# APRIL-ZJU/Ctrl-VIO

Measured on NVIDIA H100. Metric: residual+Jacobian block evaluations per second (sliding-window LM solve), higher is better.
Workload: dtype f64

## Files before the change

ctrl-vio_b200/csrc/engine.cu:

```cuda
#include <atomic>
#include <cmath>
#include <cstdlib>
#include <map>

#include "engine_state.h"

namespace ctvio::host {

int refresh_mirror(ctvio_engine* e) {
  const size_t need = 4 * size_t(e->nK) + kPStride * size_t(e->nK) + 6 * size_t(std::max(e->nB, 1)) + size_t(std::max(e->nL, 1)) + 8;
  if (need > e->h_mirror_cap) {
    if (e->h_mirror) cudaFreeHost(e->h_mirror);
    e->h_mirror = nullptr;
    e->h_mirror_cap = 0;
    if (cudaHostAlloc(reinterpret_cast<void**>(&e->h_mirror), (2 * need) * sizeof(double), cudaHostAllocDefault) != cudaSuccess) {
      cudaGetLastError();
      e->mirror_valid = false;
      return CTVIO_OK;
    }
    e->h_mirror_cap = 2 * need;
  }
  DevState& x = e->x[e->cur];
  double* m = e->h_mirror;
  cudaStream_t st = e->stream;
  CUDA_OK(cudaMemcpyAsync(m, x.q.p, 4 * size_t(e->nK) * sizeof(double), cudaMemcpyDeviceToHost, st));
  m += 4 * size_t(e->nK);
  CUDA_OK(cudaMemcpyAsync(m, x.p.p, kPStride * size_t(e->nK) * sizeof(double), cudaMemcpyDeviceToHost, st));
  m += kPStride * size_t(e->nK);
  if (e->nB) CUDA_OK(cudaMemcpyAsync(m, x.bias.p, 6 * size_t(e->nB) * sizeof(double), cudaMemcpyDeviceToHost, st));
  m += 6 * size_t(std::max(e->nB, 1));
  if (e->nL) CUDA_OK(cudaMemcpyAsync(m, x.rho.p, size_t(e->nL) * sizeof(double), cudaMemcpyDeviceToHost, st));
  m += size_t(std::max(e->nL, 1));
  CUDA_OK(cudaMemcpyAsync(m, x.ld.p, sizeof(double), cudaMemcpyDeviceToHost, st));
  e->mirror_valid = true;
  return CTVIO_OK;
}

int knot_window_first(const ctvio_engine* e, int64_t t) {
  int64_t s = (t - e->cfg.t0_ns) / e->cfg.dt_ns;
  return int(s);
}

bool knot_window(const ctvio_engine* e, int64_t t, int& first, int& last) {
  const int64_t maxt = e->cfg.t0_ns + int64_t(e->nK - 3) * e->cfg.dt_ns;
  if (t < e->cfg.t0_ns || t >= maxt) return false;
  const int smax = e->nK - 4;
  const int s1 = knot_window_first(e, t);
  int64_t t2 = t + e->cfg.rs_padding_ns;
  int s2 = (t2 >= maxt) ? smax : int((t2 - e->cfg.t0_ns) / e->cfg.dt_ns);
  if (s2 > s1 + 1) return false;
  first = s1;
  last = std::min(s2 + 3, e->nK - 1);
  return true;
}

int prepare_prior(ctvio_engine* e);
int fetch_new_prior(ctvio_engine* e);

int prepare(ctvio_engine* e) {
  if (!e->have_knots) return fail(CTVIO_ERR_STATE, "knots have not been set");
  ArenaScope arena(e);
  if (e->nK < 4) return fail(CTVIO_ERR_STATE, "need at least 4 knots");
  if (!e->have_bias) { e->nB = 0; }
  cudaStream_t st = e->stream;
  const ProblemDims d = e->dims();
  if (e->structure_dirty) {
    e->shard_checked = false;
    const int n = int(e->img.size());
    std::vector<int32_t>&wi0 = e->img_wi0, &wj0 = e->img_wj0;
    wi0.resize(n); wj0.resize(n);
    e->img_li.resize(n); e->img_lj.resize(n);
    e->h_lo.assign(e->nL, INT32_MAX);
    e->h_hi.assign(e->nL, 0);
    struct WinCache { int64_t t = INT64_MIN; int f = 0, l = 0; bool ok = false; } wc[64];
    auto window_of = [&](int64_t t, int& f, int& l) {
      WinCache& c = wc[size_t(uint64_t(t) * 0x9E3779B97F4A7C15ull >> 58)];
      if (c.t != t) { c.t = t; c.ok = knot_window(e, t, c.f, c.l); }
      f = c.f; l = c.l;
      return c.ok;
    };
    for (int k = 0; k < n; ++k) {
      const HostImage& o = e->img[k];
      int f0, l0, f1, l1;
      if (!window_of(o.ti, f0, l0) || !window_of(o.tj, f1, l1))
        return fail(CTVIO_ERR_TIME_RANGE, "image factor time (+ rolling-shutter padding) outside the spline");
      if (o.lm < 0 || o.lm >= e->nL) return fail(CTVIO_ERR_INVALID, "landmark index out of range");
      wi0[k] = f0; wj0[k] = f1;
      e->img_li[k] = l0; e->img_lj[k] = l1;
      e->h_lo[o.lm] = std::min(e->h_lo[o.lm], 6 * std::min(f0, f1));
      e->h_hi[o.lm] = std::max(e->h_hi[o.lm], 6 * (std::max(l0, l1) + 1));
    }
    e->img_order.resize(n);
    {
      bool lm_sorted = true;
      for (int k = 1; k < n && lm_sorted; ++k) lm_sorted = e->img[k - 1].lm <= e->img[k].lm;
      const size_t nKk = size_t(e->nK) + 1;
      if (lm_sorted && nKk * nKk <= (size_t(1) << 22)) {
        std::vector<int32_t> start(nKk * nKk + 1, 0);
        for (int k = 0; k < n; ++k) ++start[size_t(wi0[k]) * nKk + size_t(wj0[k]) + 1];
        for (size_t g = 1; g < start.size(); ++g) start[g] += start[g - 1];
        for (int k = 0; k < n; ++k) e->img_order[start[size_t(wi0[k]) * nKk + size_t(wj0[k])]++] = k;
      } else {
        std::vector<uint64_t> key(n);
        const uint64_t nLl = uint64_t(std::max(e->nL, 1));
        if (uint64_t(nKk) * nKk * nLl < (uint64_t(1) << 40) && uint64_t(n) < (uint64_t(1) << 24)) {
          for (int k = 0; k < n; ++k)
            key[k] = (((uint64_t(wi0[k]) * nKk + uint64_t(wj0[k])) * nLl + uint64_t(e->img[k].lm)) << 24) | uint64_t(k);
          std::sort(key.begin(), key.end());
          for (int k = 0; k < n; ++k) e->img_order[k] = int32_t(key[k] & 0xffffffu);
        } else {
          for (int k = 0; k < n; ++k) e->img_order[k] = k;
          std::stable_sort(e->img_order.begin(), e->img_order.end(), [&](int a, int b) {
            if (wi0[a] != wi0[b]) return wi0[a] < wi0[b];
            if (wj0[a] != wj0[b]) return wj0[a] < wj0[b];
            return e->img[a].lm < e->img[b].lm;
          });
        }
      }
    }
    std::vector<longlong2> ht(n);
    std::vector<double2> hpi(n), hpj(n);
    std::vector<int4> hm(n);
    for (int k = 0; k < n; ++k) {
      const HostImage& o = e->img[e->img_order[k]];
      ht[k] = make_longlong2(o.ti, o.tj);
      hpi[k] = make_double2(o.pi[0], o.pi[1]);
      hpj[k] = make_double2(o.pj[0], o.pj[1]);
      hm[k] = make_int4(o.rowi, o.rowj, o.lm, o.marg);
    }
    std::vector<int2> groups;
    for (int k = 0; k < n;) {
      const int a = e->img_order[k];
      int end = k;
      while (end < n && wi0[e->img_order[end]] == wi0[a] && wj0[e->img_order[end]] == wj0[a]) ++end;
      groups.push_back(make_int2(k, end));
      k = end;
    }
    auto n_chunks = [&](int c) {
      size_t m = 0;
      for (const int2& g : groups) m += (g.y - g.x + c - 1) / c;
      return m;
    };
    int cap = kVisObsPerRound;
    const size_t n_sm = size_t(device_sm_count());
    while (cap / 2 >= kVisMinChunk && n_chunks(cap / 2) <= n_sm) cap /= 2;
    std::vector<VisualItem>& items = e->h_items;
    items.clear();
    for (const int2& g : groups) {
      const int a = e->img_order[g.x];
      const int cnt = g.y - g.x;
      const int nchunks = (cnt + cap - 1) / cap;
      const int per = (cnt + nchunks - 1) / nchunks;
      for (int s = g.x; s < g.y; s += per) items.push_back(VisualItem{s, std::min(per, g.y - s), wi0[a], wj0[a]});
    }
    e->n_items = int(items.size());
    if (!e->img_desc.empty()) {
      std::vector<ctvio::FactorDesc> sd(n);
      for (int k = 0; k < n; ++k) sd[k] = e->img_desc[e->img_order[k]];
      CUDA_OK(e->d_img_desc.upload(sd, st));
      CUDA_OK(e->d_img_t.reserve(n)); CUDA_OK(e->d_img_pi.reserve(n)); CUDA_OK(e->d_img_pj.reserve(n)); CUDA_OK(e->d_img_meta.reserve(n));
      ctvio::GatherFactorsArgs ga;
      ga.n = n; ga.desc = e->d_img_desc.p; ga.table = e->d_frames.p; ga.frame_t = e->d_frame_t.p;
      ga.frame_cap = ctvio_engine::kFrameCap;
      ga.t = e->d_img_t.p; ga.pi = e->d_img_pi.p; ga.pj = e->d_img_pj.p; ga.meta = e->d_img_meta.p;
      e->launches += ctvio::launch_gather_factors(ga, st);
    } else {
      CUDA_OK(e->d_img_t.upload(ht, st));
      CUDA_OK(e->d_img_pi.upload(hpi, st));
      CUDA_OK(e->d_img_pj.upload(hpj, st));
      CUDA_OK(e->d_img_meta.upload(hm, st));
    }
    CUDA_OK(e->d_img_orig.upload(e->img_order, st));
    CUDA_OK(e->d_items.upload(items, st));

    e->h_woff.assign(e->nL + 1, 0);
    for (int l = 0; l < e->nL; ++l) {
      if (e->h_hi[l] == 0) e->h_lo[l] = 0;
      e->h_woff[l + 1] = e->h_woff[l] + (e->h_hi[l] - e->h_lo[l]);
    }
    CUDA_OK(e->d_lo.upload(e->h_lo, st));
    CUDA_OK(e->d_hi.upload(e->h_hi, st));
    CUDA_OK(e->d_woff.upload(e->h_woff, st));
    const int ni = int(e->imu.size());
    std::vector<longlong2> it(ni);
    std::vector<double2> iga(3 * size_t(ni));
    const int64_t maxt = e->cfg.t0_ns + int64_t(e->nK - 3) * e->cfg.dt_ns;
    std::vector<int32_t>& imu_order = e->imu_order;
    imu_order.assign(ni, 0);
    std::vector<int32_t> imu_s(ni);
    for (int k = 0; k < ni; ++k) {
      const HostImu& o = e->imu[k];
      if (o.t < e->cfg.t0_ns || o.t >= maxt) return fail(CTVIO_ERR_TIME_RANGE, "imu time outside the spline");
      if (o.node < 0 || o.node >= e->nB) return fail(CTVIO_ERR_INVALID, "bias node out of range");
      imu_order[k] = k;
      imu_s[k] = knot_window_first(e, o.t);
    }
    std::stable_sort(imu_order.begin(), imu_order.end(), [&](int a, int b) {
      if (imu_s[a] != imu_s[b]) return imu_s[a] < imu_s[b];
      return e->imu[a].node < e->imu[b].node;
    });
    std::vector<ImuItem> imu_items;
    for (int k = 0; k < ni; ++k) {
      const HostImu& o = e->imu[imu_order[k]];
      it[k] = make_longlong2(o.t, o.node);
      iga[3 * k] = make_double2(o.gyro[0], o.gyro[1]);
      iga[3 * k + 1] = make_double2(o.gyro[2], o.accel[0]);
      iga[3 * k + 2] = make_double2(o.accel[1], o.accel[2]);
      const int s = imu_s[imu_order[k]];
      if (imu_items.empty() || imu_items.back().s != s || imu_items.back().node != o.node ||
          imu_items.back().count >= kImuMaxPerItem)
        imu_items.push_back(ImuItem{k, 0, s, o.node});
      imu_items.back().count++;
    }
    e->n_imu_items = int(imu_items.size());
    CUDA_OK(e->d_imu_items.upload(imu_items, st));
    CUDA_OK(e->d_imu_orig.upload(imu_order, st));
    if (!e->imu_src.empty()) {
      std::vector<int2> src(ni);
      for (int k = 0; k < ni; ++k) src[k] = make_int2(e->imu_src[imu_order[k]], e->imu[imu_order[k]].node);
      CUDA_OK(e->d_imu_src.upload(src, st));
      CUDA_OK(e->d_imu_t.reserve(ni)); CUDA_OK(e->d_imu_ga.reserve(3 * size_t(ni)));
      e->launches += ctvio::launch_gather_imu(e->d_imu_src.p, ni, e->d_imu_tab_t.p, e->d_imu_tab_ga.p, e->d_imu_t.p, e->d_imu_ga.p, st);
    } else {
      CUDA_OK(e->d_imu_t.upload(it, st));
      CUDA_OK(e->d_imu_ga.upload(iga, st));
    }
    const int nb = int(e->biasf.size());
    std::vector<int2> bij(nb);
    std::vector<double> bs(6 * size_t(nb));
    for (int k = 0; k < nb; ++k) {
      const HostBias& o = e->biasf[k];
      if (o.i < 0 || o.i >= e->nB || o.j < 0 || o.j >= e->nB) return fail(CTVIO_ERR_INVALID, "bias node out of range");
      bij[k] = make_int2(o.i, o.j);
      for (int c = 0; c < 6; ++c) bs[6 * k + c] = o.s[c];
    }
    CUDA_OK(e->d_bf_ij.upload(bij, st));
    CUDA_OK(e->d_bf_s.upload(bs, st));

    const size_t np = size_t(d.np);
    e->off_gc = np * np;
    e->off_hl = e->off_gc + np;
    e->off_gl = e->off_hl + e->nL;
    e->off_wld = e->off_gl + e->nL;
    e->off_W = e->off_wld + e->nL;
    e->ne_slab_len = e->off_W + size_t(e->h_woff[e->nL]);
    for (int b = 0; b < 2; ++b) CUDA_OK(e->ne_slab[b].reserve(e->ne_slab_len));
    e->npad = ((d.np + kCholNB - 1) / kCholNB) * kCholNB;
    CUDA_OK(e->d_M.reserve(size_t(e->npad) * e->npad + 3 * size_t(e->npad)));
    if (chol_dag_lpub_len(e->npad) > e->d_Linv.cap || chol_dag_part_len(e->npad) > e->d_chol_part.cap || e->linv_npad != e->npad) {
      CUDA_OK(e->d_Linv.reserve(chol_dag_lpub_len(e->npad)));
      CUDA_OK(e->d_chol_part.reserve(chol_dag_part_len(e->npad)));
      e->launches += launch_chol_dag_init(e->d_Linv.p, e->d_chol_part.p, e->npad, e->stream);
      e->linv_npad = e->npad;
      e->chol_seq = 0;
    }
    {
      const int T = e->npad / kCholNB;
      std::vector<std::vector<int32_t>> lists(size_t(T) * (T + 1) / 2);
      std::vector<int32_t> order;
      for (int l = 0; l < e->nL; ++l)
        if (e->h_hi[l] > 0) order.push_back(l);
      std::stable_sort(order.begin(), order.end(), [&](int a, int b) {
        if (e->h_lo[a] != e->h_lo[b]) return e->h_lo[a] < e->h_lo[b];
        return e->h_hi[a] < e->h_hi[b];
      });
      size_t total = 0;
      for (int l : order) {
        int blocks[64], nbk = 0;
        const int b0 = e->h_lo[l] / kCholNB, b1 = (e->h_hi[l] - 1) / kCholNB;
        for (int b = b0; b <= b1 && nbk < 63; ++b) blocks[nbk++] = b;
        for (int x = 0; x < nbk; ++x)
          for (int y = 0; y <= x; ++y) {
            lists[size_t(blocks[x]) * (blocks[x] + 1) / 2 + blocks[y]].push_back(l);
            ++total;
          }
      }
      const int n_sm = device_sm_count();
      const int part = std::max(32, int((total / size_t(2 * n_sm) + 31) / 32) * 32);
      std::vector<SchurTileItem> items;
      std::vector<SchurEntry> flat;
      flat.reserve(total);
      for (int ti = 0; ti < T; ++ti)
        for (int tj = 0; tj <= ti; ++tj) {
          const std::vector<int32_t>& v = lists[size_t(ti) * (ti + 1) / 2 + tj];
          for (size_t s0 = 0; s0 < v.size(); s0 += part)
            items.push_back(SchurTileItem{ti, tj, int32_t(flat.size() + s0), int32_t(std::min(v.size() - s0, size_t(part)))});
          for (int32_t l : v) flat.push_back(SchurEntry{l, e->h_lo[l], e->h_hi[l], 0, e->h_woff[l]});
        }
      e->n_schur_items = int(items.size());
      CUDA_OK(e->d_schur_list.upload(flat, st));
      CUDA_OK(e->d_schur_items.upload(items, st));
      CUDA_OK(e->d_lis.reserve(e->nL));
      CUDA_OK(e->d_lc.reserve(e->nL));
    }
    if (chol_dag_flags_len(e->npad) > e->d_chol_flags.cap) {
      CUDA_OK(e->d_chol_flags.reserve(chol_dag_flags_len(e->npad)));
      CUDA_OK(cudaMemsetAsync(e->d_chol_flags.p, 0, e->d_chol_flags.cap * sizeof(int32_t), e->stream));
    }
    CUDA_OK(e->d_y.reserve(e->npad));
    CUDA_OK(e->d_sc.reserve(np));
    CUDA_OK(e->d_sl.reserve(e->nL));
    CUDA_OK(e->d_hh.reserve(e->nL));
    CUDA_OK(e->d_dc.reserve(np));
    CUDA_OK(e->d_dl.reserve(e->nL));
    if (e->nL > 0) CUDA_OK(cudaMemsetAsync(e->d_hh.p, 0, sizeof(double) * e->nL, st));
    e->prior_dirty = true;
  }
  if (e->structure_dirty || e->masks_dirty) {
    e->h_cmask.assign(d.np, 0);
    for (int k = 0; k < e->nK; ++k)
      if (e->opt.lock_traj || (e->opt.fixed_knot_index >= 0 && k <= e->opt.fixed_knot_index))
        for (int c = 0; c < 6; ++c) e->h_cmask[6 * k + c] = 1;
    for (int b = 0; b < e->nB; ++b)
      for (int c = 0; c < 3; ++c) {
        if (e->opt.lock_wb) e->h_cmask[d.idx_bias0 + 6 * b + c] = 1;
        if (e->opt.lock_ab) e->h_cmask[d.idx_bias0 + 6 * b + 3 + c] = 1;
      }
    if (e->opt.fix_ld) e->h_cmask[d.idx_ld] = 1;
    std::vector<uint8_t> touched(d.np + e->nL, 0);
    auto mark = [&](int f, int l) {
      for (int k = f; k <= l; ++k)
        for (int c = 0; c < 6; ++c) touched[6 * k + c] = 1;
    };
    {
      std::vector<uint8_t> seen(size_t(e->nK) * 8, 0);
      auto mark_once = [&](int f, int l) {
        uint8_t& sflag = seen[size_t(f) * 8 + size_t(l - f)];
        if (!sflag) { sflag = 1; mark(f, l); }
      };
      const size_t n = e->img.size();
      for (size_t k = 0; k < n; ++k) {
        mark_once(e->img_wi0[k], e->img_li[k]);
        mark_once(e->img_wj0[k], e->img_lj[k]);
        touched[d.np + e->img[k].lm] = 1;
      }
      if (n) touched[d.idx_ld] = 1;
    }
    for (const HostImu& o : e->imu) {
      const int s = knot_window_first(e, o.t);
      mark(s, s + 3);
      for (int c = 0; c < 6; ++c) touched[d.idx_bias0 + 6 * o.node + c] = 1;
    }
    for (const HostBias& o : e->biasf)
      for (int c = 0; c < 6; ++c) touched[d.idx_bias0 + 6 * o.i + c] = touched[d.idx_bias0 + 6 * o.j + c] = 1;
    if (e->prior.n > 0 && e->prior_enabled)
      for (size_t b = 0; b < e->prior.type.size(); ++b) {
        const int g = ctvio::prior_block_base(e->prior.type[b], e->prior.index[b], d.nK, d.nB);
        const int ls = (e->prior.type[b] == CTVIO_BLK_LD || e->prior.type[b] == CTVIO_BLK_RHO) ? 1 : 3;
        if (g >= 0) for (int c = 0; c < ls; ++c) touched[g + c] = 1;
      }
    e->h_active.assign(d.np + e->nL, 0);
    for (int i = 0; i < d.np; ++i) e->h_active[i] = touched[i] && !e->h_cmask[i];
    for (int l = 0; l < e->nL; ++l) e->h_active[d.np + l] = touched[d.np + l];
    CUDA_OK(e->d_cmask.upload(e->h_cmask, st));
    CUDA_OK(e->d_active.upload(e->h_active, st));
    e->masks_dirty = false;
  }
  e->structure_dirty = false;
  if (e->prior_dirty) {
    const int rc = prepare_prior(e);
    if (rc != CTVIO_OK) return rc;
  }
  return CTVIO_OK;
}

int prepare_prior(ctvio_engine* e) {
  const ProblemDims d = e->dims();
  const ctvio::PriorHost& pr = e->prior;
  e->prior_dirty = false;
  if (pr.n <= 0) return CTVIO_OK;
  cudaStream_t st = e->stream;
  std::vector<int32_t> col2g(pr.n, -1);
  for (size_t b = 0; b < pr.type.size(); ++b) {
    const int g = ctvio::prior_block_base(pr.type[b], pr.index[b], d.nK, d.nB);
    if (pr.type[b] == CTVIO_BLK_RHO) return fail(CTVIO_ERR_INVALID, "inverse-depth blocks cannot be part of a prior");
    if (g < 0) return fail(CTVIO_ERR_INVALID, "prior block index out of range");
    const int ls = pr.type[b] == CTVIO_BLK_LD ? 1 : 3;
    for (int c = 0; c < ls; ++c)
      if (!e->h_cmask[g + c]) col2g[pr.col[b] + c] = g + c;
  }
  if (!e->prior_on_device) {
    CUDA_OK(e->d_prior_J.upload(pr.J, st));
    CUDA_OK(e->d_prior_r.upload(pr.r, st));
    CUDA_OK(e->d_prior_x0.upload(pr.x0, st));
  }
  CUDA_OK(e->d_prior_type.upload(pr.type, st));
  CUDA_OK(e->d_prior_index.upload(pr.index, st));
  CUDA_OK(e->d_prior_col.upload(pr.col, st));
  CUDA_OK(e->d_prior_col2g.upload(col2g, st));
  CUDA_OK(e->d_prior_JtJ.reserve(size_t(pr.n) * pr.n));
  CUDA_OK(e->d_prior_dx.reserve(pr.n));
  CUDA_OK(e->d_prior_res.reserve(pr.n));
  CUDA_OK(cudaMemsetAsync(e->d_prior_dx.p, 0, size_t(pr.n) * sizeof(double), st));
  e->launches += ctvio::launch_gram(e->d_prior_J.p, pr.n, pr.n, e->d_prior_JtJ.p, st);
  return CTVIO_OK;
}

int fetch_new_prior(ctvio_engine* e) {
  ctvio::PriorHost& np_ = e->new_prior;
  if (e->new_prior_on_host || np_.n <= 0) return CTVIO_OK;
  np_.J.resize(size_t(np_.n) * np_.n);
  np_.r.resize(np_.n);
  np_.x0.resize(4 * np_.type.size());
  CUDA_OK(cudaMemcpyAsync(np_.J.data(), e->mws.J.p, np_.J.size() * sizeof(double), cudaMemcpyDeviceToHost, e->stream));
  CUDA_OK(cudaMemcpyAsync(np_.r.data(), e->mws.r.p, np_.r.size() * sizeof(double), cudaMemcpyDeviceToHost, e->stream));
  CUDA_OK(cudaMemcpyAsync(np_.x0.data(), e->d_newprior_x0.p, np_.x0.size() * sizeof(double), cudaMemcpyDeviceToHost, e->stream));
  CUDA_OK(cudaStreamSynchronize(e->stream));
  e->d2h_bytes += (np_.J.size() + np_.r.size() + np_.x0.size()) * sizeof(double);
  e->new_prior_on_host = true;
  return CTVIO_OK;
}

PriorPtrs prior_ptrs(ctvio_engine* e) {
  PriorPtrs p;
  std::memset(&p, 0, sizeof(p));
  p.n = e->prior_enabled ? e->prior.n : 0;
  if (p.n <= 0) return p;
  p.n_blocks = int(e->prior.type.size());
  p.J = e->d_prior_J.p; p.r = e->d_prior_r.p; p.JtJ = e->d_prior_JtJ.p;
  p.type = e->d_prior_type.p; p.index = e->d_prior_index.p; p.col = e->d_prior_col.p;
  p.x0 = e->d_prior_x0.p; p.col2g = e->d_prior_col2g.p;
  p.dx = e->d_prior_dx.p; p.res = e->d_prior_res.p;
  return p;
}

VisualLaunch visual_launch(ctvio_engine* e, int xb, int nb, double cauchy) {
  VisualLaunch v;
  v.obs = ImageObsPtrs{e->d_img_t.p, e->d_img_pi.p, e->d_img_pj.p, e->d_img_meta.p, int32_t(e->img.size())};
  v.items = e->d_items.p;
  v.n_items = e->n_items;
  v.st = e->state(xb).ptrs();
  v.ne = e->ne(nb);
  v.lm = e->lml();
  v.dims = e->dims();
  v.sp = e->sp;
  v.rig = e->rig;
  v.cauchy = cauchy;
  v.cmask = e->d_cmask.p;
  v.scal = e->d_scal.p;
  v.det_ticket = e->deterministic ? e->d_ticket.p : nullptr;
  return v;
}
ImuLaunch imu_launch(ctvio_engine* e, int xb, int nb) {
  ImuLaunch v;
  v.obs = ImuObsPtrs{e->d_imu_t.p, e->d_imu_ga.p, int32_t(e->imu.size())};
  v.items = e->d_imu_items.p;
  v.n_items = e->n_imu_items;
  v.st = e->state(xb).ptrs();
  v.ne = e->ne(nb);
  v.dims = e->dims();
  v.sp = e->sp;
  v.rig = e->rig;
  v.cmask = e->d_cmask.p;
  v.scal = e->d_scal.p;
  v.det_ticket = e->deterministic ? e->d_ticket.p : nullptr;
  return v;
}
SmallFactorsLaunch small_launch(ctvio_engine* e, int xb, int nb) {
  SmallFactorsLaunch v;
  v.bf = BiasFactorPtrs{e->d_bf_ij.p, e->d_bf_s.p, int32_t(e->biasf.size())};
  v.prior = prior_ptrs(e);
  v.st = e->state(xb).ptrs();
  v.ne = e->ne(nb);
  v.dims = e->dims();
  v.cmask = e->d_cmask.p;
  v.scal = e->d_scal.p;
  v.deterministic = e->deterministic ? 1 : 0;
  return v;
}
LinearLaunch linear_launch(ctvio_engine* e, int nb) {
  LinearLaunch a;
  a.dims = e->dims();
  a.ne = e->ne(nb);
  a.lm = e->lml();
  a.schur_list = e->d_schur_list.p;
  a.schur_items = e->d_schur_items.p;
  a.n_schur_items = e->n_schur_items;
  a.lis = e->d_lis.p; a.lc = e->d_lc.p;
  a.cmask = e->d_cmask.p;
  a.active = e->d_active.p;
  a.sc = e->d_sc.p; a.sl = e->d_sl.p;
  a.M = e->d_M.p; a.Linv = e->d_Linv.p; a.y = e->d_y.p;
  a.rhs = e->d_M.p + size_t(e->npad) * e->npad;
  a.diagA = a.rhs + e->npad;
  a.yf = a.diagA + e->npad;
  a.chol_part = e->d_chol_part.p; a.chol_flags = e->d_chol_flags.p; a.chol_seq = &e->chol_seq;
  a.sharded = e->world > 1 ? 1 : 0;
  a.hh = e->d_hh.p; a.dc = e->d_dc.p; a.dl = e->d_dl.p;
  a.npad = e->npad;
  a.scal = e->d_scal.p;
  a.go = nullptr;
  a.det_ticket = e->deterministic ? e->d_ticket.p : nullptr;
  return a;
}

void evaluate(ctvio_engine* e, int xb, int nb, bool full, bool reset_cost) {
  cudaStream_t st = e->stream;
  if (full) {
    if (e->slab_zeroed[nb]) {
      cudaStreamWaitEvent(st, e->ev_zero, 0);
      e->slab_zeroed[nb] = false;
    } else {
      cudaMemsetAsync(e->ne_slab[nb].p, 0, e->ne_slab_len * sizeof(double), st);
    }
  }
  if (reset_cost) cudaMemsetAsync(&e->d_scal.p->cost_eval, 0, sizeof(double), st);
  const bool fork = (e->rank == 0) && (!e->imu.empty() || !e->biasf.empty() || (e->prior.n > 0 && e->prior_enabled));
  if (e->deterministic) {
    cudaMemsetAsync(e->d_ticket.p, 0, 2 * sizeof(int32_t), st);
    e->launches += launch_visual(visual_launch(e, xb, nb, e->cfg.cauchy_solve), full, st);
    if (fork) {
      cudaMemsetAsync(e->d_ticket.p, 0, 2 * sizeof(int32_t), st);
      e->launches += launch_imu(imu_launch(e, xb, nb), full, st);
      e->launches += launch_small_factors(small_launch(e, xb, nb), full, st);
    }
    return;
  }
  const bool split = fork && !e->imu.empty() && (!e->biasf.empty() || (e->prior.n > 0 && e->prior_enabled));
  if (fork) {
    cudaEventRecord(e->ev_fork, st);
    cudaStreamWaitEvent(e->stream2, e->ev_fork, 0);
    e->launches += launch_imu(imu_launch(e, xb, nb), full, e->stream2);
    if (split) {
      cudaStreamWaitEvent(e->stream3, e->ev_fork, 0);
      e->launches += launch_small_factors(small_launch(e, xb, nb), full, e->stream3);
      cudaEventRecord(e->ev_join3, e->stream3);
    } else {
      e->launches += launch_small_factors(small_launch(e, xb, nb), full, e->stream2);
    }
    cudaEventRecord(e->ev_join, e->stream2);
  }
  e->launches += launch_visual(visual_launch(e, xb, nb, e->cfg.cauchy_solve), full, st);
  if (fork) cudaStreamWaitEvent(st, e->ev_join, 0);
  if (split) cudaStreamWaitEvent(st, e->ev_join3, 0);
}

int read_scalars(ctvio_engine* e, bool published) {
  if (published) {
    volatile unsigned long long* seq = &e->h_pub->seq;
    unsigned spins = 0;
    while (*seq != e->pub_seq) {
      if ((++spins & 0xfffu) == 0 && cudaStreamQuery(e->stream) != cudaErrorNotReady) {
        if (*seq == e->pub_seq) break;
        CUDA_OK(cudaStreamSynchronize(e->stream));
        CUDA_OK(cudaStreamSynchronize(e->stream2));
        if (*seq != e->pub_seq) return fail(CTVIO_ERR_CUDA, "LM step finished without publishing its scalars");
      }
    }
    std::atomic_thread_fence(std::memory_order_acquire);
    *e->h_scal = const_cast<const LmPublished*>(e->h_pub)->s;
  } else {
    CUDA_OK(cudaMemcpyAsync(e->h_scal, e->d_scal.p, sizeof(LmScalars), cudaMemcpyDeviceToHost, e->stream));
    CUDA_OK(cudaStreamSynchronize(e->stream));
  }
  if ((e->h_scal->error_flags & 1) || (e->world > 1 && e->h_scal->err_sum > 0.0)) {
    cudaMemsetAsync(&e->d_scal.p->error_flags, 0, sizeof(int32_t), e->stream);
    return fail(CTVIO_ERR_TIME_RANGE, "a factor time left its knot window / the spline (line delay too large?)");
  }
  return CTVIO_OK;
}

int alloc_state(ctvio_engine* e, DevState& s) {
  CUDA_OK(s.q.reserve(4 * size_t(e->nK)));
  CUDA_OK(s.p.reserve(kPStride * size_t(e->nK)));
  CUDA_OK(s.tab.reserve(size_t(std::max(e->nK - 1, 1))));
  CUDA_OK(s.bias.reserve(6 * size_t(std::max(e->nB, 1))));
  CUDA_OK(s.rho.reserve(size_t(std::max(e->nL, 1))));
  CUDA_OK(s.ld.reserve(1));
  return CTVIO_OK;
}

}

extern "C" {

const char* ctvio_last_error(void) { return g_err.c_str(); }
int ctvio_abi_version(void) { return CTVIO_ABI_VERSION; }

int ctvio_create(const ctvio_config* cfg, ctvio_handle* out) {
  if (!cfg || !out) return fail(CTVIO_ERR_INVALID, "null argument");
  if (cfg->dt_ns <= 0) return fail(CTVIO_ERR_INVALID, "dt_ns must be positive");
  if (cfg->rs_padding_ns < 0 || cfg->rs_padding_ns > cfg->dt_ns)
    return fail(CTVIO_ERR_INVALID, "rs_padding_ns must lie in [0, dt_ns]: the staged knot window holds 5 knots "
                                   "(4 + one interval of rolling-shutter padding, se3_spline.h:463-503 with 39 ms / 50 ms)");
  int ndev = 0;
  if (cudaGetDeviceCount(&ndev) != cudaSuccess || ndev == 0)
    return fail(CTVIO_ERR_NO_DEVICE, "no CUDA device visible: the ctvio engine has no CPU fallback");
  if (cfg->device < 0 || cfg->device >= ndev) return fail(CTVIO_ERR_NO_DEVICE, "device ordinal out of range");
  CUDA_OK(cudaSetDevice(cfg->device));
  cudaDeviceProp prop;
  CUDA_OK(cudaGetDeviceProperties(&prop, cfg->device));
  if (prop.major != 9 || prop.minor != 0)
    return fail(CTVIO_ERR_NO_DEVICE, "libctvio_b200 is built for sm_90a (H100) only");
  ctvio_engine* e = new ctvio_engine();
  e->cfg = *cfg;
  std::memset(&e->opt, 0, sizeof(e->opt));
  e->opt.fixed_knot_index = -1;
  e->opt.fix_ld = 1;
  e->sp = SplineParams{cfg->t0_ns, cfg->dt_ns, 0, 1e9 / double(cfg->dt_ns)};
  e->rig.R_CI = so3_matrix(Q4{cfg->q_CtoI[0], cfg->q_CtoI[1], cfg->q_CtoI[2], cfg->q_CtoI[3]});
  e->rig.p_CI = V3{cfg->p_CinI[0], cfg->p_CinI[1], cfg->p_CinI[2]};
  e->rig.w_img = cfg->image_weight;
  e->rig.gravity = V3{cfg->gravity[0], cfg->gravity[1], cfg->gravity[2]};
  for (int k = 0; k < 6; ++k) e->rig.imu_info[k] = cfg->imu_info[k];
  if (const char* det = std::getenv("CTVIO_DETERMINISTIC")) e->deterministic = det[0] == '1';
  if (cudaStreamCreateWithFlags(&e->stream, cudaStreamNonBlocking) != cudaSuccess ||
      cudaStreamCreateWithFlags(&e->stream2, cudaStreamNonBlocking) != cudaSuccess ||
      cudaStreamCreateWithFlags(&e->stream3, cudaStreamNonBlocking) != cudaSuccess ||
      cudaEventCreateWithFlags(&e->ev_join3, cudaEventDisableTiming) != cudaSuccess ||
      cudaEventCreate(&e->ev0) != cudaSuccess || cudaEventCreate(&e->ev1) != cudaSuccess ||
      cudaEventCreateWithFlags(&e->ev_fork, cudaEventDisableTiming) != cudaSuccess ||
      cudaEventCreateWithFlags(&e->ev_join, cudaEventDisableTiming) != cudaSuccess ||
      cudaEventCreateWithFlags(&e->ev_zero, cudaEventDisableTiming) != cudaSuccess ||
      e->d_dec.reserve(1) != cudaSuccess ||
      cudaHostAlloc(&e->h_pub, sizeof(LmPublished), cudaHostAllocMapped) != cudaSuccess ||
      cudaMallocHost(&e->h_scal, sizeof(LmScalars)) != cudaSuccess || e->d_scal.reserve(1) != cudaSuccess ||
      e->d_ticket.reserve(4) != cudaSuccess) {
    delete e;
    return fail(CTVIO_ERR_CUDA, "could not create stream / events / scalar block");
  }
  cudaMemsetAsync(e->d_scal.p, 0, sizeof(LmScalars), e->stream);
  std::memset(e->h_pub, 0, sizeof(LmPublished));
  *out = e;
  return CTVIO_OK;
}

int ctvio_destroy(ctvio_handle e) {
  if (!e) return CTVIO_OK;
  cudaSetDevice(e->cfg.device);
  cudaStreamSynchronize(e->stream);
  ctvio::comm_destroy(e->nccl_comm);
  if (e->h_scal) cudaFreeHost(e->h_scal);
  if (e->h_pub) cudaFreeHost(e->h_pub);
  if (e->h_mirror) cudaFreeHost(e->h_mirror);
  if (e->ft.h_map_head) cudaFreeHost(e->ft.h_map_head);
  if (e->ev_zero) cudaEventDestroy(e->ev_zero);
  cudaEventDestroy(e->ev0);
  cudaEventDestroy(e->ev1);
  cudaEventDestroy(e->ev_fork);
  cudaEventDestroy(e->ev_join);
  cudaStreamDestroy(e->stream2);
  if (e->stream3) cudaStreamDestroy(e->stream3);
  if (e->ev_join3) cudaEventDestroy(e->ev_join3);
  cudaStreamDestroy(e->stream);
  delete e;
  return CTVIO_OK;
}

int ctvio_set_options(ctvio_handle e, const ctvio_options* o) {
  if (!e || !o) return fail(CTVIO_ERR_INVALID, "null argument");
  e->opt = *o;
  e->masks_dirty = true;
  e->prior_dirty = true;
  return CTVIO_OK;
}

int ctvio_set_knots(ctvio_handle e, int32_t n, const double* q, const double* p) {
  if (!e || !q || !p || n < 4) return fail(CTVIO_ERR_INVALID, "need >= 4 knots");
  cudaSetDevice(e->cfg.device);
  if (n != e->nK) e->structure_dirty = true;
  e->nK = n;
  e->sp.n_knots = n;
  for (int b = 0; b < 2; ++b) { const int rc = alloc_state(e, e->x[b]); if (rc) return rc; }
  ArenaScope arena(e);
  std::vector<double> p4(kPStride * size_t(n), 0.0);
  for (int k = 0; k < n; ++k) for (int c = 0; c < 3; ++c) p4[kPStride * k + c] = p[3 * k + c];
  CUDA_OK(staged_h2d(e->x[e->cur].q.p, q, 4 * size_t(n) * sizeof(double), e->stream));
  CUDA_OK(staged_h2d(e->x[e->cur].p.p, p4.data(), p4.size() * sizeof(double), e->stream));
  e->mirror_valid = false;
  e->h2d_bytes += size_t(n) * 56;
  e->have_knots = true;
  e->table_valid = false;
  return CTVIO_OK;
}

int ctvio_set_biases(ctvio_handle e, int32_t n, const double* b) {
  if (!e || (n > 0 && !b) || n < 0) return fail(CTVIO_ERR_INVALID, "bad bias array");
  cudaSetDevice(e->cfg.device);
  if (n != e->nB) e->structure_dirty = true;
  e->nB = n;
  for (int k = 0; k < 2; ++k) CUDA_OK(e->x[k].bias.reserve(6 * size_t(std::max(n, 1))));
  ArenaScope arena(e);
  if (n > 0) CUDA_OK(staged_h2d(e->x[e->cur].bias.p, b, 6 * size_t(n) * sizeof(double), e->stream));
  e->mirror_valid = false;
  e->h2d_bytes += size_t(n) * 48;
  e->have_bias = true;
  return CTVIO_OK;
}

int ctvio_set_inv_depths(ctvio_handle e, int32_t n, const double* r) {
  if (!e || (n > 0 && !r) || n < 0) return fail(CTVIO_ERR_INVALID, "bad inverse-depth array");
  cudaSetDevice(e->cfg.device);
  if (n != e->nL) e->structure_dirty = true;
  e->nL = n;
  for (int k = 0; k < 2; ++k) CUDA_OK(e->x[k].rho.reserve(size_t(std::max(n, 1))));
  ArenaScope arena(e);
  if (n > 0) CUDA_OK(staged_h2d(e->x[e->cur].rho.p, r, size_t(n) * sizeof(double), e->stream));
  e->mirror_valid = false;
  e->h2d_bytes += size_t(n) * 8;
  e->have_rho = true;
  return CTVIO_OK;
}

int ctvio_set_time_origin(ctvio_handle e, int64_t t0_ns) {
  if (!e) return fail(CTVIO_ERR_INVALID, "null handle");
  if ((t0_ns - e->cfg.t0_ns) % e->cfg.dt_ns != 0) return fail(CTVIO_ERR_INVALID, "time origin off the knot grid");
  e->cfg.t0_ns = t0_ns;
  e->sp.t0_ns = t0_ns;
  e->structure_dirty = true;
  e->table_valid = false;
  return CTVIO_OK;
}

int ctvio_set_line_delay(ctvio_handle e, double ld) {
  if (!e) return fail(CTVIO_ERR_INVALID, "null handle");
  cudaSetDevice(e->cfg.device);
  for (int k = 0; k < 2; ++k) CUDA_OK(e->x[k].ld.reserve(1));
  ArenaScope arena(e);
  CUDA_OK(staged_h2d(e->x[e->cur].ld.p, &ld, sizeof(double), e->stream));
  e->mirror_valid = false;
  return CTVIO_OK;
}

int ctvio_get_knots(ctvio_handle e, double* q, double* p) {
  if (!e || !e->have_knots) return fail(CTVIO_ERR_STATE, "knots have not been set");
  cudaSetDevice(e->cfg.device);
  e->d2h_bytes += size_t(e->nK) * ((q ? 32 : 0) + (p ? 32 : 0));
  if (e->mirror_valid) {
    const double* mq = e->h_mirror;
    const double* mp = mq + 4 * size_t(e->nK);
    if (q) std::memcpy(q, mq, 4 * size_t(e->nK) * sizeof(double));
    if (p) for (int k = 0; k < e->nK; ++k) for (int c = 0; c < 3; ++c) p[3 * k + c] = mp[kPStride * k + c];
    return CTVIO_OK;
  }
  if (q) CUDA_OK(cudaMemcpyAsync(q, e->x[e->cur].q.p, 4 * size_t(e->nK) * sizeof(double), cudaMemcpyDeviceToHost, e->stream));
  std::vector<double> p4;
  if (p) {
    p4.resize(kPStride * size_t(e->nK));
    CUDA_OK(cudaMemcpyAsync(p4.data(), e->x[e->cur].p.p, p4.size() * sizeof(double), cudaMemcpyDeviceToHost, e->stream));
  }
  CUDA_OK(cudaStreamSynchronize(e->stream));
  if (p) for (int k = 0; k < e->nK; ++k) for (int c = 0; c < 3; ++c) p[3 * k + c] = p4[kPStride * k + c];
  return CTVIO_OK;
}
int ctvio_get_biases(ctvio_handle e, double* b) {
  if (!e || !b) return fail(CTVIO_ERR_INVALID, "null argument");
  cudaSetDevice(e->cfg.device);
  e->d2h_bytes += size_t(e->nB) * 48;
  if (e->mirror_valid) {
    std::memcpy(b, e->h_mirror + (4 + kPStride) * size_t(e->nK), 6 * size_t(e->nB) * sizeof(double));
    return CTVIO_OK;
  }
  if (e->nB > 0) CUDA_OK(cudaMemcpyAsync(b, e->x[e->cur].bias.p, 6 * size_t(e->nB) * sizeof(double), cudaMemcpyDeviceToHost, e->stream));
  CUDA_OK(cudaStreamSynchronize(e->stream));
  return CTVIO_OK;
}
int ctvio_get_inv_depths(ctvio_handle e, double* r) {
  if (!e || !r) return fail(CTVIO_ERR_INVALID, "null argument");
  cudaSetDevice(e->cfg.device);
  e->d2h_bytes += size_t(e->nL) * 8;
  if (e->mirror_valid) {
    std::memcpy(r, e->h_mirror + (4 + kPStride) * size_t(e->nK) + 6 * size_t(std::max(e->nB, 1)), size_t(e->nL) * sizeof(double));
    return CTVIO_OK;
  }
  if (e->nL > 0) CUDA_OK(cudaMemcpyAsync(r, e->x[e->cur].rho.p, size_t(e->nL) * sizeof(double), cudaMemcpyDeviceToHost, e->stream));
  CUDA_OK(cudaStreamSynchronize(e->stream));
  return CTVIO_OK;
}
int ctvio_get_line_delay(ctvio_handle e, double* ld) {
  if (!e || !ld) return fail(CTVIO_ERR_INVALID, "null argument");
  cudaSetDevice(e->cfg.device);
  if (e->mirror_valid) {
    *ld = e->h_mirror[(4 + kPStride) * size_t(e->nK) + 6 * size_t(std::max(e->nB, 1)) + size_t(std::max(e->nL, 1))];
    return CTVIO_OK;
  }
  CUDA_OK(cudaMemcpyAsync(ld, e->x[e->cur].ld.p, sizeof(double), cudaMemcpyDeviceToHost, e->stream));
  CUDA_OK(cudaStreamSynchronize(e->stream));
  return CTVIO_OK;
}

int ctvio_clear_factors(ctvio_handle e) {
  if (!e) return fail(CTVIO_ERR_INVALID, "null handle");
  e->img.clear(); e->imu.clear(); e->biasf.clear();
  e->img_desc.clear(); e->imu_src.clear();
  e->structure_dirty = true;
  return CTVIO_OK;
}

int ctvio_add_image_features(ctvio_handle e, int32_t n, const int64_t* ti, const int32_t* rowi, const double* pi,
                             const int64_t* tj, const int32_t* rowj, const double* pj, const int32_t* lm,
                             const int32_t* marg) {
  if (!e || n < 0 || (n > 0 && (!ti || !rowi || !pi || !tj || !rowj || !pj || !lm)))
    return fail(CTVIO_ERR_INVALID, "null argument");
  if (!e->img_desc.empty()) return fail(CTVIO_ERR_STATE, "image factors from the resident tables are already present");
  e->img.reserve(e->img.size() + n);
  for (int k = 0; k < n; ++k) {
    HostImage o{ti[k], tj[k], rowi[k], rowj[k], {pi[2 * k], pi[2 * k + 1]}, {pj[2 * k], pj[2 * k + 1]}, lm[k],
                marg ? marg[k] : 0};
    e->img.push_back(o);
  }
  e->structure_dirty = true;
  return CTVIO_OK;
}
int ctvio_add_imu_measurements(ctvio_handle e, int32_t n, const int64_t* t, const double* gyro, const double* accel,
                               const int32_t* node, const int32_t* marg) {
  if (!e || n < 0 || (n > 0 && (!t || !gyro || !accel || !node))) return fail(CTVIO_ERR_INVALID, "null argument");
  if (!e->imu_src.empty()) return fail(CTVIO_ERR_STATE, "IMU factors from the resident table are already present");
  for (int k = 0; k < n; ++k) {
    HostImu o{t[k], {gyro[3 * k], gyro[3 * k + 1], gyro[3 * k + 2]}, {accel[3 * k], accel[3 * k + 1], accel[3 * k + 2]},
              node[k], marg ? marg[k] : 0};
    e->imu.push_back(o);
  }
  e->structure_dirty = true;
  return CTVIO_OK;
}
int ctvio_add_bias_factors(ctvio_handle e, int32_t n, const int32_t* ni, const int32_t* nj, const double* s,
                           const int32_t* marg) {
  if (!e || n < 0 || (n > 0 && (!ni || !nj || !s))) return fail(CTVIO_ERR_INVALID, "null argument");
  for (int k = 0; k < n; ++k) {
    HostBias o{ni[k], nj[k], {s[6 * k], s[6 * k + 1], s[6 * k + 2], s[6 * k + 3], s[6 * k + 4], s[6 * k + 5]},
               marg ? marg[k] : 0};
    e->biasf.push_back(o);
  }
  e->structure_dirty = true;
  return CTVIO_OK;
}

int ctvio_set_prior(ctvio_handle e, int32_t n, const double* J, const double* r, int32_t nb, const int32_t* type,
                    const int32_t* index, const int32_t* col, const double* x0) {
  if (!e) return fail(CTVIO_ERR_INVALID, "null handle");
  e->prior = ctvio::PriorHost();
  e->prior_dirty = true;
  e->prior_on_device = false;
  e->masks_dirty = true;
  if (n <= 0) return CTVIO_OK;
  if (!J || !r || nb <= 0 || !type || !index || !col || !x0) return fail(CTVIO_ERR_INVALID, "null argument");
  {
    std::vector<uint8_t> covered(size_t(n), 0);
    for (int b = 0; b < nb; ++b) {
      if (type[b] < CTVIO_BLK_ROT || type[b] > CTVIO_BLK_RHO) return fail(CTVIO_ERR_INVALID, "prior block type out of range");
      const int ls = (type[b] == CTVIO_BLK_LD || type[b] == CTVIO_BLK_RHO) ? 1 : 3;
      if (col[b] < 0 || col[b] + ls > n) return fail(CTVIO_ERR_INVALID, "prior block column outside [0, n)");
      for (int c = 0; c < ls; ++c) {
        if (covered[col[b] + c]) return fail(CTVIO_ERR_INVALID, "prior blocks overlap");
        covered[col[b] + c] = 1;
      }
    }
    for (int c = 0; c < n; ++c)
      if (!covered[c]) return fail(CTVIO_ERR_INVALID, "prior blocks do not cover all n columns");
  }
  e->prior.n = n;
  e->prior.J.assign(J, J + size_t(n) * n);
  e->prior.r.assign(r, r + n);
  e->prior.type.assign(type, type + nb);
  e->prior.index.assign(index, index + nb);
  e->prior.col.assign(col, col + nb);
  e->prior.x0.assign(x0, x0 + 4 * size_t(nb));
  return CTVIO_OK;
}

int ctvio_gauge_realign(ctvio_handle e, int32_t min_idx, const double* R0, const double* t0) {
  if (!e || !R0 || !t0 || min_idx < 0 || min_idx >= e->nK) return fail(CTVIO_ERR_INVALID, "bad argument");
  cudaSetDevice(e->cfg.device);
  CUDA_OK(e->d_tmp.reserve(12));
  double h[12];
  for (int k = 0; k < 9; ++k) h[k] = R0[k];
  for (int k = 0; k < 3; ++k) h[9 + k] = t0[k];
  CUDA_OK(cudaMemcpyAsync(e->d_tmp.p, h, sizeof(h), cudaMemcpyHostToDevice, e->stream));
  e->launches += launch_gauge_realign(e->x[e->cur].ptrs(), e->nK, min_idx, e->d_tmp.p, e->stream);
  {
    const int rcm = refresh_mirror(e);
    if (rcm) return rcm;
  }
  CUDA_OK(cudaStreamSynchronize(e->stream));
  e->table_valid = true;
  return CTVIO_OK;
}

int ctvio_save_state(ctvio_handle e) {
  if (!e || !e->have_knots) return fail(CTVIO_ERR_STATE, "state not set");
  cudaSetDevice(e->cfg.device);
  int rc = alloc_state(e, e->snap);
  if (rc) return rc;
  DevState& s = e->x[e->cur];
  cudaStream_t st = e->stream;
  CUDA_OK(cudaMemcpyAsync(e->snap.q.p, s.q.p, 4 * size_t(e->nK) * sizeof(double), cudaMemcpyDeviceToDevice, st));
  CUDA_OK(cudaMemcpyAsync(e->snap.p.p, s.p.p, kPStride * size_t(e->nK) * sizeof(double), cudaMemcpyDeviceToDevice, st));
  if (e->nB) CUDA_OK(cudaMemcpyAsync(e->snap.bias.p, s.bias.p, 6 * size_t(e->nB) * sizeof(double), cudaMemcpyDeviceToDevice, st));
  if (e->nL) CUDA_OK(cudaMemcpyAsync(e->snap.rho.p, s.rho.p, size_t(e->nL) * sizeof(double), cudaMemcpyDeviceToDevice, st));
  CUDA_OK(cudaMemcpyAsync(e->snap.ld.p, s.ld.p, sizeof(double), cudaMemcpyDeviceToDevice, st));
  return CTVIO_OK;
}
int ctvio_restore_state(ctvio_handle e) {
  if (!e || !e->snap.q.p) return fail(CTVIO_ERR_STATE, "no snapshot");
  cudaSetDevice(e->cfg.device);
  DevState& s = e->x[e->cur];
  cudaStream_t st = e->stream;
  CUDA_OK(cudaMemcpyAsync(s.q.p, e->snap.q.p, 4 * size_t(e->nK) * sizeof(double), cudaMemcpyDeviceToDevice, st));
  CUDA_OK(cudaMemcpyAsync(s.p.p, e->snap.p.p, kPStride * size_t(e->nK) * sizeof(double), cudaMemcpyDeviceToDevice, st));
  if (e->nB) CUDA_OK(cudaMemcpyAsync(s.bias.p, e->snap.bias.p, 6 * size_t(e->nB) * sizeof(double), cudaMemcpyDeviceToDevice, st));
  if (e->nL) CUDA_OK(cudaMemcpyAsync(s.rho.p, e->snap.rho.p, size_t(e->nL) * sizeof(double), cudaMemcpyDeviceToDevice, st));
  CUDA_OK(cudaMemcpyAsync(s.ld.p, e->snap.ld.p, sizeof(double), cudaMemcpyDeviceToDevice, st));
  e->table_valid = false;
  e->mirror_valid = false;
  return CTVIO_OK;
}

int ctvio_eval_image_factors(ctvio_handle e, int32_t want_jac, double cauchy, double* r, int32_t* s, double* J,
                             double* cost) {
  if (!e) return fail(CTVIO_ERR_INVALID, "null handle");
  cudaSetDevice(e->cfg.device);
  int rc = prepare(e);
  if (rc) return rc;
  ensure_table(e);
  const size_t n = e->img.size();
  DevBuf<double> dr, dJ;
  DevBuf<int32_t> ds;
  CUDA_OK(dr.reserve(2 * n));
  CUDA_OK(ds.reserve(2 * n));
  if (want_jac) CUDA_OK(dJ.reserve(100 * n));
  cudaStream_t st = e->stream;
  cudaMemsetAsync(&e->d_scal.p->cost_eval, 0, sizeof(double), st);
  e->launches += launch_probe_image(visual_launch(e, e->cur, e->cur, cauchy), e->d_img_orig.p, want_jac != 0, dr.p, ds.p,
                                    want_jac ? dJ.p : nullptr, st);
  rc = read_scalars(e);
  if (rc) return rc;
  if (r && n) CUDA_OK(cudaMemcpy(r, dr.p, 2 * n * sizeof(double), cudaMemcpyDeviceToHost));
  if (s && n) CUDA_OK(cudaMemcpy(s, ds.p, 2 * n * sizeof(int32_t), cudaMemcpyDeviceToHost));
  if (J && want_jac && n) CUDA_OK(cudaMemcpy(J, dJ.p, 100 * n * sizeof(double), cudaMemcpyDeviceToHost));
  if (cost) *cost = e->h_scal->cost_eval;
  return CTVIO_OK;
}

int ctvio_eval_imu_factors(ctvio_handle e, int32_t want_jac, double* r, int32_t* s, double* J, double* cost) {
  if (!e) return fail(CTVIO_ERR_INVALID, "null handle");
  cudaSetDevice(e->cfg.device);
  int rc = prepare(e);
  if (rc) return rc;
  ensure_table(e);
  const size_t n = e->imu.size();
  DevBuf<double> dr, dJ;
  DevBuf<int32_t> ds;
  CUDA_OK(dr.reserve(6 * n));
  CUDA_OK(ds.reserve(n));
  if (want_jac) CUDA_OK(dJ.reserve(156 * n));
  cudaStream_t st = e->stream;
  cudaMemsetAsync(&e->d_scal.p->cost_eval, 0, sizeof(double), st);
  e->launches += launch_probe_imu(imu_launch(e, e->cur, e->cur), e->d_imu_orig.p, want_jac != 0, dr.p, ds.p,
                                  want_jac ? dJ.p : nullptr, st);
  rc = read_scalars(e);
  if (rc) return rc;
  if (r && n) CUDA_OK(cudaMemcpy(r, dr.p, 6 * n * sizeof(double), cudaMemcpyDeviceToHost));
  if (s && n) CUDA_OK(cudaMemcpy(s, ds.p, n * sizeof(int32_t), cudaMemcpyDeviceToHost));
  if (J && want_jac && n) CUDA_OK(cudaMemcpy(J, dJ.p, 156 * n * sizeof(double), cudaMemcpyDeviceToHost));
  if (cost) *cost = e->h_scal->cost_eval;
  return CTVIO_OK;
}

int ctvio_residual_summary(ctvio_handle e, int32_t* counts, double* sums, double* prior_sum) {
  if (!e || !counts || !sums) return fail(CTVIO_ERR_INVALID, "null argument");
  cudaSetDevice(e->cfg.device);
  int rc = prepare(e);
  if (rc) return rc;
  ensure_table(e);
  cudaStream_t st = e->stream;
  const size_t ni = e->img.size(), nm = e->imu.size(), nb = e->biasf.size();
  const int np_ = e->prior_enabled ? e->prior.n : 0;
  DevBuf<double> dr, dout;
  DevBuf<int32_t> ds;
  CUDA_OK(dr.reserve(2 * ni + 6 * nm + 8));
  CUDA_OK(ds.reserve(2 * ni + nm + 8));
  CUDA_OK(dout.reserve(18));
  CUDA_OK(cudaMemsetAsync(dout.p, 0, 18 * sizeof(double), st));
  if (ni) e->launches += launch_probe_image(visual_launch(e, e->cur, e->cur, 0.0), e->d_img_orig.p, false, dr.p, ds.p, nullptr, st);
  if (nm) e->launches += launch_probe_imu(imu_launch(e, e->cur, e->cur), e->d_imu_orig.p, false, dr.p + 2 * ni, ds.p + 2 * ni, nullptr, st);
  e->launches += ctvio::launch_abs_column_sums(dr.p, int(ni), 2, dout.p, st);
  e->launches += ctvio::launch_abs_column_sums(dr.p + 2 * ni, int(nm), 6, dout.p + 2, st);
  e->launches += ctvio::launch_bias_abs_sums(e->d_bf_ij.p, e->d_bf_s.p, int(nb), e->x[e->cur].bias.p, dout.p + 8, st);
  if (np_ > 0) {
    e->launches += launch_small_factors(small_launch(e, e->cur, e->cur), false, st);
  }
  rc = read_scalars(e);
  if (rc) return rc;
  CUDA_OK(cudaMemcpy(sums, dout.p, 18 * sizeof(double), cudaMemcpyDeviceToHost));
  counts[0] = int32_t(ni); counts[1] = int32_t(nm); counts[2] = int32_t(nb); counts[3] = np_ > 0 ? 1 : 0;
  if (prior_sum && np_ > 0) {
    CUDA_OK(cudaMemcpy(prior_sum, e->d_prior_res.p, size_t(np_) * sizeof(double), cudaMemcpyDeviceToHost));
    for (int i = 0; i < np_; ++i) prior_sum[i] = std::fabs(prior_sum[i]);
  }
  return CTVIO_OK;
}

int ctvio_eval_cost(ctvio_handle e, double* cost) {
  if (!e || !cost) return fail(CTVIO_ERR_INVALID, "null argument");
  cudaSetDevice(e->cfg.device);
  int rc = prepare(e);
  if (rc) return rc;
  ensure_table(e);
  evaluate(e, e->cur, e->cur, false);
  rc = read_scalars(e);
  if (rc) return rc;
  *cost = e->h_scal->cost_eval;
  return CTVIO_OK;
}

int ctvio_normal_equations(ctvio_handle e, double* Hcc, double* gc, double* hl, double* gl, double* cost) {
  if (!e) return fail(CTVIO_ERR_INVALID, "null handle");
  cudaSetDevice(e->cfg.device);
  int rc = prepare(e);
  if (rc) return rc;
  ensure_table(e);
  evaluate(e, e->cur, e->cur, true);
  rc = read_scalars(e);
  if (rc) return rc;
  const ProblemDims d = e->dims();
  const size_t np = d.np;
  NormalEqPtrs ne = e->ne(e->cur);
  if (Hcc) {
    std::vector<double> up(np * np);
    CUDA_OK(cudaMemcpy(up.data(), ne.A, np * np * sizeof(double), cudaMemcpyDeviceToHost));
    for (size_t i = 0; i < np; ++i)
      for (size_t j = i; j < np; ++j) Hcc[i * np + j] = Hcc[j * np + i] = up[i * np + j];
  }
  if (gc) CUDA_OK(cudaMemcpy(gc, ne.gc, np * sizeof(double), cudaMemcpyDeviceToHost));
  if (hl && e->nL) CUDA_OK(cudaMemcpy(hl, ne.hl, e->nL * sizeof(double), cudaMemcpyDeviceToHost));
  if (gl && e->nL) CUDA_OK(cudaMemcpy(gl, ne.gl, e->nL * sizeof(double), cudaMemcpyDeviceToHost));
  if (cost) *cost = e->h_scal->cost_eval;
  return CTVIO_OK;
}

int ctvio_query_trajectory(ctvio_handle e, int32_t n, const int64_t* t, double* q, double* p, double* omega,
                           double* vel, double* acc) {
  if (!e || n < 0 || (n > 0 && !t)) return fail(CTVIO_ERR_INVALID, "bad argument");
  if (!e->have_knots) return fail(CTVIO_ERR_STATE, "knots have not been set");
  cudaSetDevice(e->cfg.device);
  ensure_table(e);
  if (n == 0) return CTVIO_OK;
  DevBuf<int64_t> dt;
  DevBuf<double> out;
  CUDA_OK(dt.reserve(n));
  CUDA_OK(out.reserve(16 * size_t(n)));
  cudaStream_t st = e->stream;
  CUDA_OK(cudaMemcpyAsync(dt.p, t, size_t(n) * sizeof(int64_t), cudaMemcpyHostToDevice, st));
  QueryLaunch a;
  a.st = e->x[e->cur].ptrs();
  a.sp = e->sp;
  a.n = n;
  a.t = dt.p;
  a.q = out.p; a.p = out.p + 4 * size_t(n); a.omega = out.p + 7 * size_t(n); a.vel = out.p + 10 * size_t(n);
  a.acc = out.p + 13 * size_t(n);
  a.scal = e->d_scal.p;
  e->launches += launch_query(a, st);
  int rc = read_scalars(e);
  if (rc) return rc;
  if (q) CUDA_OK(cudaMemcpy(q, a.q, 4 * size_t(n) * sizeof(double), cudaMemcpyDeviceToHost));
  if (p) CUDA_OK(cudaMemcpy(p, a.p, 3 * size_t(n) * sizeof(double), cudaMemcpyDeviceToHost));
  if (omega) CUDA_OK(cudaMemcpy(omega, a.omega, 3 * size_t(n) * sizeof(double), cudaMemcpyDeviceToHost));
  if (vel) CUDA_OK(cudaMemcpy(vel, a.vel, 3 * size_t(n) * sizeof(double), cudaMemcpyDeviceToHost));
  if (acc) CUDA_OK(cudaMemcpy(acc, a.acc, 3 * size_t(n) * sizeof(double), cudaMemcpyDeviceToHost));
  return CTVIO_OK;
}

int ctvio_profile_kernels(ctvio_handle e, int32_t reps, int32_t flush_l2, double* out) {
  if (!e || !out || reps == 0) return fail(CTVIO_ERR_INVALID, "bad argument");
  const bool visual_only = reps < 0;
  if (visual_only) reps = -reps;
  cudaSetDevice(e->cfg.device);
  int rc = prepare(e);
  if (rc) return rc;
  ensure_table(e);
  cudaStream_t st = e->stream;
  const int cur = e->cur, cand = cur ^ 1;
  DevBuf<unsigned char> flush;
  const size_t flush_bytes = size_t(256) << 20;
  if (flush_l2) CUDA_OK(flush.reserve(flush_bytes));
  if (visual_only) {
    for (int k = 0; k < 8; ++k) out[k] = 0.0;
    double total = 0;
    for (int it = -3; it < reps; ++it) {
      if (flush_l2) cudaMemsetAsync(flush.p, it & 0xff, flush_bytes, st);
      cudaMemsetAsync(e->ne_slab[cur].p, 0, e->ne_slab_len * sizeof(double), st);
      cudaEventRecord(e->ev0, st);
      launch_visual(visual_launch(e, cur, cur, e->cfg.cauchy_solve), true, st);
      cudaEventRecord(e->ev1, st);
      if (cudaEventSynchronize(e->ev1) != cudaSuccess) return fail(CTVIO_ERR_CUDA, "kernel failed while profiling");
      float ms = 0;
      cudaEventElapsedTime(&ms, e->ev0, e->ev1);
      if (it >= 0) total += ms;
    }
    out[0] = total / reps;
    cudaMemsetAsync(&e->d_scal.p->error_flags, 0, sizeof(int32_t), st);
    CUDA_OK(cudaStreamSynchronize(st));
    return CTVIO_OK;
  }
  evaluate(e, cur, cur, true);
  LinearLaunch lin = linear_launch(e, cur);
  launch_jacobi_scale(lin, st);
  launch_lm_step(lin, 1e4, st);
  rc = read_scalars(e);
  if (rc) return rc;
  ApplyLaunch ap;
  ap.dims = e->dims();
  ap.x = e->x[cur].ptrs(); ap.xc = e->x[cand].ptrs();
  ap.dc = e->d_dc.p; ap.dl = e->d_dl.p; ap.alpha = 1.0; ap.active = e->d_active.p;
  ap.count_camera = 1;
  ap.clamp_ld = e->opt.fix_ld ? 0 : 1; ap.ld_lower = e->opt.ld_lower; ap.ld_upper = e->opt.ld_upper;
  ap.scal = e->d_scal.p;
  auto time_stage = [&](int stage, double* ms_out) -> int {
    double total = 0;
    for (int it = -3; it < reps; ++it) {
      if (flush_l2) cudaMemsetAsync(flush.p, it & 0xff, flush_bytes, st);
      if (stage == 0 || stage == 1 || stage == 2)
        cudaMemsetAsync(e->ne_slab[cur].p, 0, e->ne_slab_len * sizeof(double), st);
      cudaEventRecord(e->ev0, st);
      switch (stage) {
        case 0: launch_visual(visual_launch(e, cur, cur, e->cfg.cauchy_solve), true, st); break;
        case 1: launch_imu(imu_launch(e, cur, cur), true, st); break;
        case 2: launch_small_factors(small_launch(e, cur, cur), true, st); break;
        case 3: launch_reduced_system(lin, 1e4, st); break;
        case 4: launch_factor_solve(lin, st); break;
        case 5: launch_step_vectors(lin, st); break;
        case 6: launch_apply_step(ap, st); break;
        default: launch_visual(visual_launch(e, cur, cur, e->cfg.cauchy_solve), false, st); break;
      }
      cudaEventRecord(e->ev1, st);
      if (cudaEventSynchronize(e->ev1) != cudaSuccess) return fail(CTVIO_ERR_CUDA, "kernel failed while profiling");
      float ms = 0;
      cudaEventElapsedTime(&ms, e->ev0, e->ev1);
      if (it >= 0) total += ms;
    }
    *ms_out = total / reps;
    return CTVIO_OK;
  };
  for (int stage : {0, 1, 2, 7}) { rc = time_stage(stage, &out[stage]); if (rc) return rc; }
  evaluate(e, cur, cur, true);
  {
    double total3 = 0, total4 = 0, total5 = 0;
    for (int it = -3; it < reps; ++it) {
      float ms;
      if (flush_l2) cudaMemsetAsync(flush.p, it & 0xff, flush_bytes, st);
      cudaEventRecord(e->ev0, st); launch_reduced_system(lin, 1e4, st); cudaEventRecord(e->ev1, st);
      cudaEventSynchronize(e->ev1); cudaEventElapsedTime(&ms, e->ev0, e->ev1); if (it >= 0) total3 += ms;
      if (flush_l2) cudaMemsetAsync(flush.p, it & 0xff, flush_bytes, st);
      cudaEventRecord(e->ev0, st); launch_factor_solve(lin, st); cudaEventRecord(e->ev1, st);
      cudaEventSynchronize(e->ev1); cudaEventElapsedTime(&ms, e->ev0, e->ev1); if (it >= 0) total4 += ms;
      if (flush_l2) cudaMemsetAsync(flush.p, it & 0xff, flush_bytes, st);
      cudaEventRecord(e->ev0, st); launch_step_vectors(lin, st); cudaEventRecord(e->ev1, st);
      cudaEventSynchronize(e->ev1); cudaEventElapsedTime(&ms, e->ev0, e->ev1); if (it >= 0) total5 += ms;
    }
    out[3] = total3 / reps; out[4] = total4 / reps; out[5] = total5 / reps;
  }
  rc = time_stage(6, &out[6]);
  if (rc) return rc;
  cudaMemsetAsync(&e->d_scal.p->error_flags, 0, sizeof(int32_t), st);
  CUDA_OK(cudaStreamSynchronize(st));
  return CTVIO_OK;
}

int ctvio_selfcheck_solver(ctvio_handle e, int32_t reps, int32_t* mismatches, double* rel_residual) {
  if (!e || !mismatches || !rel_residual || reps <= 0) return fail(CTVIO_ERR_INVALID, "bad argument");
  cudaSetDevice(e->cfg.device);
  int rc = prepare(e);
  if (rc) return rc;
  ensure_table(e);
  cudaStream_t st = e->stream;
  const int cur = e->cur;
  evaluate(e, cur, cur, true);
  LinearLaunch lin = linear_launch(e, cur);
  launch_jacobi_scale(lin, st);
  launch_reduced_system(lin, 1e4, st);
  const size_t n = size_t(e->npad), len = n * n + n;
  DevBuf<double> backup;
  CUDA_OK(backup.reserve(len));
  CUDA_OK(cudaMemcpyAsync(backup.p, lin.M, len * sizeof(double), cudaMemcpyDeviceToDevice, st));
  std::vector<double> hM(len), x0(n), x(n);
  CUDA_OK(cudaMemcpyAsync(hM.data(), lin.M, len * sizeof(double), cudaMemcpyDeviceToHost, st));
  *mismatches = 0;
  for (int r = 0; r < reps; ++r) {
    if (r > 0) CUDA_OK(cudaMemcpyAsync(lin.M, backup.p, len * sizeof(double), cudaMemcpyDeviceToDevice, st));
    launch_factor_solve(lin, st);
    CUDA_OK(cudaMemcpyAsync((r == 0 ? x0 : x).data(), lin.y, n * sizeof(double), cudaMemcpyDeviceToHost, st));
    CUDA_OK(cudaStreamSynchronize(st));
    if (r > 0 && std::memcmp(x.data(), x0.data(), n * sizeof(double)) != 0) ++*mismatches;
  }
  for (size_t i = 0; i < n; ++i)
    for (size_t j = i + 1; j < n; ++j) hM[i * n + j] = hM[j * n + i];
  const double* rhs = hM.data() + n * n;
  double rmax = 0, bmax = 0;
  for (size_t i = 0; i < n; ++i) {
    double s = -rhs[i];
    for (size_t j = 0; j < n; ++j) s += hM[i * n + j] * x0[j];
    rmax = std::max(rmax, std::fabs(s));
    bmax = std::max(bmax, std::fabs(rhs[i]));
  }
  *rel_residual = bmax > 0 ? rmax / bmax : rmax;
  cudaMemsetAsync(&e->d_scal.p->error_flags, 0, sizeof(int32_t), st);
  CUDA_OK(cudaStreamSynchronize(st));
  return CTVIO_OK;
}

int ctvio_measure_fp64_tflops(ctvio_handle e, double* tflops) {
  if (!e || !tflops) return fail(CTVIO_ERR_INVALID, "null argument");
  cudaSetDevice(e->cfg.device);
  const double v = ctvio::measure_fp64_tflops(e->stream);
  if (v < 0) return fail(CTVIO_ERR_CUDA, "fp64 micro-benchmark failed");
  *tflops = v;
  return CTVIO_OK;
}

int ctvio_measure_fp64_tensor_tflops(ctvio_handle e, double* tflops) {
  if (!e || !tflops) return fail(CTVIO_ERR_INVALID, "null argument");
  cudaSetDevice(e->cfg.device);
  const double v = ctvio::measure_fp64_tensor_tflops(e->stream);
  if (v < 0) return fail(CTVIO_ERR_CUDA, "fp64 tensor-core micro-benchmark failed");
  *tflops = v;
  return CTVIO_OK;
}

int ctvio_marginalize(ctvio_handle e, int32_t* n_out, int32_t* nb_out) {
  if (!e || !n_out || !nb_out) return fail(CTVIO_ERR_INVALID, "null argument");
  *n_out = 0;
  *nb_out = 0;
  cudaSetDevice(e->cfg.device);
  e->new_prior = ctvio::PriorHost();
  if (!e->opt.is_marg_state) return CTVIO_OK;
  ArenaScope arena(e);
  int rc = prepare(e);
  if (rc) return rc;
  ensure_table(e);
  cudaStream_t st = e->stream;
  const ProblemDims d = e->dims();
  const int later = e->opt.ctrl_to_be_opt_later, nowk = e->opt.ctrl_to_be_opt_now;
  const bool drop_knots = later > nowk;

  struct Key {
    int type, index;
    bool operator<(const Key& o) const {
      auto rank = [](const Key& k) {
        switch (k.type) {
          case CTVIO_BLK_ROT: return std::make_pair(0, 2 * k.index);
          case CTVIO_BLK_POS: return std::make_pair(0, 2 * k.index + 1);
          case CTVIO_BLK_BG: return std::make_pair(1, 2 * k.index);
          case CTVIO_BLK_BA: return std::make_pair(1, 2 * k.index + 1);
          case CTVIO_BLK_LD: return std::make_pair(2, 0);
          default: return std::make_pair(3, k.index);
        }
      };
      return rank(*this) < rank(o);
    }
  };
  struct Info { bool dropped = false; int pos = -1; };
  std::map<Key, Info> blocks;
  auto touch = [&](int type, int index, bool drop) { Info& b = blocks[Key{type, index}]; b.dropped = b.dropped || drop; };
  bool use_prior = false;
  if (e->prior.n > 0) {
    auto is_drop = [&](size_t b) {
      const int t = e->prior.type[b], i = e->prior.index[b];
      const bool isknot = t == CTVIO_BLK_ROT || t == CTVIO_BLK_POS;
      return (isknot && i >= nowk && i < later) || ((t == CTVIO_BLK_BG || t == CTVIO_BLK_BA) && i == 0);
    };
    for (size_t b = 0; b < e->prior.type.size(); ++b) use_prior = use_prior || is_drop(b);
    if (use_prior)
      for (size_t b = 0; b < e->prior.type.size(); ++b) touch(e->prior.type[b], e->prior.index[b], is_drop(b));
  }
  std::vector<int32_t> marg_img, marg_imu;
  for (size_t k = 0; k < e->img_order.size(); ++k) {
    const HostImage& o = e->img[e->img_order[k]];
    if (!o.marg) continue;
    marg_img.push_back(int32_t(k));
    int f0, l0, f1, l1;
    knot_window(e, o.ti, f0, l0);
    knot_window(e, o.tj, f1, l1);
    for (int side = 0; side < 2; ++side)
      for (int kk = (side ? f1 : f0); kk <= (side ? l1 : l0); ++kk) {
        touch(CTVIO_BLK_ROT, kk, drop_knots && kk < later);
        touch(CTVIO_BLK_POS, kk, drop_knots && kk < later);
      }
    touch(CTVIO_BLK_RHO, o.lm, true);
    touch(CTVIO_BLK_LD, 0, false);
  }
  for (size_t k = 0; k < e->imu_order.size(); ++k) {
    const HostImu& o = e->imu[e->imu_order[k]];
    if (!o.marg) continue;
    marg_imu.push_back(int32_t(k));
    const int s = knot_window_first(e, o.t);
    for (int kk = s; kk <= s + 3; ++kk) {
      touch(CTVIO_BLK_ROT, kk, drop_knots && kk < later);
      touch(CTVIO_BLK_POS, kk, drop_knots && kk < later);
    }
    touch(CTVIO_BLK_BG, o.node, true);
    touch(CTVIO_BLK_BA, o.node, true);
  }
  std::vector<int2> bij;
  std::vector<double> bs;
  for (const HostBias& o : e->biasf) {
    if (!o.marg) continue;
    bij.push_back(make_int2(o.i, o.j));
    for (int c = 0; c < 6; ++c) bs.push_back(o.s[c]);
    touch(CTVIO_BLK_BG, o.i, true); touch(CTVIO_BLK_BG, o.j, false);
    touch(CTVIO_BLK_BA, o.i, true); touch(CTVIO_BLK_BA, o.j, false);
  }
  if (blocks.empty()) return CTVIO_OK;
  auto local_size = [](int t) { return (t == CTVIO_BLK_LD || t == CTVIO_BLK_RHO) ? 1 : 3; };
  int pos = 0;
  for (auto& kv : blocks) if (kv.second.dropped) { kv.second.pos = pos; pos += local_size(kv.first.type); }
  const int m = pos;
  for (auto& kv : blocks) if (!kv.second.dropped) { kv.second.pos = pos; pos += local_size(kv.first.type); }
  const int n = pos - m, P = pos;
  if (n <= 0) return CTVIO_OK;

  std::vector<int32_t> pos_cam(d.np, -1), pos_lm(std::max(e->nL, 1), -1), prior_pos(std::max(e->prior.n, 1), -1);
  for (const auto& kv : blocks) {
    if (kv.first.type == CTVIO_BLK_RHO) { pos_lm[kv.first.index] = kv.second.pos; continue; }
    const int g = ctvio::prior_block_base(kv.first.type, kv.first.index, d.nK, d.nB);
    if (g < 0) return fail(CTVIO_ERR_INVALID, "marginalization block index out of range");
    for (int c = 0; c < local_size(kv.first.type); ++c) pos_cam[g + c] = kv.second.pos + c;
  }
  if (use_prior)
    for (size_t b = 0; b < e->prior.type.size(); ++b) {
      const int p0 = blocks[Key{e->prior.type[b], e->prior.index[b]}].pos;
      for (int c = 0; c < local_size(e->prior.type[b]); ++c) prior_pos[e->prior.col[b] + c] = p0 + c;
    }

  ctvio_engine::MargWs& ws = e->mws;
  DevBuf<int32_t>&d_pos_cam = ws.pos_cam, &d_pos_lm = ws.pos_lm, &d_prior_pos = ws.prior_pos, &d_marg_img = ws.marg_img,
      &d_marg_imu = ws.marg_imu;
  DevBuf<int2>& d_bij = ws.bij;
  DevBuf<double>&d_bs = ws.bs, &d_A = ws.A, &d_b = ws.b;
  CUDA_OK(d_pos_cam.upload(pos_cam, st));
  CUDA_OK(d_pos_lm.upload(pos_lm, st));
  CUDA_OK(d_prior_pos.upload(prior_pos, st));
  CUDA_OK(d_marg_img.upload(marg_img, st));
  CUDA_OK(d_marg_imu.upload(marg_imu, st));
  CUDA_OK(d_bij.upload(bij, st));
  CUDA_OK(d_bs.upload(bs, st));
  CUDA_OK(d_A.reserve(size_t(P) * P));
  CUDA_OK(d_b.reserve(P));
  {
    const int n_old = use_prior ? e->prior.n : 0;
    const int row_img = 0, row_imu = 2 * int(marg_img.size()), row_bias = row_imu + 6 * int(marg_imu.size());
    const int row_prior = row_bias + 6 * int(bij.size());
    const int R = row_prior + n_old;
    const int ldj = (P + 2) & ~1;
    CUDA_OK(ws.Jrow.reserve(size_t(std::max(R, 1)) * ldj));
    CUDA_OK(cudaMemsetAsync(ws.Jrow.p, 0, size_t(std::max(R, 1)) * ldj * sizeof(double), st));
    ctvio::MargImageArgs a;
    a.obs = ImageObsPtrs{e->d_img_t.p, e->d_img_pi.p, e->d_img_pj.p, e->d_img_meta.p, int32_t(e->img.size())};
    a.marg_index = d_marg_img.p; a.n_marg = int32_t(marg_img.size());
    a.st = e->x[e->cur].ptrs(); a.sp = e->sp; a.rig = e->rig; a.cauchy = e->cfg.cauchy_marg;
    a.pos_cam = d_pos_cam.p; a.pos_lm = d_pos_lm.p; a.idx_ld = d.idx_ld;
    a.Jrow = ws.Jrow.p; a.ldj = ldj; a.row0 = row_img; a.P = P; a.scal = e->d_scal.p;
    cudaEventRecord(e->ev_fork, st);
    e->launches += ctvio::launch_marg_image(a, st);
    ctvio::MargImuArgs b;
    b.obs = ImuObsPtrs{e->d_imu_t.p, e->d_imu_ga.p, int32_t(e->imu.size())};
    b.marg_index = d_marg_imu.p; b.n_marg = int32_t(marg_imu.size());
    b.st = a.st; b.sp = e->sp; b.rig = e->rig; b.pos_cam = d_pos_cam.p; b.idx_bias0 = d.idx_bias0;
    b.Jrow = ws.Jrow.p; b.ldj = ldj; b.row0 = row_imu; b.P = P; b.scal = e->d_scal.p;
    cudaStreamWaitEvent(e->stream2, e->ev_fork, 0);
    e->launches += ctvio::launch_marg_imu(b, e->stream2);
    cudaEventRecord(e->ev_join, e->stream2);
    ctvio::MargSmallArgs c;
    c.bf_ij = d_bij.p; c.bf_s = d_bs.p; c.n_bias = int32_t(bij.size());
    c.prior = prior_ptrs(e); c.use_prior = use_prior ? 1 : 0; c.prior_pos = d_prior_pos.p;
    c.st = a.st; c.pos_cam = d_pos_cam.p; c.idx_bias0 = d.idx_bias0;
    c.Jrow = ws.Jrow.p; c.ldj = ldj; c.row0_bias = row_bias; c.row0_prior = row_prior; c.P = P;
    cudaStreamWaitEvent(e->stream3, e->ev_fork, 0);
    e->launches += ctvio::launch_marg_small(c, e->stream3);
    cudaEventRecord(e->ev_join3, e->stream3);
    cudaStreamWaitEvent(st, e->ev_join, 0);
    cudaStreamWaitEvent(st, e->ev_join3, 0);
    e->launches += ctvio::launch_marg_syrk(ws.Jrow.p, R, ldj, P, d_A.p, d_b.p, st);
  }
  const double eps = 1e-30;
  auto eig = [&](double* A, double* V, double* ev, int k) {
    const int launched = ctvio::launch_jacobi_eig(A, V, ev, k, ws.eig_scratch.p, st);
    if (launched < 0) return fail(CTVIO_ERR_CUDA, "marginalization: eigen-solver launch refused at n = " + std::to_string(k));
    e->launches += launched;
    return int(CTVIO_OK);
  };
  DevBuf<double>&d_Amm = ws.Amm, &d_V = ws.V, &d_ev = ws.ev, &d_Vs = ws.Vs, &d_Ainv = ws.Ainv, &d_T = ws.T, &d_Ap = ws.Ap,
      &d_bp = ws.bp, &d_Ap2 = ws.Ap2, &d_V2 = ws.V2, &d_ev2 = ws.ev2, &d_vb = ws.vb, &d_J = ws.J, &d_r = ws.r;
  CUDA_OK(d_Ap.reserve(size_t(n) * n));
  CUDA_OK(d_bp.reserve(n));
  CUDA_OK(cudaMemcpy2DAsync(d_Ap.p, size_t(n) * sizeof(double), d_A.p + size_t(m) * P + m, size_t(P) * sizeof(double),
                            size_t(n) * sizeof(double), n, cudaMemcpyDeviceToDevice, st));
  CUDA_OK(cudaMemcpyAsync(d_bp.p, d_b.p + m, size_t(n) * sizeof(double), cudaMemcpyDeviceToDevice, st));
  if (m > 0) {
    CUDA_OK(d_Amm.reserve(size_t(m) * m)); CUDA_OK(d_V.reserve(size_t(m) * m)); CUDA_OK(d_ev.reserve(m));
    CUDA_OK(d_Vs.reserve(size_t(m) * m)); CUDA_OK(d_Ainv.reserve(size_t(m) * m)); CUDA_OK(d_T.reserve(size_t(n) * m));
    e->launches += ctvio::launch_marg_elementwise(0, m, P, d_A.p, d_Amm.p, nullptr, nullptr, nullptr, eps, st);
    CUDA_OK(ws.eig_scratch.reserve(ctvio::jacobi_log_bytes(std::max(m, n), 40) / sizeof(double) + 1));
    if ((rc = eig(d_Amm.p, d_V.p, d_ev.p, m))) return rc;
    e->launches += ctvio::launch_marg_elementwise(1, m, m, d_V.p, d_Vs.p, d_ev.p, nullptr, nullptr, eps, st);
    e->launches += ctvio::launch_dense_gemm(m, m, m, 1.0, d_Vs.p, m, false, d_V.p, m, true, 0.0, d_Ainv.p, m, st);
    e->launches += ctvio::launch_dense_gemm(n, m, m, 1.0, d_A.p + size_t(m) * P, P, false, d_Ainv.p, m, false, 0.0, d_T.p, m, st);
    e->launches += ctvio::launch_dense_gemm(n, n, m, -1.0, d_T.p, m, false, d_A.p + m, P, false, 1.0, d_Ap.p, n, st);
    e->launches += ctvio::launch_dense_gemm(n, 1, m, -1.0, d_T.p, m, false, d_b.p, 1, false, 1.0, d_bp.p, 1, st);
  }
  CUDA_OK(d_Ap2.reserve(size_t(n) * n)); CUDA_OK(d_V2.reserve(size_t(n) * n)); CUDA_OK(d_ev2.reserve(n));
  CUDA_OK(d_vb.reserve(n)); CUDA_OK(d_J.reserve(size_t(n) * n)); CUDA_OK(d_r.reserve(n));
  e->launches += ctvio::launch_marg_elementwise(2, n, n, d_Ap.p, d_Ap2.p, nullptr, nullptr, nullptr, eps, st);
  CUDA_OK(ws.eig_scratch.reserve(ctvio::jacobi_log_bytes(n, 40) / sizeof(double) + 1));
  if ((rc = eig(d_Ap2.p, d_V2.p, d_ev2.p, n))) return rc;
  e->launches += ctvio::launch_dense_gemm(n, 1, n, 1.0, d_V2.p, n, true, d_bp.p, 1, false, 0.0, d_vb.p, 1, st);
  e->launches += ctvio::launch_marg_elementwise(3, n, n, d_V2.p, d_J.p, d_ev2.p, d_vb.p, d_r.p, eps, st);
  rc = read_scalars(e);
  if (rc) return rc;

  ctvio::PriorHost& np_ = e->new_prior;
  np_.n = n;
  e->new_prior_on_host = false;
  for (const auto& kv : blocks) {
    if (kv.second.dropped) continue;
    np_.type.push_back(kv.first.type);
    np_.index.push_back(kv.first.index);
    np_.col.push_back(kv.second.pos - m);
  }
  {
    DevBuf<int32_t>&d_t = ws.pos_cam, &d_i = ws.pos_lm;
    CUDA_OK(d_t.upload(np_.type, st));
    CUDA_OK(d_i.upload(np_.index, st));
    CUDA_OK(e->d_newprior_x0.reserve(4 * np_.type.size()));
    e->launches += ctvio::launch_prior_x0(e->x[e->cur].ptrs(), d_t.p, d_i.p, int(np_.type.size()), e->d_newprior_x0.p, st);
    CUDA_OK(cudaStreamSynchronize(st));
  }
// ... 81 lines not shown
```

ctrl-vio_b200/csrc/engine_state.h:

```cpp
#pragma once
#include <algorithm>
#include <cstring>
#include <string>
#include <vector>

#include "../../include/ctvio.h"
#include "frontend.h"
#include "marginalize.h"

namespace ctvio::host {

inline thread_local std::string g_err;
inline int fail(int code, const std::string& msg) {
  g_err = msg;
  return code;
}

#define CUDA_OK(call)                                                                                   \
  do {                                                                                                  \
    cudaError_t e_ = (call);                                                                            \
    if (e_ != cudaSuccess)                                                                              \
      return fail(CTVIO_ERR_CUDA, std::string(#call) + ": " + cudaGetErrorString(e_));                  \
  } while (0)

inline thread_local size_t g_upload_bytes = 0;

struct PinnedArena {
  unsigned char* base = nullptr;
  size_t cap = 0, need = 0;
  ~PinnedArena() { if (base) cudaFreeHost(base); }
  void rewind() {
    if (need > cap) {
      if (base) cudaFreeHost(base);
      base = nullptr;
      cap = 0;
      const size_t n = std::max<size_t>(size_t(1) << 20, need + need / 2);
      if (cudaHostAlloc(reinterpret_cast<void**>(&base), n, cudaHostAllocDefault) == cudaSuccess) cap = n;
      else cudaGetLastError();
    }
    need = 0;
  }
  void* put(const void* src, size_t bytes) {
    const size_t o = (need + 15) & ~size_t(15);
    need = o + bytes;
    if (!base || need > cap) return nullptr;
    std::memcpy(base + o, src, bytes);
    return base + o;
  }
};
inline thread_local PinnedArena* g_arena = nullptr;

inline cudaError_t staged_h2d(void* dst, const void* src, size_t bytes, cudaStream_t s) {
  if (bytes == 0) return cudaSuccess;
  if (g_arena) {
    if (void* st = g_arena->put(src, bytes)) return cudaMemcpyAsync(dst, st, bytes, cudaMemcpyHostToDevice, s);
  }
  return cudaMemcpyAsync(dst, src, bytes, cudaMemcpyHostToDevice, s);
}

template <typename T>
struct DevBuf {
  T* p = nullptr;
  size_t cap = 0;
  ~DevBuf() { if (p) cudaFree(p); }
  cudaError_t reserve(size_t n) {
    if (n <= cap) return cudaSuccess;
    if (p) cudaFree(p);
    p = nullptr;
    cap = 0;
    cudaError_t e = cudaMalloc(&p, std::max<size_t>(n, 1) * sizeof(T));
    if (e == cudaSuccess) cap = n;
    return e;
  }
  cudaError_t grow(size_t n, size_t from, size_t count, cudaStream_t s) {
    DevBuf<T> nb;
    cudaError_t e = nb.reserve(n);
    if (e == cudaSuccess && count) e = cudaMemcpyAsync(nb.p, p + from, count * sizeof(T), cudaMemcpyDeviceToDevice, s);
    if (e == cudaSuccess) e = cudaStreamSynchronize(s);
    if (e == cudaSuccess) swap(*this, nb);
    return e;
  }
  cudaError_t upload(const std::vector<T>& h, cudaStream_t s) {
    cudaError_t e = reserve(h.size());
    if (e != cudaSuccess || h.empty()) return e;
    g_upload_bytes += h.size() * sizeof(T);
    return staged_h2d(p, h.data(), h.size() * sizeof(T), s);
  }
};
template <typename T>
void swap(DevBuf<T>& a, DevBuf<T>& b) { std::swap(a.p, b.p); std::swap(a.cap, b.cap); }

struct DevState {
  DevBuf<double> q, p, bias, rho, ld;
  DevBuf<KnotPair> tab;
  StatePtrs ptrs() { return StatePtrs{q.p, p.p, bias.p, rho.p, ld.p, tab.p}; }
};

struct HostImage { int64_t ti, tj; int32_t rowi, rowj; double pi[2], pj[2]; int32_t lm, marg; };
struct HostImu { int64_t t; double gyro[3], accel[3]; int32_t node, marg; };
struct HostBias { int32_t i, j; double s[6]; int32_t marg; };

}

using namespace ctvio;
using namespace ctvio::host;

struct ctvio_engine {
  ctvio_config cfg;
  ctvio_options opt;
  cudaStream_t stream = nullptr, stream2 = nullptr, stream3 = nullptr;
  cudaEvent_t ev_join3 = nullptr;
  cudaEvent_t ev0 = nullptr, ev1 = nullptr, ev_fork = nullptr, ev_join = nullptr;
  bool masks_dirty = true;
  SplineParams sp;
  RigParams rig;
  bool deterministic = false;
  DevBuf<int32_t> d_ticket;

  int nK = 0, nB = 0, nL = 0;
  bool have_knots = false, have_bias = false, have_rho = false;

  DevState x[2], snap;
  DevState xs;
  DevBuf<LmDecision> d_dec;
  DevState& state(int i) { return i < 2 ? x[i] : xs; }
  int cur = 0;
  bool table_valid = false;

  std::vector<HostImage> img;
  std::vector<HostImu> imu;
  std::vector<HostBias> biasf;
  bool structure_dirty = true;

  DevBuf<longlong2> d_img_t;
  DevBuf<double2> d_img_pi, d_img_pj;
  DevBuf<int4> d_img_meta;
  DevBuf<int32_t> d_img_orig;
  DevBuf<VisualItem> d_items;
  int n_items = 0;
  std::vector<int32_t> img_order;
  std::vector<int32_t> img_li, img_lj;
  std::vector<int32_t> img_wi0, img_wj0;
  std::vector<VisualItem> h_items;
  std::vector<int32_t> imu_order;
  DevBuf<longlong2> d_imu_t;
  DevBuf<double2> d_imu_ga;
  DevBuf<ImuItem> d_imu_items;
  DevBuf<int32_t> d_imu_orig;
  int n_imu_items = 0;
  DevBuf<int2> d_bf_ij;
  DevBuf<double> d_bf_s;

  std::vector<int32_t> h_lo, h_hi;
  std::vector<int64_t> h_woff;
  DevBuf<int32_t> d_lo, d_hi;
  DevBuf<SchurEntry> d_schur_list;
  DevBuf<int64_t> d_woff;
  DevBuf<SchurTileItem> d_schur_items;
  DevBuf<double> d_lis, d_lc;
  int n_schur_items = 0;
  DevBuf<uint8_t> d_cmask, d_active;
  std::vector<uint8_t> h_cmask, h_active;

  DevBuf<double> ne_slab[2];
  size_t ne_slab_len = 0;
  size_t off_gc = 0, off_hl = 0, off_gl = 0, off_wld = 0, off_W = 0;
  DevBuf<double> d_M, d_Linv, d_y, d_sc, d_sl, d_hh, d_dc, d_dl, d_rho_sync, d_chol_part;
  DevBuf<int32_t> d_chol_flags;
  DevBuf<uint8_t> d_owned;
  DevBuf<double> d_shard_pack, d_shard_scal;
  int npad = 0, linv_npad = -1;
  unsigned chol_seq = 0;
  DevBuf<LmScalars> d_scal;
  LmScalars* h_scal = nullptr;
  LmPublished* h_pub = nullptr;
  unsigned long long pub_seq = 0;
  cudaEvent_t ev_zero = nullptr;
  bool slab_zeroed[2] = {false, false};

  ctvio::PriorHost prior, new_prior;
  DevBuf<double> d_prior_J, d_prior_r, d_prior_JtJ, d_prior_x0, d_prior_dx, d_prior_res;
  DevBuf<int32_t> d_prior_type, d_prior_index, d_prior_col, d_prior_col2g;
  bool prior_dirty = true;
  bool prior_enabled = true;
  bool prior_on_device = false;
  bool new_prior_on_host = false;
  DevBuf<double> d_newprior_x0;
  static constexpr int kFrameSlots = ctvio::kKeyframeMaxSlots, kFrameCap = ctvio::kKeyframeMaxFeatures;
  DevBuf<ctvio::FrameFeature> d_frames;
  DevBuf<int64_t> d_frame_t;
  DevBuf<float> d_cloud_stage;
  int64_t h_frame_t[16] = {0};
  int32_t h_frame_n[16] = {0};
  std::vector<ctvio::FactorDesc> img_desc;
  DevBuf<ctvio::FactorDesc> d_img_desc;
  DevBuf<longlong2> d_imu_tab_t;
  DevBuf<double2> d_imu_tab_ga;
  DevBuf<unsigned char> d_imu_raw;
  std::vector<int64_t> h_imu_tab_t;
  std::vector<int32_t> imu_src;
  DevBuf<int2> d_imu_src;
  PinnedArena arena;
  double* h_mirror = nullptr;
  size_t h_mirror_cap = 0;
  bool mirror_valid = false;
  size_t h2d_bytes = 0, d2h_bytes = 0;

  DevBuf<double> d_tmp;
  DevBuf<int32_t> d_tri_idx;
  DevBuf<int32_t> d_tri_cnt;
  DevBuf<ctvio::KeyframeResult> d_kf_result;
  uint32_t h_frame_ingested = 0;
  struct FeatureTable {
    DevBuf<int32_t> id, anchor, lm, idx, new_index;
    DevBuf<uint32_t> mask;
    DevBuf<double> rho;
    DevBuf<uint64_t> key[2];
    int cur_key = 0;
    DevBuf<int32_t> obs_offset, obs_slot, obs_idx, lm_id, lm_anchor, lm_used, result;
    DevBuf<ctvio::FactorDesc> desc;
    int n_entries = 0;
    uint32_t held = 0;
    int n_lm = -1;
    int n_obs = 0;
    bool window_current = false;
    int32_t oldest_slot = 0;
    ctvio::MapHeader* h_map_head = nullptr;
    ctvio::MapPoint* h_map_points = nullptr;
    ctvio::FeatureTablePtrs ptrs() { return ctvio::FeatureTablePtrs{id.p, anchor.p, mask.p, lm.p, rho.p, idx.p}; }
  } ft;
  struct MargWs {
    DevBuf<int32_t> pos_cam, pos_lm, prior_pos, marg_img, marg_imu;
    DevBuf<int2> bij;
    DevBuf<double> eig_scratch, Jrow, bs, A, b, Amm, V, ev, Vs, Ainv, T, Ap, bp, Ap2, V2, ev2, vb, J, r;
  } mws;

  void* nccl_comm = nullptr;
  int rank = 0, world = 1;
  bool shard_checked = false;

  int64_t launches = 0;

  ProblemDims dims() const {
    ProblemDims d;
    d.nK = nK; d.nB = nB; d.nL = nL;
    d.idx_bias0 = 6 * nK;
    d.idx_ld = 6 * nK + 6 * nB;
    d.np = d.idx_ld + 1;
    return d;
  }
  NormalEqPtrs ne(int b) {
    double* s = ne_slab[b].p;
    return NormalEqPtrs{s, s + off_gc, s + off_hl, s + off_gl, s + off_wld, s + off_W, &d_scal.p->cost_eval};
  }
  LandmarkLayout lml() { return LandmarkLayout{d_lo.p, d_hi.p, d_woff.p}; }
};

namespace ctvio::host {

struct ArenaScope {
  PinnedArena* prev;
  explicit ArenaScope(ctvio_engine* e) : prev(g_arena) {
    if (e->stream && cudaStreamQuery(e->stream) == cudaSuccess) e->arena.rewind();
    else cudaGetLastError();
    g_arena = &e->arena;
  }
  ~ArenaScope() { g_arena = prev; }
};

inline int ensure_table(ctvio_engine* e) {
  if (!e->table_valid) {
    e->launches += launch_knot_table(e->x[e->cur].ptrs(), e->nK, e->stream);
    e->table_valid = true;
  }
  return CTVIO_OK;
}

int prepare(ctvio_engine* e);
void evaluate(ctvio_engine* e, int xb, int nb, bool full, bool reset_cost = true);
int read_scalars(ctvio_engine* e, bool published = false);
LinearLaunch linear_launch(ctvio_engine* e, int nb);
int refresh_mirror(ctvio_engine* e);
int alloc_state(ctvio_engine* e, DevState& s);

}
```

ctrl-vio_b200/csrc/kernels.h:

```cpp
#pragma once
#include <cuda_runtime.h>

#include <atomic>

#include <cstdint>
#include <utility>

#include "spline_eval.cuh"

namespace ctvio {

constexpr int kPStride = 4;
constexpr int kVisThreads = 256;
constexpr int kVisObsPerRound = 128;
constexpr int kVisMinChunk = 64;
constexpr int kLocalDim = 64;
constexpr int kRowStride = 66;
constexpr int kObsStride = 2 * kRowStride + 2;
constexpr int kWinKnots = 5;
constexpr int kColLd = 60, kColR = 61, kColRho = 62;
constexpr int kCholNB = 64;

struct StatePtrs {
  double* q;
  double* p;
  double* bias;
  double* rho;
  double* ld;
  KnotPair* tab;
};

struct NormalEqPtrs {
  double* A;
  double* gc;
  double* hl;
  double* gl;
  double* wld;
  double* W;
  double* cost;
};

struct ImageObsPtrs {
  const longlong2* t;
  const double2* pi;
  const double2* pj;
  const int4* meta;
  int32_t n;
};

struct VisualItem {
  int32_t start, count;
  int32_t wi0, wj0;
};

struct ImuObsPtrs {
  const longlong2* t_node;
  const double2* ga;
  int32_t n;
};

struct ImuItem {
  int32_t start, count;
  int32_t s, node;
};
constexpr int kImuMaxPerItem = 32;

struct BiasFactorPtrs {
  const int2* ij;
  const double* sqrt_info;
  int32_t n;
};

struct PriorPtrs {
  int32_t n, n_blocks;
  const double* J;
  const double* r;
  const double* JtJ;
  const int32_t* type;
  const int32_t* index;
  const int32_t* col;
  const double* x0;
  const int32_t* col2g;
  double* dx;
  double* res;
};

struct ProblemDims {
  int32_t nK, nB, nL, np, idx_bias0, idx_ld;
};

struct LandmarkLayout {
  const int32_t* lo;
  const int32_t* hi;
  const int64_t* woff;
};

struct SchurEntry {
  int32_t l, lo, hi, pad;
  int64_t woff;
};
struct SchurTileItem {
  int32_t ti, tj;
  int32_t first, count;
};

struct LmScalars {
  double cost_eval;
  double gd;
  double dHd;
  double step_norm2;
  double x_norm2;
  double err_sum;
  double gmax;
  double dir_max;
  double ld_value;
  int32_t chol_fail;
  int32_t error_flags;
  int32_t pad[2];
};
struct LmDecision {
  double radius_next;
  double model_cost_change;
  double rho;
  int32_t valid;
  int32_t accept;
  int32_t go;
  int32_t pad;
};
struct LmDecideArgs {
  LmDecision* dec;
  double x_cost, radius;
  double min_relative_decrease, max_radius;
  double parameter_tolerance, function_tolerance, gradient_tolerance, min_radius;
};
struct LmPublished {
  LmScalars s;
  LmDecision dec;
  unsigned long long seq;
  unsigned long long pad;
};
constexpr int kLmSumScalars = 6;

struct PerDeviceOnce {
  std::atomic<unsigned long long> mask{0};
  bool first() {
    int d = 0;
    cudaGetDevice(&d);
    const unsigned long long bit = 1ull << (d & 63);
    return !(mask.fetch_or(bit) & bit);
  }
};
inline int device_sm_count() {
  static std::atomic<int> cache[64];
  int d = 0;
  cudaGetDevice(&d);
  int v = cache[d & 63].load(std::memory_order_relaxed);
  if (v == 0) {
    cudaDeviceGetAttribute(&v, cudaDevAttrMultiProcessorCount, d);
    cache[d & 63].store(v, std::memory_order_relaxed);
  }
  return v;
}

#if defined(__CUDACC__)
__device__ __forceinline__ void det_ticket_wait(const int* ticket, int my) {
  if (!ticket) return;
  if (threadIdx.x == 0) {
    int v;
    do { asm volatile("ld.acquire.gpu.global.s32 %0, [%1];" : "=r"(v) : "l"(ticket) : "memory"); } while (v != my);
  }
  __syncthreads();
}
__device__ __forceinline__ void det_ticket_done(int* ticket, int my) {
  if (!ticket) return;
  __threadfence();
  __syncthreads();
  if (threadIdx.x == 0) asm volatile("st.release.gpu.global.s32 [%0], %1;" ::"l"(ticket), "r"(my + 1) : "memory");
}
__device__ __forceinline__ void pdl_wait() { asm volatile("griddepcontrol.wait;" ::: "memory"); }
__device__ __forceinline__ void pdl_launch_dependents() { asm volatile("griddepcontrol.launch_dependents;" ::: "memory"); }
#endif

#if defined(__CUDACC__)
template <typename... KArgs, typename... Args>
cudaError_t launch_chained(bool pdl, void (*kernel)(KArgs...), dim3 grid, dim3 block, size_t smem, cudaStream_t s,
                           Args&&... args) {
  cudaLaunchConfig_t cfg = {};
  cfg.gridDim = grid;
  cfg.blockDim = block;
  cfg.dynamicSmemBytes = smem;
  cfg.stream = s;
  cudaLaunchAttribute at[1];
  at[0].id = cudaLaunchAttributeProgrammaticStreamSerialization;
  at[0].val.programmaticStreamSerializationAllowed = 1;
  cfg.attrs = at;
  cfg.numAttrs = pdl ? 1 : 0;
  return cudaLaunchKernelEx(&cfg, kernel, std::forward<Args>(args)...);
}
#endif

int launch_knot_table(const StatePtrs& st, int nK, cudaStream_t s);

struct VisualLaunch {
  ImageObsPtrs obs;
  const VisualItem* items;
  int32_t n_items;
  StatePtrs st;
  NormalEqPtrs ne;
  LandmarkLayout lm;
  ProblemDims dims;
  SplineParams sp;
  RigParams rig;
  double cauchy;
  const uint8_t* cmask;
  LmScalars* scal;
  int* det_ticket = nullptr;
};
int launch_visual(const VisualLaunch& a, bool full, cudaStream_t s);
size_t visual_smem_bytes();

struct ImuLaunch {
  ImuObsPtrs obs;
  const ImuItem* items;
  int32_t n_items;
  StatePtrs st;
  NormalEqPtrs ne;
  ProblemDims dims;
  SplineParams sp;
  RigParams rig;
  const uint8_t* cmask;
  LmScalars* scal;
  int* det_ticket = nullptr;
};
int launch_imu(const ImuLaunch& a, bool full, cudaStream_t s);

struct SmallFactorsLaunch {
  BiasFactorPtrs bf;
  PriorPtrs prior;
  StatePtrs st;
  NormalEqPtrs ne;
  ProblemDims dims;
  const uint8_t* cmask;
  LmScalars* scal;
  int deterministic = 0;
};
int launch_small_factors(const SmallFactorsLaunch& a, bool full, cudaStream_t s);

int launch_probe_image(const VisualLaunch& a, const int32_t* orig_index, bool want_jac, double* r, int32_t* s,
                       double* J, cudaStream_t st);
int launch_probe_imu(const ImuLaunch& a, const int32_t* orig_index, bool want_jac, double* r, int32_t* s, double* J,
                     cudaStream_t st);

struct LinearLaunch {
  ProblemDims dims;
  NormalEqPtrs ne;
  LandmarkLayout lm;
  const SchurEntry* schur_list;
  const SchurTileItem* schur_items;
  int32_t n_schur_items;
  double* lis;
  double* lc;
  const uint8_t* cmask;
  const uint8_t* active;
  double* sc;
  double* sl;
  double* M;
  double* Linv;
  double* rhs;
  double* y;
  double* yf;
  double* chol_part;
  int32_t* chol_flags;
  unsigned* chol_seq;
  double* hh;
  double* diagA;
  int32_t sharded;
  double* dc;
  double* dl;
  int32_t npad;
  LmScalars* scal;
  int* det_ticket;
  const int32_t* go;
  int32_t pdl = 0;
};
int launch_jacobi_scale(const LinearLaunch& a, cudaStream_t s);
int launch_lm_step(const LinearLaunch& a, double radius, cudaStream_t s);
int launch_reduced_system(const LinearLaunch& a, double radius, cudaStream_t s, const double* radius_dev = nullptr);
int launch_factor_solve(const LinearLaunch& a, cudaStream_t s);
bool chol_dag_supported(int npad, int n_sm);
size_t chol_dag_part_len(int npad);
size_t chol_dag_flags_len(int npad);
size_t chol_dag_lpub_len(int npad);
int launch_chol_dag_init(double* linv_buf, double* part_buf, int npad, cudaStream_t s);
int launch_chol_dag(const LinearLaunch& a, cudaStream_t s);
int launch_chol_coop(const LinearLaunch& a, cudaStream_t s);
int launch_step_vectors(const LinearLaunch& a, cudaStream_t s);
int launch_extract_diag(const LinearLaunch& a, cudaStream_t s);
int launch_jacobi_scale_from_diag(const LinearLaunch& a, cudaStream_t s);
int launch_gradient_norm(const LinearLaunch& a, const StatePtrs& st, int fix_ld, double ld_lower, double ld_upper,
                         cudaStream_t s, bool reset = true, LmPublished* pub = nullptr, unsigned long long seq = 0,
                         const LmDecideArgs* decide = nullptr);

struct ApplyLaunch {
  int32_t count_camera;
  ProblemDims dims;
  StatePtrs x, xc;
  const double* dc;
  const double* dl;
  double alpha;
  const uint8_t* active;
  int32_t clamp_ld;
  double ld_lower, ld_upper;
  LmScalars* scal;
  int* det_ticket = nullptr;
};
int launch_apply_step(const ApplyLaunch& a, cudaStream_t s, bool reset = true);
int launch_step_and_apply(const LinearLaunch& a, const ApplyLaunch& ap, cudaStream_t s);
int launch_gauge_realign(const StatePtrs& st, int nK, int min_idx, const double* R0_t0_dev, cudaStream_t s);

struct QueryLaunch {
  StatePtrs st;
  SplineParams sp;
  int32_t n;
  const int64_t* t;
  double *q, *p, *omega, *vel, *acc;
  LmScalars* scal;
};
int launch_query(const QueryLaunch& a, cudaStream_t s);

}
```

ctrl-vio_b200/csrc/kernels_linear.cu:

```cuda
#include <algorithm>

#include "dmma_tiles.cuh"
#include <cstddef>

#include "kernels.h"

namespace ctvio {

__device__ __forceinline__ double warp_sum_d(double v) {
#pragma unroll
  for (int o = 16; o > 0; o >>= 1) v += __shfl_xor_sync(0xffffffffu, v, o);
  return v;
}
__device__ __forceinline__ double warp_max_d(double v) {
#pragma unroll
  for (int o = 16; o > 0; o >>= 1) v = fmax(v, __shfl_xor_sync(0xffffffffu, v, o));
  return v;
}
__device__ __forceinline__ void atomic_max_pos(double* addr, double v) {
  atomicMax(reinterpret_cast<unsigned long long*>(addr), static_cast<unsigned long long>(__double_as_longlong(v)));
}

constexpr double kMinLmDiag = 1e-6, kMaxLmDiag = 1e32;

// ... 179 lines not shown
  for (int j = j0 + threadIdx.x; j < np; j += blockDim.x) dsh[j - j0] = a.cmask[j] ? 0.0 : -a.sc[j] * a.y[j];
  __syncthreads();
  if (i < np) {
    const double di = dsh[i - j0];
    if (lane == 0) {
      a.dc[i] = di;
      gd = a.ne.gc[i] * di;
      dmax = fabs(di);
      if (!isfinite(di)) a.scal->chol_fail = 1;
    }
    if (di != 0.0) {
      double s = 0;
      for (int j = i + lane; j < np; j += 32) s = fma(a.ne.A[size_t(i) * np + j] * (j == i ? 0.5 : 1.0), dsh[j - j0], s);
      dHd = 2.0 * di * s;
    }
  }
  dHd = warp_sum_d(dHd);
  if (lane == 0) { red[0][threadIdx.x >> 5] = gd; red[1][threadIdx.x >> 5] = dHd; red[2][threadIdx.x >> 5] = dmax; }
  __syncthreads();
  det_ticket_wait(a.det_ticket ? a.det_ticket + 1 : nullptr, blockIdx.x);
  if (threadIdx.x == 0) {
    double g = 0, h = 0, m = 0;
    for (int w = 0; w < 8; ++w) { g += red[0][w]; h += red[1][w]; m = fmax(m, red[2][w]); }
    atomicAdd(&a.scal->gd, g);
    atomicAdd(&a.scal->dHd, h);
    atomic_max_pos(&a.scal->dir_max, m);
  }
  det_ticket_done(a.det_ticket ? a.det_ticket + 1 : nullptr, blockIdx.x);
}

__device__ __forceinline__ void landmark_step_block(const LinearLaunch& a, int block, const ApplyLaunch* ap = nullptr) {
  __shared__ double red[3][8];
  __shared__ double red2[2][8];
  double xn = 0, sn = 0;
  const int lane = threadIdx.x & 31, warp = threadIdx.x >> 5;
  const int l = block * 8 + warp;
  double gd = 0, dHd = 0, dmax = 0;
  if (l < a.dims.nL) {
    const double sl = a.sl[l];
    const int lo = a.lm.lo[l], hi = a.lm.hi[l], ild = a.dims.idx_ld;
    const double* Wl = a.ne.W + a.lm.woff[l] - lo;
    double wy = 0;
    for (int g = lo + lane; g < hi; g += 32) wy = fma(Wl[g], a.cmask[g] ? 0.0 : a.sc[g] * a.y[g], wy);
    wy = warp_sum_d(wy);
    if (lane == 0) {
      wy = fma(a.ne.wld[l], a.cmask[ild] ? 0.0 : a.sc[ild] * a.y[ild], wy);
      const double hh = a.hh[l];
      const double yl = hh > 0.0 ? (sl * a.ne.gl[l] - sl * wy) / hh : 0.0;
      const double d = -sl * yl;
      a.dl[l] = d;
      gd = a.ne.gl[l] * d;
      dHd = 2.0 * d * (-wy) + a.ne.hl[l] * d * d;
      dmax = fabs(d);
      if (!isfinite(d)) a.scal->chol_fail = 1;
      if (ap) {
        const double v = ap->x.rho[l], vn = v + d;
        ap->xc.rho[l] = vn;
        if (ap->active[a.dims.np + l]) { xn = v * v; sn = (v - vn) * (v - vn); }
      }
    }
  }
  if (lane == 0) { red[0][warp] = gd; red[1][warp] = dHd; red[2][warp] = dmax; red2[0][warp] = xn; red2[1][warp] = sn; }
  __syncthreads();
  det_ticket_wait(a.det_ticket ? a.det_ticket + 1 : nullptr, blockIdx.x);
  if (threadIdx.x == 0) {
    double g = 0, h = 0, m = 0, x = 0, s = 0;
    for (int w = 0; w < 8; ++w) { g += red[0][w]; h += red[1][w]; m = fmax(m, red[2][w]); x += red2[0][w]; s += red2[1][w]; }
    if (g != 0.0) atomicAdd(&a.scal->gd, g);
    if (h != 0.0) atomicAdd(&a.scal->dHd, h);
    if (m > 0.0) atomic_max_pos(&a.scal->dir_max, m);
    if (x != 0.0) atomicAdd(&a.scal->x_norm2, x);
    if (s != 0.0) atomicAdd(&a.scal->step_norm2, s);
  }
  det_ticket_done(a.det_ticket ? a.det_ticket + 1 : nullptr, blockIdx.x);
}

__global__ void __launch_bounds__(256) step_vectors_kernel(LinearLaunch a, int ncb) {
  extern __shared__ double step_dsh[];
  if (int(blockIdx.x) < ncb) camera_step_block(a, blockIdx.x, step_dsh);
  else landmark_step_block(a, blockIdx.x - ncb, nullptr);
}

__global__ void extract_diag_kernel(LinearLaunch a) {
  const int i = blockIdx.x * blockDim.x + threadIdx.x;
  if (i >= a.npad) return;
  a.diagA[i] = i < a.dims.np ? a.ne.A[size_t(i) * a.dims.np + i] : 0.0;
}
int launch_extract_diag(const LinearLaunch& a, cudaStream_t s) {
  extract_diag_kernel<<<(a.npad + 255) / 256, 256, 0, s>>>(a);
  return 1;
}
__global__ void jacobi_scale_from_diag_kernel(LinearLaunch a) {
  const int i = blockIdx.x * blockDim.x + threadIdx.x;
  if (i < a.dims.np) a.sc[i] = 1.0 / (1.0 + sqrt(a.diagA[i]));
  if (i < a.dims.nL) a.sl[i] = 1.0 / (1.0 + sqrt(a.ne.hl[i]));
}
int launch_jacobi_scale_from_diag(const LinearLaunch& a, cudaStream_t s) {
  const int n = max(a.dims.np, a.dims.nL);
  jacobi_scale_from_diag_kernel<<<(n + 255) / 256, 256, 0, s>>>(a);
  return 1;
}

int launch_reduced_system(const LinearLaunch& a, double radius, cudaStream_t s, const double* radius_dev) {
  int launches = 0;
  const size_t total = std::max(size_t(a.npad) * a.npad, size_t(a.dims.nL));
  launch_chained(a.pdl, scale_copy_kernel, dim3(unsigned((total + 255) / 256)), dim3(256), 0, s, a, radius, radius_dev);
  ++launches;
  if (a.n_schur_items > 0) {
    launch_chained(a.pdl, schur_tile_kernel, dim3(a.n_schur_items), dim3(256), 0, s, a);
    ++launches;
  }
  return launches;
}

int launch_step_vectors(const LinearLaunch& a, cudaStream_t s) {
  const int ncb = (a.dims.np + 7) / 8, nlb = (a.dims.nL + 7) / 8;
  step_vectors_kernel<<<ncb + nlb, 256, size_t(a.dims.np) * sizeof(double), s>>>(a, ncb);
  return 1;
}

int launch_lm_step(const LinearLaunch& a, double radius, cudaStream_t s) {
  return launch_reduced_system(a, radius, s) + launch_factor_solve(a, s) + launch_step_vectors(a, s);
}

__global__ void __launch_bounds__(1024) gradient_norm_kernel(LinearLaunch a, StatePtrs st, int fix_ld, double ld_lower,
                                                             double ld_upper, LmPublished* pub, unsigned long long seq,
                                                             LmDecideArgs da) {
  __shared__ double red[32];
  pdl_wait();
  pdl_launch_dependents();
  const int np = a.dims.np, nL = a.dims.nL;
  double v = 0.0;
  for (int i = blockIdx.x * blockDim.x + threadIdx.x; i < np + nL; i += gridDim.x * blockDim.x) {
    if (!a.active[i]) continue;
    double x;
    if (i < np) {
      x = fabs(a.ne.gc[i]);
      if (i == a.dims.idx_ld && !fix_ld) {
        const double ld = *st.ld;
        x = fabs(ld - fmin(fmax(ld - a.ne.gc[i], ld_lower), ld_upper));
      }
    } else {
      x = fabs(a.ne.gl[i - np]);
    }
    v = fmax(v, x);
  }
  v = warp_max_d(v);
  if ((threadIdx.x & 31) == 0) red[threadIdx.x >> 5] = v;
  __syncthreads();
  if (threadIdx.x < 32) {
    v = warp_max_d(red[threadIdx.x]);
    if (threadIdx.x == 0) {
      bool last = true;
      if (gridDim.x > 1) {
        atomicMax(reinterpret_cast<unsigned long long*>(&a.scal->gmax), static_cast<unsigned long long>(__double_as_longlong(v)));
        __threadfence();
        last = atomicAdd(&a.scal->pad[0], 1) == int(gridDim.x) - 1;
        if (last) a.scal->pad[0] = 0;
      } else {
        a.scal->gmax = fmax(a.scal->gmax, v);
      }
      if (last && pub) {
        static_assert(sizeof(LmScalars) == 88, "scalar block is copied as five 16-byte words + one 8-byte word");
        __threadfence();
        const uint4* src = reinterpret_cast<const uint4*>(a.scal);
        uint4 w[5];
#pragma unroll
        for (int k = 0; k < 5; ++k) w[k] = __ldcg(src + k);
        const uint2 w5 = __ldcg(reinterpret_cast<const uint2*>(src + 5));
        uint4* dst = reinterpret_cast<uint4*>(&pub->s);
#pragma unroll
        for (int k = 0; k < 5; ++k) dst[k] = w[k];
        *reinterpret_cast<uint2*>(dst + 5) = w5;
        if (da.dec) {
          LmScalars sc;
          uint4* loc = reinterpret_cast<uint4*>(&sc);
#pragma unroll
          for (int k = 0; k < 5; ++k) loc[k] = w[k];
          *reinterpret_cast<uint2*>(loc + 5) = w5;
          LmDecision d;
          d.model_cost_change = __dsub_rn(-sc.gd, __dmul_rn(0.5, sc.dHd));
          d.valid = (!sc.chol_fail && isfinite(d.model_cost_change) && d.model_cost_change > 0.0) ? 1 : 0;
          d.rho = __ddiv_rn(__dsub_rn(da.x_cost, sc.cost_eval), d.model_cost_change);
          d.accept = (d.valid && d.rho > da.min_relative_decrease) ? 1 : 0;
          const double t = __dsub_rn(__dmul_rn(2.0, d.rho), 1.0);
          const double t3 = __dmul_rn(__dmul_rn(t, t), t);
          d.radius_next = fmin(da.max_radius, __ddiv_rn(da.radius, fmax(1.0 / 3.0, __dsub_rn(1.0, t3))));
          const double step_norm = sqrt(sc.step_norm2), x_norm = sqrt(sc.x_norm2);
          const bool stop = step_norm <= __dmul_rn(da.parameter_tolerance, __dadd_rn(x_norm, da.parameter_tolerance)) ||
                            fabs(__dsub_rn(da.x_cost, sc.cost_eval)) <= __dmul_rn(da.function_tolerance, da.x_cost) ||
                            fmax(sc.gmax, v) <= da.gradient_tolerance || d.radius_next < da.min_radius;
          d.go = (d.accept && !stop) ? 1 : 0;
          d.pad = 0;
          *da.dec = d;
          pub->dec = d;
        }
        __threadfence_system();
        *reinterpret_cast<volatile unsigned long long*>(&pub->seq) = seq;
      }
    }
  }
}
int launch_gradient_norm(const LinearLaunch& a, const StatePtrs& st, int fix_ld, double ld_lower, double ld_upper,
                         cudaStream_t s, bool reset, LmPublished* pub, unsigned long long seq, const LmDecideArgs* decide) {
  if (reset) cudaMemsetAsync(&a.scal->gmax, 0, sizeof(double), s);
  LmDecideArgs da{};
  if (decide) da = *decide;
  const int n = a.dims.np + a.dims.nL;
  const int grid = std::min(16, std::max(1, (n + 1023) / 1024));
  launch_chained(a.pdl, gradient_norm_kernel, dim3(grid), dim3(1024), 0, s, a, st, fix_ld, ld_lower, ld_upper, pub, seq, da);
  return 1;
}

struct StepSource {
  const double* dc;
  const double* y;
  const double* sc;
  const uint8_t* cmask;
  __device__ __forceinline__ double operator()(int g) const {
    if (dc) return dc[g];
    return cmask[g] ? 0.0 : -sc[g] * y[g];
  }
};

__device__ __forceinline__ Q4 stepped_knot(const ApplyLaunch& a, const StepSource& src, int i) {
  const double d0 = src(6 * i), d1 = src(6 * i + 1), d2 = src(6 * i + 2);
  const Q4 q = load_q(a.x.q, i);
  if (d0 != 0.0 || d1 != 0.0 || d2 != 0.0) return so3_mul(q, so3_exp(V3{a.alpha * d0, a.alpha * d1, a.alpha * d2}));
  return q;
}

__device__ __forceinline__ void apply_step_block(const ApplyLaunch& a, const StepSource& src, int block, bool with_landmarks) {
  __shared__ double red[2][8];
  const int i = block * blockDim.x + threadIdx.x;
  const int nK = a.dims.nK, nB = a.dims.nB, nL = with_landmarks ? a.dims.nL : 0;
  double xn = 0, sn = 0;
  if (i < nK) {
    const Q4 q = load_q(a.x.q, i);
    const Q4 qn = stepped_knot(a, src, i);
    a.xc.q[4 * i] = qn.x; a.xc.q[4 * i + 1] = qn.y; a.xc.q[4 * i + 2] = qn.z; a.xc.q[4 * i + 3] = qn.w;
    if (i + 1 < nK) {
      const Q4 qm = stepped_knot(a, src, i + 1);
      const double q2[8] = {qn.x, qn.y, qn.z, qn.w, qm.x, qm.y, qm.z, qm.w};
      KnotPair kp;
      make_knot_pair(q2, 0, kp);
      a.xc.tab[i] = kp;
    }
    if (a.count_camera && a.active[6 * i]) {
      xn += q.x * q.x + q.y * q.y + q.z * q.z + q.w * q.w;
      sn += (q.x - qn.x) * (q.x - qn.x) + (q.y - qn.y) * (q.y - qn.y) + (q.z - qn.z) * (q.z - qn.z) + (q.w - qn.w) * (q.w - qn.w);
    }
#pragma unroll
    for (int c = 0; c < 3; ++c) {
      const double p = a.x.p[kPStride * i + c];
      const double pn = p + a.alpha * src(6 * i + 3 + c);
      a.xc.p[kPStride * i + c] = pn;
      if (a.count_camera && a.active[6 * i + 3 + c]) { xn += p * p; sn += (p - pn) * (p - pn); }
    }
    a.xc.p[kPStride * i + 3] = 0.0;
  } else if (i < nK + 6 * nB) {
    const int b = i - nK;
    const double v = a.x.bias[b];
    const double vn = v + a.alpha * src(a.dims.idx_bias0 + b);
    a.xc.bias[b] = vn;
    if (a.count_camera && a.active[a.dims.idx_bias0 + b]) { xn += v * v; sn += (v - vn) * (v - vn); }
  } else if (i == nK + 6 * nB) {
    const double v = *a.x.ld;
    double vn = v + a.alpha * src(a.dims.idx_ld);
    if (a.clamp_ld) vn = fmin(fmax(vn, a.ld_lower), a.ld_upper);
    *a.xc.ld = vn;
    a.scal->ld_value = vn;
    if (a.count_camera && a.active[a.dims.idx_ld]) { xn += v * v; sn += (v - vn) * (v - vn); }
  } else if (i < nK + 6 * nB + 1 + nL) {
    const int l = i - (nK + 6 * nB + 1);
    const double v = a.x.rho[l];
    const double vn = v + a.alpha * a.dl[l];
    a.xc.rho[l] = vn;
    if (a.active[a.dims.np + l]) { xn += v * v; sn += (v - vn) * (v - vn); }
  }
  xn = warp_sum_d(xn); sn = warp_sum_d(sn);
  if ((threadIdx.x & 31) == 0) { red[0][threadIdx.x >> 5] = xn; red[1][threadIdx.x >> 5] = sn; }
  __syncthreads();
  det_ticket_wait(a.det_ticket ? a.det_ticket + 1 : nullptr, blockIdx.x);
  if (threadIdx.x == 0) {
    double x = 0, s = 0;
    for (int w = 0; w < 8; ++w) { x += red[0][w]; s += red[1][w]; }
    if (x != 0.0) atomicAdd(&a.scal->x_norm2, x);
    if (s != 0.0) atomicAdd(&a.scal->step_norm2, s);
  }
  det_ticket_done(a.det_ticket ? a.det_ticket + 1 : nullptr, blockIdx.x);
}

__global__ void __launch_bounds__(256) apply_step_kernel(ApplyLaunch a) {
  apply_step_block(a, StepSource{a.dc, nullptr, nullptr, nullptr}, blockIdx.x, true);
}

int launch_apply_step(const ApplyLaunch& a, cudaStream_t s, bool reset) {
  const int n = a.dims.nK + 6 * a.dims.nB + 1 + a.dims.nL;
  if (reset) cudaMemsetAsync(&a.scal->step_norm2, 0, 2 * sizeof(double), s);
  apply_step_kernel<<<(n + 255) / 256, 256, 0, s>>>(a);
  return 1;
}

__global__ void __launch_bounds__(256) step_apply_kernel(LinearLaunch a, ApplyLaunch ap, int ncb, int nlb) {
  extern __shared__ double step_dsh[];
  const int b = blockIdx.x;
  pdl_wait();
  pdl_launch_dependents();
  if (b < ncb) camera_step_block(a, b, step_dsh);
  else if (b < ncb + nlb) landmark_step_block(a, b - ncb, &ap);
  else apply_step_block(ap, StepSource{nullptr, a.y, a.sc, a.cmask}, b - ncb - nlb, false);
}

int launch_step_and_apply(const LinearLaunch& a, const ApplyLaunch& ap, cudaStream_t s) {
  const int ncb = (a.dims.np + 7) / 8, nlb = (a.dims.nL + 7) / 8;
  const int nab = (a.dims.nK + 6 * a.dims.nB + 1 + 255) / 256;
  launch_chained(a.pdl, step_apply_kernel, dim3(ncb + nlb + nab), dim3(256), size_t(a.dims.np) * sizeof(double), s, a, ap,
                 ncb, nlb);
  return 1;
}

__device__ void r2ypr_deg(const M3& R, double ypr[3]) {
  const double nx = R.m[0], ny = R.m[3], nz = R.m[6];
  const double ox = R.m[1], oy = R.m[4];
  const double ax = R.m[2], ay = R.m[5];
  const double y = atan2(ny, nx);
  const double p = atan2(-nz, nx * cos(y) + ny * sin(y));
  const double r = atan2(ax * sin(y) - ay * cos(y), -ox * sin(y) + oy * cos(y));
  const double k = 180.0 / 3.14159265358979323846;
  ypr[0] = y * k; ypr[1] = p * k; ypr[2] = r * k;
}

__global__ void gauge_realign_kernel(StatePtrs st, int nK, int min_idx, const double* R0t0) {
  __shared__ double T[16];
  if (threadIdx.x == 0) {
    M3 R0;
    for (int e = 0; e < 9; ++e) R0.m[e] = R0t0[e];
    const V3 t0 = V3{R0t0[9], R0t0[10], R0t0[11]};
    const M3 R00 = so3_matrix(load_q(st.q, min_idx));
    const V3 t00 = load_p<kPStride>(st.p, min_idx);
    double e0[3], e00[3];
    r2ypr_deg(R0, e0);
    r2ypr_deg(R00, e00);
    const double y = (e0[0] - e00[0]) / 180.0 * 3.14159265358979323846;
    M3 rd = m3_identity();
    rd.m[0] = cos(y); rd.m[1] = -sin(y); rd.m[3] = sin(y); rd.m[4] = cos(y);
    if (fabs(fabs(e0[1]) - 90.0) < 1.0 || fabs(fabs(e00[1]) - 90.0) < 1.0) rd = m3_mul_bt(R0, R00);
    const V3 td = t0 - m3_vec(rd, t00);
    const Q4 qd = quat_from_matrix(rd);
    T[0] = qd.x; T[1] = qd.y; T[2] = qd.z; T[3] = qd.w; T[4] = td.x; T[5] = td.y; T[6] = td.z;
  }
  __syncthreads();
  const Q4 qd = Q4{T[0], T[1], T[2], T[3]};
  const V3 td = V3{T[4], T[5], T[6]};
  for (int i = min_idx + threadIdx.x; i < nK; i += blockDim.x) {
    const Q4 qn = so3_mul(qd, load_q(st.q, i));
    const V3 pn = so3_rotate(qd, load_p<kPStride>(st.p, i)) + td;
    st.q[4 * i] = qn.x; st.q[4 * i + 1] = qn.y; st.q[4 * i + 2] = qn.z; st.q[4 * i + 3] = qn.w;
    st.p[kPStride * i] = pn.x; st.p[kPStride * i + 1] = pn.y; st.p[kPStride * i + 2] = pn.z;
  }
}

int launch_gauge_realign(const StatePtrs& st, int nK, int min_idx, const double* R0_t0_dev, cudaStream_t s) {
  gauge_realign_kernel<<<1, 256, 0, s>>>(st, nK, min_idx, R0_t0_dev);
  return 1 + launch_knot_table(st, nK, s);
}

}
```

ctrl-vio_b200/csrc/kernels_residual.cu:

```cuda
#include <cstdio>

#include "kernels.h"

namespace ctvio {


__device__ __forceinline__ uint32_t smem_u32(const void* p) { return static_cast<uint32_t>(__cvta_generic_to_shared(p)); }

__device__ __forceinline__ void mbar_init(uint64_t* bar, uint32_t count) {
  asm volatile("mbarrier.init.shared::cta.b64 [%0], %1;" ::"r"(smem_u32(bar)), "r"(count) : "memory");
}
__device__ __forceinline__ void fence_mbar_init() { asm volatile("fence.mbarrier_init.release.cluster;" ::: "memory"); }
__device__ __forceinline__ void mbar_expect_tx(uint64_t* bar, uint32_t bytes) {
  asm volatile("mbarrier.arrive.expect_tx.shared::cta.b64 _, [%0], %1;" ::"r"(smem_u32(bar)), "r"(bytes) : "memory");
}
__device__ __forceinline__ void tma_bulk_g2s(void* dst, const void* src, uint32_t bytes, uint64_t* bar) {
  asm volatile("cp.async.bulk.shared::cluster.global.mbarrier::complete_tx::bytes [%0], [%1], %2, [%3];" ::"r"(
                   smem_u32(dst)),
               "l"(src), "r"(bytes), "r"(smem_u32(bar))
               : "memory");
}
__device__ __forceinline__ bool mbar_try_wait(uint64_t* bar, uint32_t phase) {
  uint32_t ok;
  asm volatile(
      "{\n"
      ".reg .pred p;\n"
      "mbarrier.try_wait.parity.shared::cta.b64 p, [%1], %2;\n"
      "selp.u32 %0, 1, 0, p;\n"
      "}\n"
      : "=r"(ok)
      : "r"(smem_u32(bar)), "r"(phase)
      : "memory");
  return ok != 0;
}

__device__ __forceinline__ double warp_sum(double v) {
#pragma unroll
  for (int o = 16; o > 0; o >>= 1) v += __shfl_xor_sync(0xffffffffu, v, o);
  return v;
}


__global__ void knot_table_kernel(StatePtrs st, int nK) {
  const int k = blockIdx.x * blockDim.x + threadIdx.x;
  if (k >= nK - 1) return;
  KnotPair kp;
  make_knot_pair(st.q, k, kp);
  st.tab[k] = kp;
}

int launch_knot_table(const StatePtrs& st, int nK, cudaStream_t s) {
  if (nK < 2) return 0;
  knot_table_kernel<<<(nK - 1 + 127) / 128, 128, 0, s>>>(st, nK);
  return 1;
}


struct VisArgs {
  ImageObsPtrs obs;
  const VisualItem* items;
  StatePtrs st;
  NormalEqPtrs ne;
  LandmarkLayout lm;
  ProblemDims dims;
  SplineParams sp;
  RigParams rig;
  double cauchy;
  const uint8_t* cmask;
  LmScalars* scal;
  int* det_ticket;
};

struct __align__(128) VisStatic {
  KnotPair tab[2][4];
  double q[2][kWinKnots][4];
  double p[2][kWinKnots][4];
  double cost_part[8];
  unsigned long long bar;
  int err;
};

__constant__ uint8_t c_tile_i[36] = {0, 0, 0, 0, 0, 0, 0, 0, 1, 1, 1, 1, 1, 1, 1, 2, 2, 2,
                                     2, 2, 2, 3, 3, 3, 3, 3, 4, 4, 4, 4, 5, 5, 5, 6, 6, 7};
__constant__ uint8_t c_tile_j[36] = {0, 1, 2, 3, 4, 5, 6, 7, 1, 2, 3, 4, 5, 6, 7, 2, 3, 4,
                                     5, 6, 7, 3, 4, 5, 6, 7, 4, 5, 6, 7, 5, 6, 7, 6, 7, 7};

#ifdef CTVIO_CHOL_TIMING
__device__ long long g_vis_clk[8];
__device__ long long g_imu_clk[8];
#define VCLK(i) do { if (blockIdx.x == 0 && threadIdx.x == 0) g_vis_clk[(i)] = clock64(); } while (0)
#define ICLK(i) do { if (blockIdx.x == 0 && threadIdx.x == 0) g_imu_clk[(i)] = clock64(); } while (0)
extern "C" int ctvio_debug_vis_clk(long long* out) {
  return cudaMemcpyFromSymbol(out, g_vis_clk, sizeof(g_vis_clk)) == cudaSuccess ? 0 : -1;
}
extern "C" int ctvio_debug_imu_clk(long long* out) {
  return cudaMemcpyFromSymbol(out, g_imu_clk, sizeof(g_imu_clk)) == cudaSuccess ? 0 : -1;
}
#else
#define VCLK(i)
#define ICLK(i)
#endif

size_t visual_smem_bytes() {
  return size_t(kVisObsPerRound) * kObsStride * sizeof(double) + size_t(36) * 64 * sizeof(double);
}

template <bool DIAG>
__device__ __noinline__ void syrk_round_warp(const double* Jt, double* accs, int nround, int warp, int lane) {
  constexpr int NB = DIAG ? 2 : 1;
  const int g = lane >> 2, q = lane & 3;
  int bi[NB], bj[NB];
  if constexpr (DIAG) {
    bi[0] = bj[0] = 2 * (warp - 6);
    bi[1] = bj[1] = 2 * (warp - 6) + 1;
  } else {
    bi[0] = warp < 3 ? 0 : (warp < 5 ? 1 : 2);
    bj[0] = warp < 3 ? warp + 1 : (warp < 5 ? warp - 1 : 3);
  }
  double acc[NB][2][2][2];
#pragma unroll
  for (int b = 0; b < NB; ++b)
#pragma unroll
    for (int mi = 0; mi < 2; ++mi)
#pragma unroll
      for (int nj = 0; nj < 2; ++nj) {
        if (DIAG && mi == 1 && nj == 0) continue;
        const int ti = 2 * bi[b] + mi, tj = 2 * bj[b] + nj;
        const double2 v = *reinterpret_cast<const double2*>(accs + (ti * 8 - ti * (ti - 1) / 2 + (tj - ti)) * 64 + g * 8 + 2 * q);
        acc[b][mi][nj][0] = v.x; acc[b][mi][nj][1] = v.y;
      }
  const int nsteps = (2 * nround + 3) >> 2;
#pragma unroll 2
  for (int st = 0; st < nsteps; ++st) {
    const int row = 4 * st + q;
    const double* rp = Jt + size_t(row >> 1) * kObsStride + (row & 1) * kRowStride + g;
#pragma unroll
    for (int b = 0; b < NB; ++b) {
      double av[2], bv[2];
#pragma unroll
      for (int m = 0; m < 2; ++m) {
        av[m] = rp[16 * bi[b] + 8 * m];
        bv[m] = DIAG ? av[m] : rp[16 * bj[b] + 8 * m];
      }
#pragma unroll
      for (int mi = 0; mi < 2; ++mi)
#pragma unroll
        for (int nj = 0; nj < 2; ++nj) {
          if (DIAG && mi == 1 && nj == 0) continue;
          asm volatile("mma.sync.aligned.m8n8k4.row.col.f64.f64.f64.f64 {%0,%1}, {%2}, {%3}, {%0,%1};"
                       : "+d"(acc[b][mi][nj][0]), "+d"(acc[b][mi][nj][1])
                       : "d"(av[mi]), "d"(bv[nj]));
        }
    }
  }
#pragma unroll
  for (int b = 0; b < NB; ++b)
#pragma unroll
    for (int mi = 0; mi < 2; ++mi)
#pragma unroll
      for (int nj = 0; nj < 2; ++nj) {
        if (DIAG && mi == 1 && nj == 0) continue;
        const int ti = 2 * bi[b] + mi, tj = 2 * bj[b] + nj;
        *reinterpret_cast<double2*>(accs + (ti * 8 - ti * (ti - 1) / 2 + (tj - ti)) * 64 + g * 8 + 2 * q) =
            make_double2(acc[b][mi][nj][0], acc[b][mi][nj][1]);
      }
}

__device__ __forceinline__ void syrk_round(const double* Jt, double* accs, int nround, int tid) {
  const int warp = tid >> 5, lane = tid & 31;
  if (warp < 6) syrk_round_warp<false>(Jt, accs, nround, warp, lane);
  else syrk_round_warp<true>(Jt, accs, nround, warp, lane);
  __syncthreads();
}

template <bool FULL>
__global__ void __launch_bounds__(kVisThreads, 1) visual_kernel(const __grid_constant__ VisArgs a) {
  extern __shared__ __align__(128) unsigned char dyn_smem[];
  double* Jt = reinterpret_cast<double*>(dyn_smem);
  double* accs = Jt + size_t(kVisObsPerRound) * kObsStride;
  __shared__ VisStatic sm;

  const int tid = threadIdx.x;
  const int lane = tid & 31, warp = tid >> 5;
  const VisualItem item = a.items[blockIdx.x];
  const int nK = a.dims.nK;
  VCLK(0);

  const int w0[2] = {item.wi0, item.wj0};
  if (tid == 0) {
    sm.err = 0;
    mbar_init(reinterpret_cast<uint64_t*>(&sm.bar), 1);
    fence_mbar_init();
  }
  __syncthreads();
  if (tid == 0) {
    uint32_t bytes = 0;
#pragma unroll
    for (int sd = 0; sd < 2; ++sd) {
      const int nk = min(kWinKnots, nK - w0[sd]);
      const int npair = min(4, nK - 1 - w0[sd]);
      bytes += uint32_t(nk) * 64u + uint32_t(npair) * uint32_t(sizeof(KnotPair));
    }
    mbar_expect_tx(reinterpret_cast<uint64_t*>(&sm.bar), bytes);
#pragma unroll
    for (int sd = 0; sd < 2; ++sd) {
      const int nk = min(kWinKnots, nK - w0[sd]);
      const int npair = min(4, nK - 1 - w0[sd]);
      tma_bulk_g2s(&sm.q[sd][0][0], a.st.q + 4 * w0[sd], uint32_t(nk) * 32u, reinterpret_cast<uint64_t*>(&sm.bar));
      tma_bulk_g2s(&sm.p[sd][0][0], a.st.p + 4 * w0[sd], uint32_t(nk) * 32u, reinterpret_cast<uint64_t*>(&sm.bar));
      tma_bulk_g2s(&sm.tab[sd][0], a.st.tab + w0[sd], uint32_t(npair) * uint32_t(sizeof(KnotPair)),
                   reinterpret_cast<uint64_t*>(&sm.bar));
    }
  }
  if (FULL)
    for (int i = tid; i < 36 * 64; i += kVisThreads) accs[i] = 0.0;
  while (!mbar_try_wait(reinterpret_cast<uint64_t*>(&sm.bar), 0)) {
  }
  __syncthreads();

  const double ld = *a.st.ld;
  const int64_t ld_ns = int64_t(ld * 1e9);
  const int side = tid & 1;
  double cost_local = 0.0;
  VCLK(1);

  for (int base = 0; base < item.count; base += kVisObsPerRound) {
    const int nround = min(kVisObsPerRound, item.count - base);
    const int ol = tid >> 1;
    const bool active = ol < nround;
    double* row0 = Jt + size_t(ol) * kObsStride;
    double* row1 = row0 + kRowStride;
    bool valid = false;
    const unsigned m_act = __ballot_sync(0xffffffffu, active);
    if (active) {
      const int oi = item.start + base + ol;
      const longlong2 tt = a.obs.t[oi];
      const double2 pi = a.obs.pi[oi];
      const double2 pj = a.obs.pj[oi];
      const int4 meta = a.obs.meta[oi];
      const double rho = a.st.rho[meta.z];
      const int64_t w_base = FULL ? a.lm.woff[meta.z] - a.lm.lo[meta.z] : 0;
      const int64_t t_eval = side == 0 ? tt.x + int64_t(meta.x) * ld_ns : tt.y + int64_t(meta.y) * ld_ns;
      int32_t s;
      double u;
      bool ok = spline_index(a.sp, t_eval, s, u);
      const int slot = s - w0[side];
      ok = ok && (slot == 0 || slot == 1);
      const bool ok_both = __shfl_xor_sync(m_act, ok ? 1 : 0, 1) && ok;
      const unsigned m_ok = __ballot_sync(m_act, ok_both);
      valid = ok_both;
      if (!ok_both) {
        atomicOr(&sm.err, 1);
      } else {
        PoseStage ev;
        pose_stage<FULL, kPStride>(a.sp, &sm.q[side][0][0], &sm.p[side][0][0], sm.tab[side], slot, u, ev);
        M3 Ro;
        V3 po, omo, vo;
#pragma unroll
        for (int e = 0; e < 9; ++e) Ro.m[e] = __shfl_xor_sync(m_ok, ev.R.m[e], 1);
        po = V3{__shfl_xor_sync(m_ok, ev.p.x, 1), __shfl_xor_sync(m_ok, ev.p.y, 1), __shfl_xor_sync(m_ok, ev.p.z, 1)};
        if (FULL) {
          omo = V3{__shfl_xor_sync(m_ok, ev.omega.x, 1), __shfl_xor_sync(m_ok, ev.omega.y, 1),
                   __shfl_xor_sync(m_ok, ev.omega.z, 1)};
          vo = V3{__shfl_xor_sync(m_ok, ev.vel.x, 1), __shfl_xor_sync(m_ok, ev.vel.y, 1),
                  __shfl_xor_sync(m_ok, ev.vel.z, 1)};
        }
        const M3& R_i = side == 0 ? ev.R : Ro;
        const M3& R_j = side == 0 ? Ro : ev.R;
        const V3 p_i = side == 0 ? ev.p : po;
        const V3 p_j = side == 0 ? po : ev.p;
        ImageCommon cm;
        const double pixy[2] = {pi.x, pi.y}, pjxy[2] = {pj.x, pj.y};
        image_common(a.rig, pixy, pjxy, rho, R_i, p_i, R_j, p_j, a.cauchy, cm);
        if (side == 0) cost_local += cm.cost;
        if (FULL) {
          double jrho[2], lhs[6];
          image_jrho(a.rig, cm, R_i, rho, jrho);
          image_side_lhs(side, cm, ev.R, lhs);
          const int cb = side * 30;
          const int gk0 = w0[side];
          const int l = meta.z;
          double* Wl = a.ne.W + w_base;
          {
            const int unused = cb + (slot == 0 ? 4 : 0) * 6;
#pragma unroll
            for (int c = 0; c < 6; ++c) { row0[unused + c] = 0.0; row1[unused + c] = 0.0; }
          }
          const double sgn = side == 0 ? 1.0 : -1.0;
          jacobian_stage(sm.tab[side], ev, [&](int k, const M3& Jk) {
            double rk[6];
            mul23_33(lhs, Jk, rk);
            const int gd = 6 * (gk0 + slot + k);
            const int col = cb + (slot + k) * 6;
            const double ck = sgn * ev.c[k];
#pragma unroll
            for (int c = 0; c < 3; ++c) {
              const bool mr = a.cmask[gd + c] != 0, mp = a.cmask[gd + 3 + c] != 0;
              const double r0v = mr ? 0.0 : rk[c], r1v = mr ? 0.0 : rk[3 + c];
              const double p0v = mp ? 0.0 : ck * cm.JvR[c], p1v = mp ? 0.0 : ck * cm.JvR[3 + c];
              row0[col + c] = r0v; row1[col + c] = r1v;
              row0[col + 3 + c] = p0v; row1[col + 3 + c] = p1v;
              if (!a.det_ticket) {
                if (!mr) atomicAdd(Wl + gd + c, r0v * jrho[0] + r1v * jrho[1]);
                if (!mp) atomicAdd(Wl + gd + 3 + c, p0v * jrho[0] + p1v * jrho[1]);
              }
            }
          });
          if (side == 0) {
            row0[kColR] = cm.r[0]; row1[kColR] = cm.r[1];
            row0[kColRho] = jrho[0]; row1[kColRho] = jrho[1];
          } else {
            double jld[2];
            image_jld(a.rig, cm, meta.x, meta.y, R_i, omo, vo, R_j, ev.omega, ev.vel, jld);
            const bool ld_const = a.cmask[a.dims.idx_ld] != 0;
            row0[kColLd] = ld_const ? 0.0 : jld[0];
            row1[kColLd] = ld_const ? 0.0 : jld[1];
            row0[63] = 0.0; row1[63] = 0.0;
          }
          if (!a.det_ticket) {
            if (side == 0) {
              atomicAdd(a.ne.hl + l, jrho[0] * jrho[0] + jrho[1] * jrho[1]);
              atomicAdd(a.ne.gl + l, jrho[0] * cm.r[0] + jrho[1] * cm.r[1]);
            } else {
              atomicAdd(a.ne.wld + l, row0[kColLd] * jrho[0] + row1[kColLd] * jrho[1]);
            }
          }
        }
      }
    }
    if (FULL) {
      if (!valid && ol < kVisObsPerRound) {
        const int cb = side * 30;
        for (int c = 0; c < 30; ++c) { row0[cb + c] = 0.0; row1[cb + c] = 0.0; }
        if (side == 0) { row0[kColR] = row1[kColR] = 0.0; row0[kColRho] = row1[kColRho] = 0.0; }
        else { row0[kColLd] = row1[kColLd] = 0.0; row0[63] = row1[63] = 0.0; }
      }
      VCLK(2);
      __syncthreads();
      VCLK(3);
      if (a.det_ticket) {
        det_ticket_wait(a.det_ticket, blockIdx.x * 1024 + base / kVisObsPerRound);
        if (active && valid) {
          const int oi = item.start + base + ol;
          const int l = a.obs.meta[oi].z;
          const double j0 = row0[kColRho], j1 = row1[kColRho];
          if (side == 0) {
            atomicAdd(a.ne.hl + l, j0 * j0 + j1 * j1);
            atomicAdd(a.ne.gl + l, j0 * row0[kColR] + j1 * row1[kColR]);
          } else {
            atomicAdd(a.ne.wld + l, row0[kColLd] * j0 + row1[kColLd] * j1);
          }
        }
        for (int ph = 0; ph < 2; ++ph) {
          if (active && valid && side == ph) {
            const int oi = item.start + base + ol;
            const int l = a.obs.meta[oi].z;
            const double j0 = row0[kColRho], j1 = row1[kColRho];
            double* Wl = a.ne.W + (a.lm.woff[l] - a.lm.lo[l]);
            const int cb = side * 30, gk0 = w0[side];
            for (int c = 0; c < 30; ++c) {
              const double v = row0[cb + c] * j0 + row1[cb + c] * j1;
              if (v != 0.0) atomicAdd(Wl + 6 * gk0 + c, v);
            }
          }
          __threadfence();
          __syncthreads();
        }
        det_ticket_done(a.det_ticket, blockIdx.x * 1024 + base / kVisObsPerRound);
      }
      syrk_round(Jt, accs, nround, tid);
      VCLK(4);
    }
  }

  const int n_rounds = (item.count + kVisObsPerRound - 1) / kVisObsPerRound;
  det_ticket_wait(a.det_ticket, blockIdx.x * 1024 + (FULL ? n_rounds : 0));
  cost_local = warp_sum(cost_local);
  if (lane == 0) sm.cost_part[warp] = cost_local;
  __syncthreads();
  if (tid == 0) {
    double c = 0;
#pragma unroll
    for (int w = 0; w < kVisThreads / 32; ++w) c += sm.cost_part[w];
    atomicAdd(a.ne.cost, c);
    if (sm.err) atomicOr(&a.scal->error_flags, 1);
  }
  if (FULL) {
    const int np = a.dims.np;
    const int n_class = a.det_ticket ? 11 : 1;
    for (int cls = 0; cls < n_class; ++cls) {
      for (int idx = tid; idx < 36 * 64; idx += kVisThreads) {
        const double val = accs[idx];
        if (val == 0.0) continue;
        const int tile = idx >> 6, e = idx & 63;
        const int la = c_tile_i[tile] * 8 + (e >> 3), lb = c_tile_j[tile] * 8 + (e & 7);
        if (la > lb || lb > kColR || la >= kColR) continue;
        const int sa = la < 30 ? 0 : (la < 60 ? 1 : 2);
        const int ga = sa == 0 ? 6 * item.wi0 + la : (sa == 1 ? 6 * item.wj0 + (la - 30) : a.dims.idx_ld);
        if (lb == kColR) {
          if (n_class > 1 && cls != 8 + sa) continue;
          atomicAdd(a.ne.gc + ga, val);
          continue;
        }
        const int sb = lb < 30 ? 0 : (lb < 60 ? 1 : 2);
        const int gb = sb == 0 ? 6 * item.wi0 + lb : (sb == 1 ? 6 * item.wj0 + (lb - 30) : a.dims.idx_ld);
        if (n_class > 1) {
          int c;
          if (sb == 2) c = 5 + sa;
          else if (sa == sb) c = sa == 0 ? 0 : 4;
          else c = ga < gb ? 1 : (ga > gb ? 2 : 3);
          if (c != cls) continue;
        }
        const double v = (la != lb && ga == gb) ? 2.0 * val : val;
        const int g0 = min(ga, gb), g1 = max(ga, gb);
        atomicAdd(a.ne.A + size_t(g0) * np + g1, v);
      }
      if (n_class > 1) {
        __threadfence();
        __syncthreads();
      }
    }
  }
  if (a.det_ticket) {
    __threadfence();
    __syncthreads();
    if (tid == 0) asm volatile("st.release.gpu.global.s32 [%0], %1;" ::"l"(a.det_ticket), "r"((int(blockIdx.x) + 1) * 1024) : "memory");
  }
  VCLK(5);
}

int launch_visual(const VisualLaunch& l, bool full, cudaStream_t s) {
  if (l.n_items <= 0) return 0;
  VisArgs a{l.obs, l.items, l.st, l.ne, l.lm, l.dims, l.sp, l.rig, l.cauchy, l.cmask, l.scal, l.det_ticket};
  static PerDeviceOnce once;
  if (once.first()) {
    cudaFuncSetAttribute(visual_kernel<true>, cudaFuncAttributeMaxDynamicSharedMemorySize, int(visual_smem_bytes()));
    cudaFuncSetAttribute(visual_kernel<false>, cudaFuncAttributeMaxDynamicSharedMemorySize, int(visual_smem_bytes()));
  }
  if (full) visual_kernel<true><<<l.n_items, kVisThreads, visual_smem_bytes(), s>>>(a);
  else visual_kernel<false><<<l.n_items, kVisThreads, 0, s>>>(a);
  return 1;
}


struct ImuArgs {
  ImuObsPtrs obs;
  const ImuItem* items;
  StatePtrs st;
  NormalEqPtrs ne;
  ProblemDims dims;
  SplineParams sp;
  RigParams rig;
  const uint8_t* cmask;
  LmScalars* scal;
  int* det_ticket;
};

constexpr int kImuThreads = 128;
constexpr int kImuCols = 32;
constexpr int kImuColStride = 196;
static_assert(kImuColStride >= 6 * kImuMaxPerItem && kImuColStride % 16 == 4, "K2 shared column stride");

__host__ __device__ constexpr int imu_tile(int w, int t) {
  return w == 0 ? (t == 0 ? 0 : t == 1 ? 1 : 5)
       : w == 1 ? (t == 0 ? 10 : t == 1 ? 11 : 15)
       : w == 2 ? (t == 0 ? 2 : 3)
                : (t == 0 ? 6 : 7);
}
__host__ __device__ constexpr int imu_ntiles(int w) { return w < 2 ? 3 : 2; }
__host__ __device__ constexpr bool imu_uses(int w, int c) {
  bool u = false;
  for (int t = 0; t < imu_ntiles(w); ++t) u = u || imu_tile(w, t) >> 2 == c || (imu_tile(w, t) & 3) == c;
  return u;
}

__device__ __forceinline__ void imu_zero_part(double* J, int warp) {
  const int r0 = 3 * (warp >> 1), c0 = 12 * (warp & 1), c1 = (warp & 1) ? kImuCols : 12;
  for (int c = c0; c < c1; ++c)
#pragma unroll
    for (int r = 0; r < 3; ++r) J[c * kImuColStride + r0 + r] = 0.0;
}

template <bool ACCEL, int H>
__device__ __forceinline__ void imu_write_part(const ImuArgs& a, const ImuStage& st, int s, int node, double* J) {
  constexpr int r0 = ACCEL ? 3 : 0;
  imu_jacobian_half<ACCEL, H>(a.rig, a.st.tab, s, st, [&](int k, const double rot[9], const double pos[9]) {
#pragma unroll
    for (int c = 0; c < 3; ++c) {
      const bool mr = a.cmask[6 * (s + k) + c] != 0, mp = a.cmask[6 * (s + k) + 3 + c] != 0;
#pragma unroll
      for (int r = 0; r < 3; ++r) {
        J[(k * 6 + c) * kImuColStride + r0 + r] = mr ? 0.0 : rot[3 * r + c];
        J[(k * 6 + 3 + c) * kImuColStride + r0 + r] = mp ? 0.0 : pos[3 * r + c];
      }
    }
  });
  if (H == 1) {
    const int gb0 = a.dims.idx_bias0 + 6 * node;
#pragma unroll
    for (int c = 0; c < 6; ++c) {
      const bool mb = a.cmask[gb0 + c] != 0;
#pragma unroll
      for (int r = 0; r < 3; ++r) J[(24 + c) * kImuColStride + r0 + r] = (c == r0 + r && !mb) ? a.rig.imu_info[r0 + r] : 0.0;
    }
#pragma unroll
    for (int r = 0; r < 3; ++r) {
      J[30 * kImuColStride + r0 + r] = st.r[r0 + r];
      J[31 * kImuColStride + r0 + r] = 0.0;
    }
  }
}

template <int W>
__device__ __forceinline__ void imu_syrk(const double* Js, int nsteps, int lane, double acc[3][2]) {
  const double* rp = Js + (lane >> 2) * kImuColStride + (lane & 3);
#pragma unroll
  for (int t = 0; t < 3; ++t) acc[t][0] = acc[t][1] = 0.0;
#pragma unroll 4
  for (int st = 0; st < nsteps; ++st, rp += 4) {
    double v[4];
#pragma unroll
    for (int c = 0; c < 4; ++c) v[c] = imu_uses(W, c) ? rp[8 * c * kImuColStride] : 0.0;
#pragma unroll
    for (int t = 0; t < imu_ntiles(W); ++t)
      asm volatile("mma.sync.aligned.m8n8k4.row.col.f64.f64.f64.f64 {%0,%1}, {%2}, {%3}, {%0,%1};"
                   : "+d"(acc[t][0]), "+d"(acc[t][1])
                   : "d"(v[imu_tile(W, t) >> 2]), "d"(v[imu_tile(W, t) & 3]));
  }
}

template <int W>
__device__ __forceinline__ void imu_flush(const ImuArgs& a, const ImuItem& item, int lane, const double acc[3][2]) {
  const int np = a.dims.np;
#pragma unroll
  for (int t = 0; t < imu_ntiles(W); ++t)
#pragma unroll
    for (int e = 0; e < 2; ++e) {
      const double val = acc[t][e];
      const int la = 8 * (imu_tile(W, t) >> 2) + (lane >> 2), lb = 8 * (imu_tile(W, t) & 3) + 2 * (lane & 3) + e;
      if (val == 0.0 || la > lb || lb > 30 || la >= 30) continue;
      const int ga = la < 24 ? 6 * item.s + la : a.dims.idx_bias0 + 6 * item.node + (la - 24);
      if (lb == 30) {
        atomicAdd(a.ne.gc + ga, val);
        continue;
      }
      const int gb = lb < 24 ? 6 * item.s + lb : a.dims.idx_bias0 + 6 * item.node + (lb - 24);
      atomicAdd(a.ne.A + size_t(ga) * np + gb, val);
    }
}

template <bool FULL>
__global__ void __launch_bounds__(kImuThreads) imu_kernel(const __grid_constant__ ImuArgs a) {
  extern __shared__ __align__(128) unsigned char dyn_smem[];
  double* Js = reinterpret_cast<double*>(dyn_smem);
  const int tid = threadIdx.x, warp = tid >> 5, lane = tid & 31;
  const ImuItem item = a.items[blockIdx.x];
  double cost = 0.0;
  ICLK(0);
  if ((FULL || warp == 0) && lane < item.count) {
    const int n = item.start + lane;
    const longlong2 tn = a.obs.t_node[n];
    const double2 g0 = a.obs.ga[3 * n], g1 = a.obs.ga[3 * n + 1], g2 = a.obs.ga[3 * n + 2];
    const double gyro[3] = {g0.x, g0.y, g1.x}, accel[3] = {g1.y, g2.x, g2.y};
    const int node = item.node;
    double bias[6];
#pragma unroll
    for (int c = 0; c < 6; ++c) bias[c] = a.st.bias[6 * node + c];
    int32_t s;
    double u;
    const bool ok = spline_index(a.sp, tn.x, s, u) && s == item.s;
    double* J = Js + 6 * lane;
    if (!ok) {
      if (warp == 0) atomicOr(&a.scal->error_flags, 1);
      if (FULL) imu_zero_part(J, warp);
    } else {
      ImuStage st;
      imu_stage<kPStride>(a.sp, a.rig, a.st.q, a.st.p, a.st.tab, s, u, gyro, accel, bias, st);
      cost = st.cost;
      if (FULL) {
        switch (warp) {
          case 0: imu_write_part<false, 0>(a, st, s, node, J); break;
          case 1: imu_write_part<false, 1>(a, st, s, node, J); break;
          case 2: imu_write_part<true, 0>(a, st, s, node, J); break;
          default: imu_write_part<true, 1>(a, st, s, node, J); break;
        }
      }
    }
  } else if (FULL && lane == item.count) {
    imu_zero_part(Js + 6 * lane, warp);
  }
  if (FULL) {
    ICLK(1);
    __syncthreads();
    ICLK(2);
    const int nsteps = (6 * item.count + 3) >> 2;
    double acc[3][2];
    switch (warp) {
      case 0: imu_syrk<0>(Js, nsteps, lane, acc); break;
      case 1: imu_syrk<1>(Js, nsteps, lane, acc); break;
      case 2: imu_syrk<2>(Js, nsteps, lane, acc); break;
      default: imu_syrk<3>(Js, nsteps, lane, acc); break;
    }
    ICLK(3);
    ICLK(4);
    det_ticket_wait(a.det_ticket, blockIdx.x);
    switch (warp) {
      case 0: imu_flush<0>(a, item, lane, acc); break;
      case 1: imu_flush<1>(a, item, lane, acc); break;
      case 2: imu_flush<2>(a, item, lane, acc); break;
      default: imu_flush<3>(a, item, lane, acc); break;
    }
    ICLK(5);
  }
  if (!FULL) det_ticket_wait(a.det_ticket, blockIdx.x);
  if (warp == 0) {
    cost = warp_sum(cost);
    if (lane == 0 && cost != 0.0) atomicAdd(a.ne.cost, cost);
  }
  det_ticket_done(a.det_ticket, blockIdx.x);
}

int launch_imu(const ImuLaunch& l, bool full, cudaStream_t s) {
  if (l.n_items <= 0) return 0;
  ImuArgs a{l.obs, l.items, l.st, l.ne, l.dims, l.sp, l.rig, l.cmask, l.scal, l.det_ticket};
  const size_t smem = size_t(kImuCols) * kImuColStride * sizeof(double);
  static PerDeviceOnce once;
  if (once.first()) cudaFuncSetAttribute(imu_kernel<true>, cudaFuncAttributeMaxDynamicSharedMemorySize, int(smem));
  if (full) imu_kernel<true><<<l.n_items, kImuThreads, smem, s>>>(a);
  else imu_kernel<false><<<l.n_items, kImuThreads, 0, s>>>(a);
  return 1;
}


struct SmallArgs {
  BiasFactorPtrs bf;
  PriorPtrs prior;
  StatePtrs st;
  NormalEqPtrs ne;
  ProblemDims dims;
  const uint8_t* cmask;
  LmScalars* scal;
  int deterministic;
};

__device__ __forceinline__ const double* block_data(const StatePtrs& st, int type, int index) {
  switch (type) {
    case 0: return st.q + 4 * index;
    case 1: return st.p + kPStride * index;
    case 2: return st.bias + 6 * index;
    case 3: return st.bias + 6 * index + 3;
    case 4: return st.ld;
    default: return st.rho + index;
  }
}

template <bool FULL>
__global__ void __launch_bounds__(256) small_factors_kernel(const __grid_constant__ SmallArgs a) {
  __shared__ double red[8];
  const int tid = threadIdx.x;
  double cost = 0.0;
  const int np = a.dims.np;
  for (int n = a.deterministic ? (tid == 0 ? 0 : a.bf.n) : tid; n < a.bf.n; n += a.deterministic ? 1 : blockDim.x) {
    const int2 ij = a.bf.ij[n];
#pragma unroll
    for (int k = 0; k < 6; ++k) {
      const double s = a.bf.sqrt_info[6 * n + k];
      const double r = s * (a.st.bias[6 * ij.y + k] - a.st.bias[6 * ij.x + k]);
      cost += 0.5 * r * r;
      if (FULL) {
        const int gi = a.dims.idx_bias0 + 6 * ij.x + k, gj = a.dims.idx_bias0 + 6 * ij.y + k;
        const double ji = a.cmask[gi] ? 0.0 : -s, jj = a.cmask[gj] ? 0.0 : s;
        atomicAdd(a.ne.gc + gi, ji * r);
        atomicAdd(a.ne.gc + gj, jj * r);
        atomicAdd(a.ne.A + size_t(gi) * np + gi, ji * ji);
        atomicAdd(a.ne.A + size_t(gj) * np + gj, jj * jj);
        atomicAdd(a.ne.A + size_t(min(gi, gj)) * np + max(gi, gj), ji * jj);
      }
    }
  }
  const int n = a.prior.n;
  if (n > 0) {
    for (int b = tid; b < a.prior.n_blocks; b += blockDim.x) {
      const int type = a.prior.type[b];
      const double* x = block_data(a.st, type, a.prior.index[b]);
      const double* x0 = a.prior.x0 + 4 * b;
      double* dx = a.prior.dx + a.prior.col[b];
      if (type == 0) {
        const double n2 = x0[0] * x0[0] + x0[1] * x0[1] + x0[2] * x0[2] + x0[3] * x0[3];
        const double ax = -x0[0] / n2, ay = -x0[1] / n2, az = -x0[2] / n2, aw = x0[3] / n2;
        const double bx = x[0], by = x[1], bz = x[2], bw = x[3];
        const double qx = aw * bx + ax * bw + ay * bz - az * by;
        const double qy = aw * by + ay * bw + az * bx - ax * bz;
        const double qz = aw * bz + az * bw + ax * by - ay * bx;
        const double qw = aw * bw - ax * bx - ay * by - az * bz;
        const double sg = (qw >= 0) ? 2.0 : -2.0;
        dx[0] = sg * qx; dx[1] = sg * qy; dx[2] = sg * qz;
      } else {
        const int sz = (type == 4 || type == 5) ? 1 : 3;
        for (int d = 0; d < sz; ++d) dx[d] = x[d] - x0[d];
      }
    }
    __syncthreads();
    for (int i = tid; i < n; i += blockDim.x) {
      double s = a.prior.r[i];
      const double* Ji = a.prior.J + size_t(i) * n;
      for (int j = 0; j < n; ++j) s = fma(Ji[j], a.prior.dx[j], s);
      a.prior.res[i] = s;
      cost += 0.5 * s * s;
    }
    if (FULL) {
      __syncthreads();
      for (int j = tid; j < n; j += blockDim.x) {
        const int g = a.prior.col2g[j];
        if (g < 0) continue;
        double s = 0;
        for (int i = 0; i < n; ++i) s = fma(a.prior.J[size_t(i) * n + j], a.prior.res[i], s);
        atomicAdd(a.ne.gc + g, s);
      }
    }
  }
  cost = warp_sum(cost);
  if ((tid & 31) == 0) red[tid >> 5] = cost;
  __syncthreads();
  if (tid == 0) {
    double c = 0;
    for (int w = 0; w < 8; ++w) c += red[w];
    if (c != 0.0) atomicAdd(a.ne.cost, c);
  }
}

__global__ void prior_add_jtj_kernel(PriorPtrs pr, double* A, int np) {
  const int idx = blockIdx.x * blockDim.x + threadIdx.x;
  const int n = pr.n;
  if (idx >= n * n) return;
  const int i = idx / n, j = idx % n;
  if (j < i) return;
  const int gi = pr.col2g[i], gj = pr.col2g[j];
  if (gi < 0 || gj < 0) return;
  const double v = pr.JtJ[idx];
  if (v == 0.0) return;
  atomicAdd(A + size_t(min(gi, gj)) * np + max(gi, gj), v);
}

int launch_small_factors(const SmallFactorsLaunch& l, bool full, cudaStream_t s) {
  if (l.bf.n <= 0 && l.prior.n <= 0) return 0;
  SmallArgs a{l.bf, l.prior, l.st, l.ne, l.dims, l.cmask, l.scal, l.deterministic};
  int launches = 1;
  if (full) small_factors_kernel<true><<<1, 256, 0, s>>>(a);
  else small_factors_kernel<false><<<1, 256, 0, s>>>(a);
  if (full && l.prior.n > 0) {
    const int n2 = l.prior.n * l.prior.n;
    prior_add_jtj_kernel<<<(n2 + 255) / 256, 256, 0, s>>>(l.prior, l.ne.A, l.dims.np);
    ++launches;
  }
  return launches;
}


__global__ void probe_image_kernel(VisArgs a, const int32_t* orig_index, int want_jac, double* r, int32_t* sidx,
                                   double* J) {
  const int n = blockIdx.x * blockDim.x + threadIdx.x;
  if (n >= a.obs.n) return;
  const longlong2 tt = a.obs.t[n];
  const double2 pi = a.obs.pi[n], pj = a.obs.pj[n];
  const int4 meta = a.obs.meta[n];
  const double rho = a.st.rho[meta.z];
  const int64_t ld_ns = int64_t(*a.st.ld * 1e9);
  int32_t si, sj;
  double ui, uj;
  const int out = orig_index[n];
  if (!spline_index(a.sp, tt.x + int64_t(meta.x) * ld_ns, si, ui) ||
      !spline_index(a.sp, tt.y + int64_t(meta.y) * ld_ns, sj, uj)) {
    atomicOr(&a.scal->error_flags, 1);
    return;
  }
  SideEval ea, eb;
  if (want_jac) {
    eval_side<true, kPStride>(a.sp, a.st.q, a.st.p, a.st.tab, si, ui, ea);
    eval_side<true, kPStride>(a.sp, a.st.q, a.st.p, a.st.tab, sj, uj, eb);
  } else {
    eval_side<false, kPStride>(a.sp, a.st.q, a.st.p, a.st.tab, si, ui, ea);
    eval_side<false, kPStride>(a.sp, a.st.q, a.st.p, a.st.tab, sj, uj, eb);
  }
  ImageCommon cm;
  const double pixy[2] = {pi.x, pi.y}, pjxy[2] = {pj.x, pj.y};
  image_common(a.rig, pixy, pjxy, rho, ea.R, ea.p, eb.R, eb.p, a.cauchy, cm);
  atomicAdd(a.ne.cost, cm.cost);
  if (r) { r[2 * out] = cm.r[0]; r[2 * out + 1] = cm.r[1]; }
  if (sidx) { sidx[2 * out] = si; sidx[2 * out + 1] = sj; }
  if (!want_jac || !J) return;
  double* Jo = J + size_t(out) * 100;
  double rot[4][6], pos[4][6];
  image_side_blocks(0, cm, ea, rot, pos);
  for (int k = 0; k < 4; ++k)
    for (int e = 0; e < 6; ++e) { Jo[k * 12 + e] = rot[k][e]; Jo[k * 12 + 6 + e] = pos[k][e]; }
  image_side_blocks(1, cm, eb, rot, pos);
  for (int k = 0; k < 4; ++k)
    for (int e = 0; e < 6; ++e) { Jo[48 + k * 12 + e] = rot[k][e]; Jo[48 + k * 12 + 6 + e] = pos[k][e]; }
  image_jrho(a.rig, cm, ea.R, rho, Jo + 96);
  image_jld(a.rig, cm, meta.x, meta.y, ea.R, ea.omega, ea.vel, eb.R, eb.omega, eb.vel, Jo + 98);
}

int launch_probe_image(const VisualLaunch& l, const int32_t* orig_index, bool want_jac, double* r, int32_t* s,
                       double* J, cudaStream_t st) {
  if (l.obs.n <= 0) return 0;
  VisArgs a{l.obs, l.items, l.st, l.ne, l.lm, l.dims, l.sp, l.rig, l.cauchy, l.cmask, l.scal, nullptr};
  probe_image_kernel<<<(l.obs.n + 63) / 64, 64, 0, st>>>(a, orig_index, want_jac ? 1 : 0, r, s, J);
  return 1;
}

__global__ void probe_imu_kernel(ImuArgs a, const int32_t* orig_index, int want_jac, double* r, int32_t* sidx, double* J) {
  const int n = blockIdx.x * blockDim.x + threadIdx.x;
  if (n >= a.obs.n) return;
  const int out = orig_index[n];
  const longlong2 tn = a.obs.t_node[n];
  const double2 g0 = a.obs.ga[3 * n], g1 = a.obs.ga[3 * n + 1], g2 = a.obs.ga[3 * n + 2];
  const double gyro[3] = {g0.x, g0.y, g1.x}, accel[3] = {g1.y, g2.x, g2.y};
  const int node = int(tn.y);
  double bias[6];
  for (int c = 0; c < 6; ++c) bias[c] = a.st.bias[6 * node + c];
  int32_t s;
  double u;
  if (!spline_index(a.sp, tn.x, s, u)) {
    atomicOr(&a.scal->error_flags, 1);
    return;
  }
  ImuEvalOut o;
  if (want_jac) eval_imu<true, kPStride>(a.sp, a.rig, a.st.q, a.st.p, a.st.tab, s, u, gyro, accel, bias, o);
  else eval_imu<false, kPStride>(a.sp, a.rig, a.st.q, a.st.p, a.st.tab, s, u, gyro, accel, bias, o);
  atomicAdd(a.ne.cost, o.cost);
  if (r) for (int k = 0; k < 6; ++k) r[6 * out + k] = o.r[k];
  if (sidx) sidx[out] = s;
  if (!want_jac || !J) return;
  double* Jo = J + size_t(out) * 156;
  for (int k = 0; k < 4; ++k)
    for (int e = 0; e < 18; ++e) { Jo[k * 36 + e] = o.Jrot[k][e]; Jo[k * 36 + 18 + e] = o.Jpos[k][e]; }
  for (int k = 0; k < 3; ++k) {
    Jo[144 + k] = a.rig.imu_info[k]; Jo[147 + k] = 0; Jo[150 + k] = 0; Jo[153 + k] = a.rig.imu_info[3 + k];
  }
}

int launch_probe_imu(const ImuLaunch& l, const int32_t* orig_index, bool want_jac, double* r, int32_t* s, double* J,
                     cudaStream_t st) {
  if (l.obs.n <= 0) return 0;
  ImuArgs a{l.obs, l.items, l.st, l.ne, l.dims, l.sp, l.rig, l.cmask, l.scal, nullptr};
  probe_imu_kernel<<<(l.obs.n + 63) / 64, 64, 0, st>>>(a, orig_index, want_jac ? 1 : 0, r, s, J);
  return 1;
}


__global__ void query_kernel(QueryLaunch a) {
  const int n = blockIdx.x * blockDim.x + threadIdx.x;
  if (n >= a.n) return;
  int32_t s;
  double u;
  if (!spline_index(a.sp, a.t[n], s, u)) {
    atomicOr(&a.scal->error_flags, 1);
    return;
  }
  SideEval ev;
  eval_side<true, kPStride>(a.sp, a.st.q, a.st.p, a.st.tab, s, u, ev);
  if (a.q) {
    const Q4 q = quat_from_matrix(ev.R);
    a.q[4 * n] = q.x; a.q[4 * n + 1] = q.y; a.q[4 * n + 2] = q.z; a.q[4 * n + 3] = q.w;
  }
  if (a.p) { a.p[3 * n] = ev.p.x; a.p[3 * n + 1] = ev.p.y; a.p[3 * n + 2] = ev.p.z; }
  if (a.omega) { a.omega[3 * n] = ev.omega.x; a.omega[3 * n + 1] = ev.omega.y; a.omega[3 * n + 2] = ev.omega.z; }
  if (a.vel) { a.vel[3 * n] = ev.vel.x; a.vel[3 * n + 1] = ev.vel.y; a.vel[3 * n + 2] = ev.vel.z; }
  if (a.acc) {
    double c2[4];
    plain_coeffs<2>(u, a.sp.inv_dt, c2);
    V3 acc = c2[0] * load_p<kPStride>(a.st.p, s);
    for (int k = 1; k < 4; ++k) acc = acc + c2[k] * load_p<kPStride>(a.st.p, s + k);
    a.acc[3 * n] = acc.x; a.acc[3 * n + 1] = acc.y; a.acc[3 * n + 2] = acc.z;
  }
}

int launch_query(const QueryLaunch& a, cudaStream_t s) {
  if (a.n <= 0) return 0;
  query_kernel<<<(a.n + 127) / 128, 128, 0, s>>>(a);
  return 1;
}

}
```

ctrl-vio_b200/csrc/solve.cu:

```cuda
#include <cmath>
#include <cstdlib>

#include "engine_state.h"
#include "poly_min.h"

namespace {

int allreduce_scalars(ctvio_engine* e, bool publish = false) {
  if (e->world <= 1) return CTVIO_OK;
  CUDA_OK(e->d_shard_scal.reserve(8 + 8 * size_t(e->world)));
  e->launches += ctvio::launch_shard_scalars_pack(e->d_scal.p, e->d_shard_scal.p, e->stream);
  std::string err;
  if (!ctvio::comm_allgather(e->nccl_comm, e->d_shard_scal.p, e->d_shard_scal.p + 8, 8, e->stream, &err))
    return fail(CTVIO_ERR_NCCL, err);
  e->launches += ctvio::launch_shard_scalars_reduce(e->d_shard_scal.p + 8, e->world, e->d_scal.p, publish ? e->h_pub : nullptr,
                                                    publish ? ++e->pub_seq : 0, e->stream);
  return CTVIO_OK;
}

int shard_consensus(ctvio_engine* e, int local_rc) {
  if (e->world <= 1) return local_rc;
  const std::string local_msg = g_err;
  cudaStream_t st = e->stream;
  CUDA_OK(e->d_tmp.reserve(16));
  const double flag = local_rc ? 1.0 : 0.0;
  double total = 0.0;
  CUDA_OK(cudaMemcpyAsync(e->d_tmp.p, &flag, sizeof(double), cudaMemcpyHostToDevice, st));
  std::string err;
  if (!ctvio::comm_allreduce_sum(e->nccl_comm, e->d_tmp.p, 1, st, &err)) return fail(CTVIO_ERR_NCCL, err);
  CUDA_OK(cudaMemcpyAsync(&total, e->d_tmp.p, sizeof(double), cudaMemcpyDeviceToHost, st));
  CUDA_OK(cudaStreamSynchronize(st));
  if (local_rc) return fail(local_rc, local_msg);
  if (total != 0.0) return fail(CTVIO_ERR_STATE, "another rank of the sharded solve failed before the first collective");
  return CTVIO_OK;
}

int shard_check_ownership(ctvio_engine* e) {
  if (e->world <= 1 || e->shard_checked) return CTVIO_OK;
  cudaStream_t st = e->stream;
  std::vector<double> owned(size_t(std::max(e->nL, 1)), 0.0);
  for (const HostImage& o : e->img) owned[o.lm] = 1.0;
  CUDA_OK(e->d_rho_sync.reserve(2 * size_t(std::max(e->nL, 1))));
  CUDA_OK(cudaMemcpyAsync(e->d_rho_sync.p, owned.data(), owned.size() * sizeof(double), cudaMemcpyHostToDevice, st));
  std::string err;
  if (!ctvio::comm_allreduce_sum(e->nccl_comm, e->d_rho_sync.p, owned.size(), st, &err)) return fail(CTVIO_ERR_NCCL, err);
  CUDA_OK(cudaMemcpyAsync(owned.data(), e->d_rho_sync.p, owned.size() * sizeof(double), cudaMemcpyDeviceToHost, st));
  CUDA_OK(cudaStreamSynchronize(st));
  for (int l = 0; l < e->nL; ++l)
    if (owned[l] > 1.0)
      return fail(CTVIO_ERR_INVALID, "sharded solve: landmark " + std::to_string(l) + " has observations on " +
                                         std::to_string(int(owned[l])) + " ranks (shard image factors by landmark)");
  e->shard_checked = true;
  return CTVIO_OK;
}

int shard_sync_inv_depths(ctvio_engine* e) {
  if (e->world <= 1 || e->nL == 0) return CTVIO_OK;
  cudaStream_t st = e->stream;
  CUDA_OK(e->d_rho_sync.reserve(2 * size_t(e->nL)));
  std::vector<uint8_t> owned(e->nL, 0);
  for (const HostImage& o : e->img) owned[o.lm] = 1;
  CUDA_OK(e->d_owned.upload(owned, st));
  double* rho = e->x[e->cur].rho.p;
  e->launches += ctvio::launch_rho_pack(rho, e->d_owned.p, e->d_rho_sync.p, e->nL, st);
  std::string err;
  if (!ctvio::comm_allreduce_sum(e->nccl_comm, e->d_rho_sync.p, 2 * size_t(e->nL), st, &err)) return fail(CTVIO_ERR_NCCL, err);
  e->launches += ctvio::launch_rho_unpack(rho, e->d_rho_sync.p, e->nL, st);
  return CTVIO_OK;
}

ApplyLaunch apply_launch(ctvio_engine* e, int from, int to, double alpha) {
  ApplyLaunch ap;
  ap.dims = e->dims();
  ap.x = e->state(from).ptrs();
  ap.xc = e->state(to).ptrs();
  ap.dc = e->d_dc.p; ap.dl = e->d_dl.p;
  ap.alpha = alpha;
  ap.active = e->d_active.p;
  ap.count_camera = e->rank == 0 ? 1 : 0;
  ap.clamp_ld = e->opt.fix_ld ? 0 : 1;
  ap.ld_lower = e->opt.ld_lower; ap.ld_upper = e->opt.ld_upper;
  ap.scal = e->d_scal.p;
  ap.det_ticket = e->deterministic ? e->d_ticket.p : nullptr;
  return ap;
}

void gradient_norm(ctvio_engine* e, int xb, int nb, bool reset, bool publish, const LmDecideArgs* decide = nullptr) {
  LinearLaunch lin = linear_launch(e, nb);
  lin.pdl = decide ? 1 : 0;
  e->launches += launch_gradient_norm(lin, e->state(xb).ptrs(), e->opt.fix_ld, e->opt.ld_lower, e->opt.ld_upper, e->stream,
                                      reset, publish ? e->h_pub : nullptr, publish ? ++e->pub_seq : 0, decide);
}

int lm_step(ctvio_engine* e, int nb, double radius, const ApplyLaunch& ap, bool pdl, const double* radius_dev = nullptr,
            const int32_t* go = nullptr) {
  LinearLaunch lin = linear_launch(e, nb);
  lin.go = go;
  lin.pdl = pdl ? 1 : 0;
  cudaStream_t st = e->stream;
  if (e->deterministic) cudaMemsetAsync(e->d_ticket.p, 0, 2 * sizeof(int32_t), st);
  e->launches += launch_reduced_system(lin, radius, st, radius_dev);
  if (e->world > 1) {
    std::string err;
    const size_t count = ctvio::shard_pack_len(e->npad);
    CUDA_OK(e->d_shard_pack.reserve(count));
    e->launches += ctvio::launch_shard_pack(lin, e->d_shard_pack.p, st);
    if (!ctvio::comm_allreduce_sum(e->nccl_comm, e->d_shard_pack.p, count, st, &err)) return fail(CTVIO_ERR_NCCL, err);
    e->launches += ctvio::launch_shard_unpack(lin, e->d_shard_pack.p, radius, st);
  }
  e->launches += launch_factor_solve(lin, st);
  e->launches += launch_step_and_apply(lin, ap, st);
  return CTVIO_OK;
}

void prezero_slab(ctvio_engine* e, int nb) {
  cudaMemsetAsync(e->ne_slab[nb].p, 0, e->ne_slab_len * sizeof(double), e->stream2);
  cudaEventRecord(e->ev_zero, e->stream2);
  e->slab_zeroed[nb] = true;
}

int line_search(ctvio_engine* e, int cur, int cand, double x_cost, const LmScalars& sc, ctvio_summary& sum) {
  const double ls_sufficient_decrease = 1e-4, ls_max_contraction = 1e-3, ls_min_contraction = 0.6, ls_min_step = 1e-9;
  const int ls_max_iterations = 20;
  cudaStream_t st = e->stream;
  auto evaluate_at = [&](double alpha) {
    if (e->deterministic) cudaMemsetAsync(e->d_ticket.p, 0, 2 * sizeof(int32_t), st);
    e->launches += launch_apply_step(apply_launch(e, cur, cand, alpha), st);
    evaluate(e, cand, cand, true);
    sum.num_jacobian_evals++;
    gradient_norm(e, cand, cand, true, false);
    const int rc = allreduce_scalars(e);
    return rc ? rc : read_scalars(e);
  };
  const double g0 = sc.gd;
  struct Sample { double x, value, gradient; bool value_ok, grad_ok; };
  Sample initial{0.0, x_cost, g0, true, true}, previous{0, 0, 0, false, false};
  Sample current{1.0, sc.cost_eval, 0.0, std::isfinite(sc.cost_eval), false};
  bool have_grad = false;
  int ls_iters = 0;
  bool success = true;
  while (!current.value_ok || current.value > x_cost + ls_sufficient_decrease * g0 * current.x) {
    ++ls_iters;
    if (ls_iters >= ls_max_iterations) { success = false; break; }
    if (current.value_ok && !have_grad) {
      e->launches += ctvio::launch_dot_gradient(linear_launch(e, cand), st);
      int rc = allreduce_scalars(e);
      if (rc) return rc;
      rc = read_scalars(e);
      if (rc) return rc;
      current.gradient = e->h_scal->gd;
      current.grad_ok = std::isfinite(current.gradient);
    }
    const double smin = ls_max_contraction * current.x, smax = ls_min_contraction * current.x;
    double step;
    if (!current.value_ok) {
      step = std::min(std::max(current.x * 0.5, smin), smax);
    } else {
      std::vector<ctvio::PolySample> samples;
      samples.push_back({initial.x, initial.value, initial.gradient, true, true});
      samples.push_back({current.x, current.value, current.gradient, true, current.grad_ok});
      if (previous.value_ok) samples.push_back({previous.x, previous.value, previous.gradient, true, previous.grad_ok});
      step = ctvio::minimize_interpolating_polynomial(samples, smin, smax);
    }
    if (step * sc.dir_max < ls_min_step) { success = false; break; }
    previous = current;
    const int rc = evaluate_at(step);
    if (rc) return rc;
    current = Sample{step, e->h_scal->cost_eval, 0.0, std::isfinite(e->h_scal->cost_eval), false};
    have_grad = false;
  }
  sum.num_line_search_steps += ls_iters;
  if (!success && current.x != 1.0) return evaluate_at(1.0);
  return CTVIO_OK;
}

struct StepOutcome {
  bool valid = false;
  bool accept = false;
  double cost = 0, gmax = 0, step_norm2 = 0, x_norm2 = 0;
  double radius_next = 0;
};

}

extern "C" {

int ctvio_solve(ctvio_handle e, int32_t max_iterations, ctvio_summary* out) {
  if (!e) return fail(CTVIO_ERR_INVALID, "null handle");
  cudaSetDevice(e->cfg.device);
  int rc = prepare(e);
  rc = shard_consensus(e, rc);
  if (rc) return rc;
  rc = shard_check_ownership(e);
  if (rc) return rc;
  cudaStream_t st = e->stream;
  const ProblemDims d = e->dims();
  const double initial_radius = 1e4, max_radius = 1e16, min_radius = 1e-32, min_relative_decrease = 1e-3;
  const double function_tolerance = 1e-6, gradient_tolerance = 1e-10, parameter_tolerance = 1e-8;
  const int max_consecutive_invalid = 5;

  ctvio_summary sum;
  std::memset(&sum, 0, sizeof(sum));
  const int64_t launches0 = e->launches;
  cudaEventRecord(e->ev0, st);

  const bool is_constrained = !e->opt.fix_ld && (e->world > 1 || e->h_active[d.idx_ld]);
  if (is_constrained) {
    double ld;
    CUDA_OK(cudaMemcpyAsync(&ld, e->x[e->cur].ld.p, sizeof(double), cudaMemcpyDeviceToHost, st));
    CUDA_OK(cudaStreamSynchronize(st));
    const double c = std::min(std::max(ld, e->opt.ld_lower), e->opt.ld_upper);
    if (c != ld) CUDA_OK(cudaMemcpyAsync(e->x[e->cur].ld.p, &c, sizeof(double), cudaMemcpyHostToDevice, st));
  }
  ensure_table(e);
  const bool sharded = e->world > 1;
  int cur = e->cur;
  evaluate(e, cur, cur, true);
  sum.num_jacobian_evals++;
  LinearLaunch lin = linear_launch(e, cur);
  if (sharded) {
    e->launches += launch_extract_diag(lin, st);
    std::string err;
    if (!ctvio::comm_allreduce_sum(e->nccl_comm, lin.diagA, size_t(e->npad), st, &err)) return fail(CTVIO_ERR_NCCL, err);
    e->launches += launch_jacobi_scale_from_diag(lin, st);
  } else {
    e->launches += launch_jacobi_scale(lin, st);
  }
  gradient_norm(e, cur, cur, true, !sharded);
  if (sharded) {
    rc = allreduce_scalars(e);
    if (rc) return rc;
  }
  rc = read_scalars(e, !sharded);
  if (rc) return rc;
  double x_cost = e->h_scal->cost_eval;
  double gmax = e->h_scal->gmax;
  sum.initial_cost = x_cost;
  sum.num_successful_steps = 1;

  double radius = initial_radius, decrease_factor = 2.0;
  int num_invalid = 0;
  bool last_ok = true;
  int iter = 0;
  int term = CTVIO_TERM_NO_CONVERGENCE;

  bool spec_size_ok = e->img.size() <= 20000;
  if (const char* sp = std::getenv("CTVIO_SPECULATION")) {
    if (std::strcmp(sp, "always") == 0) spec_size_ok = true;
    if (std::strcmp(sp, "never") == 0) spec_size_ok = false;
  }
  const bool pipelined = spec_size_ok && !sharded && !is_constrained && !e->deterministic;
  if (pipelined) {
    rc = alloc_state(e, e->xs);
    if (rc) return rc;
  }
  int cur_ne = cur;
  bool spec_ready = false;
  bool spec_in_flight = false;
  int spec_out = -1;
  unsigned spec_chol_seq0 = e->chol_seq;
  while (true) {
    if (iter >= max_iterations) { term = CTVIO_TERM_NO_CONVERGENCE; break; }
    if (last_ok && gmax <= gradient_tolerance) { term = CTVIO_TERM_GRADIENT; break; }
    if (radius < min_radius) { term = CTVIO_TERM_MIN_RADIUS; break; }
    ++iter;
    const int cand_ne = cur_ne ^ 1;
    int cand;
    if (spec_ready) {
      cand = spec_out;
      prezero_slab(e, cand_ne);
    } else {
      cand = 0;
      while (cand == cur) ++cand;
      if (!spec_in_flight) prezero_slab(e, cand_ne);
      rc = lm_step(e, cur_ne, radius, apply_launch(e, cur, cand, 1.0), pipelined);
      if (rc) return rc;
    }
    sum.num_linear_solves++;
    evaluate(e, cand, cand_ne, true, false);
    sum.num_jacobian_evals++;
    if (pipelined) {
      const LmDecideArgs da{e->d_dec.p, x_cost, radius, min_relative_decrease, max_radius,
                            parameter_tolerance, function_tolerance, gradient_tolerance, min_radius};
      gradient_norm(e, cand, cand_ne, false, true, &da);
      spec_ready = false;
      if (iter < max_iterations) {
        spec_out = 0;
        while (spec_out == cur || spec_out == cand) ++spec_out;
        spec_chol_seq0 = e->chol_seq;
        rc = lm_step(e, cand_ne, 0.0, apply_launch(e, cand, spec_out, 1.0), true, &e->d_dec.p->radius_next,
                     &e->d_dec.p->go);
        if (rc) return rc;
        spec_ready = true;
        spec_in_flight = true;
      }
    } else {
      gradient_norm(e, cand, cand_ne, false, !sharded);
      if (sharded) {
        rc = allreduce_scalars(e, true);
        if (rc) return rc;
      }
    }
    rc = read_scalars(e, true);
    if (rc) return rc;
    const LmScalars sc = *e->h_scal;
    StepOutcome o;
    if (pipelined) {
      const LmDecision dec = const_cast<const LmPublished*>(e->h_pub)->dec;
      if (spec_ready && !dec.go) {
        e->chol_seq = spec_chol_seq0;
        spec_ready = false;
      }
      if (dec.accept && !spec_ready) spec_in_flight = false;
      o.valid = dec.valid;
      o.accept = dec.accept;
      o.cost = sc.cost_eval; o.gmax = sc.gmax; o.step_norm2 = sc.step_norm2; o.x_norm2 = sc.x_norm2;
      o.radius_next = dec.radius_next;
    } else {
      const double model_cost_change = -sc.gd - 0.5 * sc.dHd;
      o.valid = !sc.chol_fail && std::isfinite(model_cost_change) && model_cost_change > 0.0;
      if (o.valid && is_constrained) {
        rc = line_search(e, cur, cand, x_cost, sc, sum);
        if (rc) return rc;
      }
      const LmScalars& c = *e->h_scal;
      o.cost = c.cost_eval; o.gmax = c.gmax; o.step_norm2 = c.step_norm2; o.x_norm2 = c.x_norm2;
      const double rho = (x_cost - o.cost) / model_cost_change;
      o.accept = o.valid && rho > min_relative_decrease;
      o.radius_next = std::min(max_radius, radius / std::max(1.0 / 3.0, 1.0 - std::pow(2.0 * rho - 1.0, 3)));
    }
    if (!o.valid) {
      ++sum.num_unsuccessful_steps;
      last_ok = false;
      if (++num_invalid >= max_consecutive_invalid) { term = CTVIO_TERM_FAILURE; break; }
      radius /= decrease_factor;
      decrease_factor *= 2.0;
      continue;
    }
    num_invalid = 0;
    const double step_norm = std::sqrt(o.step_norm2), x_norm = std::sqrt(o.x_norm2);
    if (step_norm <= parameter_tolerance * (x_norm + parameter_tolerance)) { term = CTVIO_TERM_PARAMETER; break; }
    if (std::fabs(x_cost - o.cost) <= function_tolerance * x_cost) { term = CTVIO_TERM_FUNCTION; break; }
    if (o.accept) {
      cur = cand;
      cur_ne = cand_ne;
      x_cost = o.cost;
      gmax = o.gmax;
      radius = o.radius_next;
      decrease_factor = 2.0;
      last_ok = true;
      ++sum.num_successful_steps;
    } else {
      radius /= decrease_factor;
      decrease_factor *= 2.0;
      last_ok = false;
      ++sum.num_unsuccessful_steps;
    }
  }
  if (cur == 2) {
    const int f = 0;
    DevState &a = e->xs, &b = e->x[f];
    swap(a.q, b.q); swap(a.p, b.p); swap(a.bias, b.bias); swap(a.rho, b.rho); swap(a.ld, b.ld); swap(a.tab, b.tab);
    cur = f;
  }
  e->cur = cur;
  e->table_valid = true;
  e->slab_zeroed[0] = e->slab_zeroed[1] = false;
  rc = shard_sync_inv_depths(e);
  if (rc) return rc;
  cudaEventRecord(e->ev1, st);
  rc = refresh_mirror(e);
  if (rc) return rc;
  CUDA_OK(cudaStreamSynchronize(st));
  float ms = 0;
  cudaEventElapsedTime(&ms, e->ev0, e->ev1);
  sum.iterations = iter;
  sum.termination = term;
  sum.final_cost = x_cost;
  sum.final_radius = radius;
  sum.device_ms = ms;
  sum.kernel_launches = e->launches - launches0;
  if (out) *out = sum;
  return CTVIO_OK;
}

}
```

Baseline: 35.58 million.

## Fuse visual, IMU and small-factor evaluation into one role-split kernel with PDL chaining

Replaces the separate visual, IMU, small-factor and prior kernels, previously forked across three streams with events, with a single evaluate kernel whose CTAs take roles by block index. It is launched with programmatic dependent launch after the step kernel. Zeroing of the next normal-equation slab moves into spare CTAs of the step/apply kernel when speculation is active, and the first speculative LM step is issued before the initial scalar readback. Visual chunk sizing now reserves SMs for the side-role CTAs. The aim is to cut launch, event and memset overhead and overlap the stages. The cost is that IMU and small work share the visual kernel's register and shared-memory footprint.

```diff
diff --git a/ctrl-vio_b200/csrc/engine.cu b/ctrl-vio_b200/csrc/engine.cu
--- a/ctrl-vio_b200/csrc/engine.cu
+++ b/ctrl-vio_b200/csrc/engine.cu
@@ -136,24 +136,6 @@
       groups.push_back(make_int2(k, end));
       k = end;
     }
-    auto n_chunks = [&](int c) {
-      size_t m = 0;
-      for (const int2& g : groups) m += (g.y - g.x + c - 1) / c;
-      return m;
-    };
-    int cap = kVisObsPerRound;
-    const size_t n_sm = size_t(device_sm_count());
-    while (cap / 2 >= kVisMinChunk && n_chunks(cap / 2) <= n_sm) cap /= 2;
-    std::vector<VisualItem>& items = e->h_items;
-    items.clear();
-    for (const int2& g : groups) {
-      const int a = e->img_order[g.x];
-      const int cnt = g.y - g.x;
-      const int nchunks = (cnt + cap - 1) / cap;
-      const int per = (cnt + nchunks - 1) / nchunks;
-      for (int s = g.x; s < g.y; s += per) items.push_back(VisualItem{s, std::min(per, g.y - s), wi0[a], wj0[a]});
-    }
-    e->n_items = int(items.size());
     if (!e->img_desc.empty()) {
       std::vector<ctvio::FactorDesc> sd(n);
       for (int k = 0; k < n; ++k) sd[k] = e->img_desc[e->img_order[k]];
@@ -171,7 +153,6 @@
       CUDA_OK(e->d_img_meta.upload(hm, st));
     }
     CUDA_OK(e->d_img_orig.upload(e->img_order, st));
-    CUDA_OK(e->d_items.upload(items, st));
 
     e->h_woff.assign(e->nL + 1, 0);
     for (int l = 0; l < e->nL; ++l) {
@@ -236,6 +217,29 @@
     }
     CUDA_OK(e->d_bf_ij.upload(bij, st));
     CUDA_OK(e->d_bf_s.upload(bs, st));
+
+    auto n_chunks = [&](int c) {
+      size_t m = 0;
+      for (const int2& g : groups) m += (g.y - g.x + c - 1) / c;
+      return m;
+    };
+    const bool side_roles = e->rank == 0;
+    const size_t n_side = size_t(eval_side_ctas(side_roles ? e->n_imu_items : 0, side_roles ? nb : 0,
+                                                side_roles && e->prior_enabled ? e->prior.n : 0, true));
+    int cap = kVisObsPerRound;
+    const size_t n_sm = size_t(device_sm_count());
+    while (cap / 2 >= kVisMinChunk && n_chunks(cap / 2) + n_side <= n_sm) cap /= 2;
+    std::vector<VisualItem>& items = e->h_items;
+    items.clear();
+    for (const int2& g : groups) {
+      const int a = e->img_order[g.x];
+      const int cnt = g.y - g.x;
+      const int nchunks = (cnt + cap - 1) / cap;
+      const int per = (cnt + nchunks - 1) / nchunks;
+      for (int s = g.x; s < g.y; s += per) items.push_back(VisualItem{s, std::min(per, g.y - s), wi0[a], wj0[a]});
+    }
+    e->n_items = int(items.size());
+    CUDA_OK(e->d_items.upload(items, st));
 
     const size_t np = size_t(d.np);
     e->off_gc = np * np;
@@ -494,9 +498,22 @@
   return a;
 }
 
-void evaluate(ctvio_engine* e, int xb, int nb, bool full, bool reset_cost) {
+EvalLaunch eval_launch(ctvio_engine* e, int xb, int nb) {
+  EvalLaunch l;
+  l.vis = visual_launch(e, xb, nb, e->cfg.cauchy_solve);
+  l.imu = imu_launch(e, xb, nb);
+  l.small = small_launch(e, xb, nb);
+  if (e->rank != 0) {
+    l.imu.n_items = 0;
+    l.small.bf.n = 0;
+    l.small.prior.n = 0;
+  }
+  return l;
+}
+
+void evaluate(ctvio_engine* e, int xb, int nb, bool full, bool reset_cost, bool chained) {
   cudaStream_t st = e->stream;
-  if (full) {
+  if (full && !chained) {
     if (e->slab_zeroed[nb]) {
       cudaStreamWaitEvent(st, e->ev_zero, 0);
       e->slab_zeroed[nb] = false;
@@ -505,34 +522,9 @@
     }
   }
   if (reset_cost) cudaMemsetAsync(&e->d_scal.p->cost_eval, 0, sizeof(double), st);
-  const bool fork = (e->rank == 0) && (!e->imu.empty() || !e->biasf.empty() || (e->prior.n > 0 && e->prior_enabled));
-  if (e->deterministic) {
-    cudaMemsetAsync(e->d_ticket.p, 0, 2 * sizeof(int32_t), st);
-    e->launches += launch_visual(visual_launch(e, xb, nb, e->cfg.cauchy_solve), full, st);
-    if (fork) {
-      cudaMemsetAsync(e->d_ticket.p, 0, 2 * sizeof(int32_t), st);
-      e->launches += launch_imu(imu_launch(e, xb, nb), full, st);
-      e->launches += launch_small_factors(small_launch(e, xb, nb), full, st);
-    }
-    return;
-  }
-  const bool split = fork && !e->imu.empty() && (!e->biasf.empty() || (e->prior.n > 0 && e->prior_enabled));
-  if (fork) {
-    cudaEventRecord(e->ev_fork, st);
-    cudaStreamWaitEvent(e->stream2, e->ev_fork, 0);
-    e->launches += launch_imu(imu_launch(e, xb, nb), full, e->stream2);
-    if (split) {
-      cudaStreamWaitEvent(e->stream3, e->ev_fork, 0);
-      e->launches += launch_small_factors(small_launch(e, xb, nb), full, e->stream3);
-      cudaEventRecord(e->ev_join3, e->stream3);
-    } else {
-      e->launches += launch_small_factors(small_launch(e, xb, nb), full, e->stream2);
-    }
-    cudaEventRecord(e->ev_join, e->stream2);
-  }
-  e->launches += launch_visual(visual_launch(e, xb, nb, e->cfg.cauchy_solve), full, st);
-  if (fork) cudaStreamWaitEvent(st, e->ev_join, 0);
-  if (split) cudaStreamWaitEvent(st, e->ev_join3, 0);
+  EvalLaunch l = eval_launch(e, xb, nb);
+  l.pdl = chained ? 1 : 0;
+  e->launches += launch_evaluate(l, full, kEvalAll, st);
 }
 
 int read_scalars(ctvio_engine* e, bool published) {
@@ -543,7 +535,6 @@
       if ((++spins & 0xfffu) == 0 && cudaStreamQuery(e->stream) != cudaErrorNotReady) {
         if (*seq == e->pub_seq) break;
         CUDA_OK(cudaStreamSynchronize(e->stream));
-        CUDA_OK(cudaStreamSynchronize(e->stream2));
         if (*seq != e->pub_seq) return fail(CTVIO_ERR_CUDA, "LM step finished without publishing its scalars");
       }
     }
@@ -978,7 +969,7 @@
   e->launches += ctvio::launch_abs_column_sums(dr.p + 2 * ni, int(nm), 6, dout.p + 2, st);
   e->launches += ctvio::launch_bias_abs_sums(e->d_bf_ij.p, e->d_bf_s.p, int(nb), e->x[e->cur].bias.p, dout.p + 8, st);
   if (np_ > 0) {
-    e->launches += launch_small_factors(small_launch(e, e->cur, e->cur), false, st);
+    e->launches += launch_evaluate(eval_launch(e, e->cur, e->cur), false, kEvalSmall, st);
   }
   rc = read_scalars(e);
   if (rc) return rc;
@@ -1081,7 +1072,7 @@
       if (flush_l2) cudaMemsetAsync(flush.p, it & 0xff, flush_bytes, st);
       cudaMemsetAsync(e->ne_slab[cur].p, 0, e->ne_slab_len * sizeof(double), st);
       cudaEventRecord(e->ev0, st);
-      launch_visual(visual_launch(e, cur, cur, e->cfg.cauchy_solve), true, st);
+      launch_evaluate(eval_launch(e, cur, cur), true, kEvalVisual, st);
       cudaEventRecord(e->ev1, st);
       if (cudaEventSynchronize(e->ev1) != cudaSuccess) return fail(CTVIO_ERR_CUDA, "kernel failed while profiling");
       float ms = 0;
@@ -1114,14 +1105,14 @@
         cudaMemsetAsync(e->ne_slab[cur].p, 0, e->ne_slab_len * sizeof(double), st);
       cudaEventRecord(e->ev0, st);
       switch (stage) {
-        case 0: launch_visual(visual_launch(e, cur, cur, e->cfg.cauchy_solve), true, st); break;
-        case 1: launch_imu(imu_launch(e, cur, cur), true, st); break;
-        case 2: launch_small_factors(small_launch(e, cur, cur), true, st); break;
+        case 0: launch_evaluate(eval_launch(e, cur, cur), true, kEvalVisual, st); break;
+        case 1: launch_evaluate(eval_launch(e, cur, cur), true, kEvalImu, st); break;
+        case 2: launch_evaluate(eval_launch(e, cur, cur), true, kEvalSmall, st); break;
         case 3: launch_reduced_system(lin, 1e4, st); break;
         case 4: launch_factor_solve(lin, st); break;
         case 5: launch_step_vectors(lin, st); break;
         case 6: launch_apply_step(ap, st); break;
-        default: launch_visual(visual_launch(e, cur, cur, e->cfg.cauchy_solve), false, st); break;
+        default: launch_evaluate(eval_launch(e, cur, cur), false, kEvalVisual, st); break;
       }
       cudaEventRecord(e->ev1, st);
       if (cudaEventSynchronize(e->ev1) != cudaSuccess) return fail(CTVIO_ERR_CUDA, "kernel failed while profiling");
diff --git a/ctrl-vio_b200/csrc/engine_state.h b/ctrl-vio_b200/csrc/engine_state.h
--- a/ctrl-vio_b200/csrc/engine_state.h
+++ b/ctrl-vio_b200/csrc/engine_state.h
@@ -277,7 +277,7 @@
 }
 
 int prepare(ctvio_engine* e);
-void evaluate(ctvio_engine* e, int xb, int nb, bool full, bool reset_cost = true);
+void evaluate(ctvio_engine* e, int xb, int nb, bool full, bool reset_cost = true, bool chained = false);
 int read_scalars(ctvio_engine* e, bool published = false);
 LinearLaunch linear_launch(ctvio_engine* e, int nb);
 int refresh_mirror(ctvio_engine* e);
diff --git a/ctrl-vio_b200/csrc/kernels.h b/ctrl-vio_b200/csrc/kernels.h
--- a/ctrl-vio_b200/csrc/kernels.h
+++ b/ctrl-vio_b200/csrc/kernels.h
@@ -216,8 +216,6 @@
   LmScalars* scal;
   int* det_ticket = nullptr;
 };
-int launch_visual(const VisualLaunch& a, bool full, cudaStream_t s);
-size_t visual_smem_bytes();
 
 struct ImuLaunch {
   ImuObsPtrs obs;
@@ -232,7 +230,6 @@
   LmScalars* scal;
   int* det_ticket = nullptr;
 };
-int launch_imu(const ImuLaunch& a, bool full, cudaStream_t s);
 
 struct SmallFactorsLaunch {
   BiasFactorPtrs bf;
@@ -244,7 +241,16 @@
   LmScalars* scal;
   int deterministic = 0;
 };
-int launch_small_factors(const SmallFactorsLaunch& a, bool full, cudaStream_t s);
+
+enum : unsigned { kEvalVisual = 1u, kEvalImu = 2u, kEvalSmall = 4u, kEvalAll = 7u };
+struct EvalLaunch {
+  VisualLaunch vis;
+  ImuLaunch imu;
+  SmallFactorsLaunch small;
+  int32_t pdl = 0;
+};
+int launch_evaluate(const EvalLaunch& a, bool full, unsigned roles, cudaStream_t s);
+int eval_side_ctas(int n_imu_items, int n_bias_factors, int prior_n, bool full);
 
 int launch_probe_image(const VisualLaunch& a, const int32_t* orig_index, bool want_jac, double* r, int32_t* s,
                        double* J, cudaStream_t st);
@@ -282,6 +288,8 @@
   int* det_ticket;
   const int32_t* go;
   int32_t pdl = 0;
+  double* clear = nullptr;
+  size_t clear_len = 0;
 };
 int launch_jacobi_scale(const LinearLaunch& a, cudaStream_t s);
 int launch_lm_step(const LinearLaunch& a, double radius, cudaStream_t s);
diff --git a/ctrl-vio_b200/csrc/kernels_linear.cu b/ctrl-vio_b200/csrc/kernels_linear.cu
--- a/ctrl-vio_b200/csrc/kernels_linear.cu
+++ b/ctrl-vio_b200/csrc/kernels_linear.cu
@@ -505,21 +505,30 @@
   return 1;
 }
 
-__global__ void __launch_bounds__(256) step_apply_kernel(LinearLaunch a, ApplyLaunch ap, int ncb, int nlb) {
+__global__ void __launch_bounds__(256) step_apply_kernel(LinearLaunch a, ApplyLaunch ap, int ncb, int nlb, int nab) {
   extern __shared__ double step_dsh[];
   const int b = blockIdx.x;
+  const int z = b - (ncb + nlb + nab);
+  if (z >= 0 && *a.go) {
+    const int nzb = gridDim.x - (ncb + nlb + nab);
+    const size_t n2 = a.clear_len / 2;
+    double2* c2 = reinterpret_cast<double2*>(a.clear);
+    for (size_t i = size_t(z) * blockDim.x + threadIdx.x; i < n2; i += size_t(nzb) * blockDim.x) c2[i] = make_double2(0.0, 0.0);
+    if (z == 0 && threadIdx.x == 0 && (a.clear_len & 1)) a.clear[a.clear_len - 1] = 0.0;
+  }
   pdl_wait();
   pdl_launch_dependents();
   if (b < ncb) camera_step_block(a, b, step_dsh);
   else if (b < ncb + nlb) landmark_step_block(a, b - ncb, &ap);
-  else apply_step_block(ap, StepSource{nullptr, a.y, a.sc, a.cmask}, b - ncb - nlb, false);
+  else if (b < ncb + nlb + nab) apply_step_block(ap, StepSource{nullptr, a.y, a.sc, a.cmask}, b - ncb - nlb, false);
 }
 
 int launch_step_and_apply(const LinearLaunch& a, const ApplyLaunch& ap, cudaStream_t s) {
   const int ncb = (a.dims.np + 7) / 8, nlb = (a.dims.nL + 7) / 8;
   const int nab = (a.dims.nK + 6 * a.dims.nB + 1 + 255) / 256;
-  launch_chained(a.pdl, step_apply_kernel, dim3(ncb + nlb + nab), dim3(256), size_t(a.dims.np) * sizeof(double), s, a, ap,
-                 ncb, nlb);
+  const int nzb = a.clear ? int(std::min<size_t>(32, (a.clear_len + 8191) / 8192)) : 0;
+  launch_chained(a.pdl, step_apply_kernel, dim3(ncb + nlb + nab + nzb), dim3(256), size_t(a.dims.np) * sizeof(double), s,
+                 a, ap, ncb, nlb, nab);
   return 1;
 }
 
diff --git a/ctrl-vio_b200/csrc/kernels_residual.cu b/ctrl-vio_b200/csrc/kernels_residual.cu
--- a/ctrl-vio_b200/csrc/kernels_residual.cu
+++ b/ctrl-vio_b200/csrc/kernels_residual.cu
@@ -69,6 +69,7 @@
   const uint8_t* cmask;
   LmScalars* scal;
   int* det_ticket;
+  int32_t b0;
 };
 
 struct __align__(128) VisStatic {
@@ -88,8 +89,8 @@
 #ifdef CTVIO_CHOL_TIMING
 __device__ long long g_vis_clk[8];
 __device__ long long g_imu_clk[8];
-#define VCLK(i) do { if (blockIdx.x == 0 && threadIdx.x == 0) g_vis_clk[(i)] = clock64(); } while (0)
-#define ICLK(i) do { if (blockIdx.x == 0 && threadIdx.x == 0) g_imu_clk[(i)] = clock64(); } while (0)
+#define VCLK(i) do { if (chunk() == 0 && threadIdx.x == 0) g_vis_clk[(i)] = clock64(); } while (0)
+#define ICLK(i) do { if (b == 0 && threadIdx.x == 0) g_imu_clk[(i)] = clock64(); } while (0)
 extern "C" int ctvio_debug_vis_clk(long long* out) {
   return cudaMemcpyFromSymbol(out, g_vis_clk, sizeof(g_vis_clk)) == cudaSuccess ? 0 : -1;
 }
@@ -101,9 +102,10 @@
 #define ICLK(i)
 #endif
 
-size_t visual_smem_bytes() {
+__host__ __device__ constexpr size_t visual_tile_bytes() {
   return size_t(kVisObsPerRound) * kObsStride * sizeof(double) + size_t(36) * 64 * sizeof(double);
 }
+static_assert(visual_tile_bytes() % 128 == 0, "VisStatic behind the tile keeps the TMA destinations aligned");
 
 template <bool DIAG>
 __device__ __noinline__ void syrk_round_warp(const double* Jt, double* accs, int nround, int warp, int lane) {
@@ -174,16 +176,18 @@
 }
 
 template <bool FULL>
-__global__ void __launch_bounds__(kVisThreads, 1) visual_kernel(const __grid_constant__ VisArgs a) {
-  extern __shared__ __align__(128) unsigned char dyn_smem[];
-  double* Jt = reinterpret_cast<double*>(dyn_smem);
+__device__ __forceinline__ void visual_role(const VisArgs& a, unsigned char* smem) {
+  const auto chunk = [&] { return int(blockIdx.x) - a.b0; };
+  double* Jt = reinterpret_cast<double*>(smem);
   double* accs = Jt + size_t(kVisObsPerRound) * kObsStride;
-  __shared__ VisStatic sm;
+  VisStatic& sm = *reinterpret_cast<VisStatic*>(smem + (FULL ? visual_tile_bytes() : 0));
 
   const int tid = threadIdx.x;
   const int lane = tid & 31, warp = tid >> 5;
-  const VisualItem item = a.items[blockIdx.x];
+  const VisualItem item = a.items[chunk()];
   const int nK = a.dims.nK;
+  pdl_wait();
+  pdl_launch_dependents();
   VCLK(0);
 
   const int w0[2] = {item.wi0, item.wj0};
@@ -339,7 +343,7 @@
       __syncthreads();
       VCLK(3);
       if (a.det_ticket) {
-        det_ticket_wait(a.det_ticket, blockIdx.x * 1024 + base / kVisObsPerRound);
+        det_ticket_wait(a.det_ticket, chunk() * 1024 + base / kVisObsPerRound);
         if (active && valid) {
           const int oi = item.start + base + ol;
           const int l = a.obs.meta[oi].z;
@@ -366,7 +370,7 @@
           __threadfence();
           __syncthreads();
         }
-        det_ticket_done(a.det_ticket, blockIdx.x * 1024 + base / kVisObsPerRound);
+        det_ticket_done(a.det_ticket, chunk() * 1024 + base / kVisObsPerRound);
       }
       syrk_round(Jt, accs, nround, tid);
       VCLK(4);
@@ -374,7 +378,7 @@
   }
 
   const int n_rounds = (item.count + kVisObsPerRound - 1) / kVisObsPerRound;
-  det_ticket_wait(a.det_ticket, blockIdx.x * 1024 + (FULL ? n_rounds : 0));
+  det_ticket_wait(a.det_ticket, chunk() * 1024 + (FULL ? n_rounds : 0));
   cost_local = warp_sum(cost_local);
   if (lane == 0) sm.cost_part[warp] = cost_local;
   __syncthreads();
@@ -424,22 +428,9 @@
   if (a.det_ticket) {
     __threadfence();
     __syncthreads();
-    if (tid == 0) asm volatile("st.release.gpu.global.s32 [%0], %1;" ::"l"(a.det_ticket), "r"((int(blockIdx.x) + 1) * 1024) : "memory");
+    if (tid == 0) asm volatile("st.release.gpu.global.s32 [%0], %1;" ::"l"(a.det_ticket), "r"((chunk() + 1) * 1024) : "memory");
   }
   VCLK(5);
-}
-
-int launch_visual(const VisualLaunch& l, bool full, cudaStream_t s) {
-  if (l.n_items <= 0) return 0;
-  VisArgs a{l.obs, l.items, l.st, l.ne, l.lm, l.dims, l.sp, l.rig, l.cauchy, l.cmask, l.scal, l.det_ticket};
-  static PerDeviceOnce once;
-  if (once.first()) {
-    cudaFuncSetAttribute(visual_kernel<true>, cudaFuncAttributeMaxDynamicSharedMemorySize, int(visual_smem_bytes()));
-    cudaFuncSetAttribute(visual_kernel<false>, cudaFuncAttributeMaxDynamicSharedMemorySize, int(visual_smem_bytes()));
-  }
-  if (full) visual_kernel<true><<<l.n_items, kVisThreads, visual_smem_bytes(), s>>>(a);
-  else visual_kernel<false><<<l.n_items, kVisThreads, 0, s>>>(a);
-  return 1;
 }
 
 
@@ -549,12 +540,16 @@
     }
 }
 
+constexpr size_t kImuItemSmem = size_t(kImuCols) * kImuColStride * sizeof(double);
+
 template <bool FULL>
-__global__ void __launch_bounds__(kImuThreads) imu_kernel(const __grid_constant__ ImuArgs a) {
-  extern __shared__ __align__(128) unsigned char dyn_smem[];
-  double* Js = reinterpret_cast<double*>(dyn_smem);
-  const int tid = threadIdx.x, warp = tid >> 5, lane = tid & 31;
-  const ImuItem item = a.items[blockIdx.x];
+__device__ __forceinline__ void imu_role(const ImuArgs& a, int b, int n_items, int ticket0, unsigned char* smem) {
+  const int half = threadIdx.x / kImuThreads;
+  const int tid = threadIdx.x % kImuThreads, warp = tid >> 5, lane = tid & 31;
+  double* Js = reinterpret_cast<double*>(smem + half * kImuItemSmem);
+  const ImuItem item = 2 * b + half < n_items ? a.items[2 * b + half] : ImuItem{0, 0, 0, 0};
+  pdl_wait();
+  pdl_launch_dependents();
   double cost = 0.0;
   ICLK(0);
   if ((FULL || warp == 0) && lane < item.count) {
@@ -589,12 +584,12 @@
   } else if (FULL && lane == item.count) {
     imu_zero_part(Js + 6 * lane, warp);
   }
+  double acc[3][2];
   if (FULL) {
     ICLK(1);
     __syncthreads();
     ICLK(2);
     const int nsteps = (6 * item.count + 3) >> 2;
-    double acc[3][2];
     switch (warp) {
       case 0: imu_syrk<0>(Js, nsteps, lane, acc); break;
       case 1: imu_syrk<1>(Js, nsteps, lane, acc); break;
@@ -603,32 +598,31 @@
     }
     ICLK(3);
     ICLK(4);
-    det_ticket_wait(a.det_ticket, blockIdx.x);
-    switch (warp) {
-      case 0: imu_flush<0>(a, item, lane, acc); break;
-      case 1: imu_flush<1>(a, item, lane, acc); break;
-      case 2: imu_flush<2>(a, item, lane, acc); break;
-      default: imu_flush<3>(a, item, lane, acc); break;
-    }
-    ICLK(5);
-  }
-  if (!FULL) det_ticket_wait(a.det_ticket, blockIdx.x);
-  if (warp == 0) {
-    cost = warp_sum(cost);
-    if (lane == 0 && cost != 0.0) atomicAdd(a.ne.cost, cost);
-  }
-  det_ticket_done(a.det_ticket, blockIdx.x);
-}
-
-int launch_imu(const ImuLaunch& l, bool full, cudaStream_t s) {
-  if (l.n_items <= 0) return 0;
-  ImuArgs a{l.obs, l.items, l.st, l.ne, l.dims, l.sp, l.rig, l.cmask, l.scal, l.det_ticket};
-  const size_t smem = size_t(kImuCols) * kImuColStride * sizeof(double);
-  static PerDeviceOnce once;
-  if (once.first()) cudaFuncSetAttribute(imu_kernel<true>, cudaFuncAttributeMaxDynamicSharedMemorySize, int(smem));
-  if (full) imu_kernel<true><<<l.n_items, kImuThreads, smem, s>>>(a);
-  else imu_kernel<false><<<l.n_items, kImuThreads, 0, s>>>(a);
-  return 1;
+  }
+  det_ticket_wait(a.det_ticket, ticket0 + 2 * b);
+  for (int h = 0; h < 2; ++h) {
+    if (half == h) {
+      if (FULL) {
+        switch (warp) {
+          case 0: imu_flush<0>(a, item, lane, acc); break;
+          case 1: imu_flush<1>(a, item, lane, acc); break;
+          case 2: imu_flush<2>(a, item, lane, acc); break;
+          default: imu_flush<3>(a, item, lane, acc); break;
+        }
+        ICLK(5);
+      }
+      if (warp == 0) {
+        cost = warp_sum(cost);
+        if (lane == 0 && cost != 0.0) atomicAdd(a.ne.cost, cost);
+      }
+    }
+    if (a.det_ticket) {
+      __threadfence();
+      __syncthreads();
+    }
+  }
+  if (a.det_ticket && threadIdx.x == 0)
+    asm volatile("st.release.gpu.global.s32 [%0], %1;" ::"l"(a.det_ticket), "r"(ticket0 + min(2 * b + 2, n_items)) : "memory");
 }
 
 
@@ -655,8 +649,11 @@
 }
 
 template <bool FULL>
-__global__ void __launch_bounds__(256) small_factors_kernel(const __grid_constant__ SmallArgs a) {
-  __shared__ double red[8];
+__device__ __forceinline__ void small_role(const SmallArgs& a, int* det_ticket, int my_ticket, unsigned char* smem) {
+  double* red = reinterpret_cast<double*>(smem);
+  pdl_wait();
+  pdl_launch_dependents();
+  det_ticket_wait(det_ticket, my_ticket);
   const int tid = threadIdx.x;
   double cost = 0.0;
   const int np = a.dims.np;
@@ -727,33 +724,101 @@
     for (int w = 0; w < 8; ++w) c += red[w];
     if (c != 0.0) atomicAdd(a.ne.cost, c);
   }
-}
-
-__global__ void prior_add_jtj_kernel(PriorPtrs pr, double* A, int np) {
-  const int idx = blockIdx.x * blockDim.x + threadIdx.x;
+  det_ticket_done(det_ticket, my_ticket);
+}
+
+__device__ __forceinline__ void prior_role(const PriorPtrs& pr, double* A, int np, int b, int nblk, const int* det_ticket,
+                                           int my_ticket) {
+  pdl_wait();
+  pdl_launch_dependents();
+  det_ticket_wait(det_ticket, my_ticket);
   const int n = pr.n;
-  if (idx >= n * n) return;
-  const int i = idx / n, j = idx % n;
-  if (j < i) return;
-  const int gi = pr.col2g[i], gj = pr.col2g[j];
-  if (gi < 0 || gj < 0) return;
-  const double v = pr.JtJ[idx];
-  if (v == 0.0) return;
-  atomicAdd(A + size_t(min(gi, gj)) * np + max(gi, gj), v);
-}
-
-int launch_small_factors(const SmallFactorsLaunch& l, bool full, cudaStream_t s) {
-  if (l.bf.n <= 0 && l.prior.n <= 0) return 0;
-  SmallArgs a{l.bf, l.prior, l.st, l.ne, l.dims, l.cmask, l.scal, l.deterministic};
-  int launches = 1;
-  if (full) small_factors_kernel<true><<<1, 256, 0, s>>>(a);
-  else small_factors_kernel<false><<<1, 256, 0, s>>>(a);
-  if (full && l.prior.n > 0) {
-    const int n2 = l.prior.n * l.prior.n;
-    prior_add_jtj_kernel<<<(n2 + 255) / 256, 256, 0, s>>>(l.prior, l.ne.A, l.dims.np);
-    ++launches;
-  }
-  return launches;
+  for (int idx = b * blockDim.x + threadIdx.x; idx < n * n; idx += nblk * blockDim.x) {
+    const int i = idx / n, j = idx % n;
+    if (j < i) continue;
+    const int gi = pr.col2g[i], gj = pr.col2g[j];
+    if (gi < 0 || gj < 0) continue;
+    const double v = pr.JtJ[idx];
+    if (v == 0.0) continue;
+    atomicAdd(A + size_t(min(gi, gj)) * np + max(gi, gj), v);
+  }
+}
+
+
+struct EvalArgs {
+  VisArgs vis;
+  ImuArgs imu;
+  SmallArgs small;
+  int32_t vis0, n_vis;
+  int32_t imu0, n_imu;
+  int32_t small0, n_small;
+  int32_t prior0, n_prior;
+  int32_t n_imu_items;
+  int32_t t_imu, t_small;
+  int* det_ticket;
+};
+
+template <bool FULL>
+__global__ void __launch_bounds__(kVisThreads, 1) evaluate_kernel(const __grid_constant__ EvalArgs a) {
+  extern __shared__ __align__(128) unsigned char dyn_smem[];
+  const int b = blockIdx.x;
+  if (b >= a.vis0 && b < a.vis0 + a.n_vis) visual_role<FULL>(a.vis, dyn_smem);
+  else if (b >= a.imu0 && b < a.imu0 + a.n_imu) imu_role<FULL>(a.imu, b - a.imu0, a.n_imu_items, a.t_imu, dyn_smem);
+  else if (b >= a.small0 && b < a.small0 + a.n_small) small_role<FULL>(a.small, a.det_ticket, a.t_small, dyn_smem);
+  else prior_role(a.small.prior, a.small.ne.A, a.small.dims.np, b - a.prior0, a.n_prior, a.det_ticket, a.t_small + 1);
+}
+
+static_assert(2 * kImuItemSmem <= visual_tile_bytes(), "two K2 items fit in K1's shared memory");
+size_t evaluate_smem_bytes(bool full) { return (full ? visual_tile_bytes() : 0) + sizeof(VisStatic); }
+
+static int prior_ctas(int prior_n, bool full) {
+  return (full && prior_n > 0) ? (prior_n * prior_n + 4095) / 4096 : 0;
+}
+
+int eval_side_ctas(int n_imu_items, int n_bias_factors, int prior_n, bool full) {
+  return (n_imu_items + 1) / 2 + ((n_bias_factors > 0 || prior_n > 0) ? 1 : 0) + prior_ctas(prior_n, full);
+}
+
+int launch_evaluate(const EvalLaunch& l, bool full, unsigned roles, cudaStream_t s) {
+  EvalArgs a;
+  const VisualLaunch& v = l.vis;
+  const ImuLaunch& m = l.imu;
+  const SmallFactorsLaunch& f = l.small;
+  a.vis = VisArgs{v.obs, v.items, v.st, v.ne, v.lm, v.dims, v.sp, v.rig, v.cauchy, v.cmask, v.scal, v.det_ticket, 0};
+  a.imu = ImuArgs{m.obs, m.items, m.st, m.ne, m.dims, m.sp, m.rig, m.cmask, m.scal, v.det_ticket};
+  a.small = SmallArgs{f.bf, f.prior, f.st, f.ne, f.dims, f.cmask, f.scal, f.deterministic};
+  a.det_ticket = v.det_ticket;
+  a.n_vis = (roles & kEvalVisual) ? v.n_items : 0;
+  a.n_imu_items = (roles & kEvalImu) ? m.n_items : 0;
+  a.n_imu = (a.n_imu_items + 1) / 2;
+  const bool small = (roles & kEvalSmall) != 0;
+  a.n_small = small && (f.bf.n > 0 || f.prior.n > 0) ? 1 : 0;
+  a.n_prior = small ? prior_ctas(f.prior.n, full) : 0;
+  const int side = a.n_imu + a.n_small + a.n_prior;
+  const int grid = a.n_vis + side;
+  if (grid == 0) return 0;
+  if (a.det_ticket) {
+    a.vis0 = 0;
+    a.imu0 = a.n_vis;
+  } else {
+    a.imu0 = 0;
+    a.vis0 = side;
+  }
+  a.vis.b0 = a.vis0;
+  a.small0 = a.imu0 + a.n_imu;
+  a.prior0 = a.small0 + a.n_small;
+  a.t_imu = a.n_vis * 1024;
+  a.t_small = a.t_imu + a.n_imu_items;
+  const size_t smem = evaluate_smem_bytes(full);
+  static PerDeviceOnce once;
+  if (once.first()) {
+    cudaFuncSetAttribute(evaluate_kernel<true>, cudaFuncAttributeMaxDynamicSharedMemorySize, int(evaluate_smem_bytes(true)));
+    cudaFuncSetAttribute(evaluate_kernel<false>, cudaFuncAttributeMaxDynamicSharedMemorySize, int(evaluate_smem_bytes(false)));
+  }
+  if (a.det_ticket) cudaMemsetAsync(a.det_ticket, 0, 2 * sizeof(int32_t), s);
+  if (full) launch_chained(l.pdl, evaluate_kernel<true>, dim3(grid), dim3(kVisThreads), smem, s, a);
+  else launch_chained(l.pdl, evaluate_kernel<false>, dim3(grid), dim3(kVisThreads), smem, s, a);
+  return 1;
 }
 
 
diff --git a/ctrl-vio_b200/csrc/solve.cu b/ctrl-vio_b200/csrc/solve.cu
--- a/ctrl-vio_b200/csrc/solve.cu
+++ b/ctrl-vio_b200/csrc/solve.cu
@@ -97,6 +97,10 @@
   LinearLaunch lin = linear_launch(e, nb);
   lin.go = go;
   lin.pdl = pdl ? 1 : 0;
+  if (go) {
+    lin.clear = e->ne_slab[nb ^ 1].p;
+    lin.clear_len = e->ne_slab_len;
+  }
   cudaStream_t st = e->stream;
   if (e->deterministic) cudaMemsetAsync(e->d_ticket.p, 0, 2 * sizeof(int32_t), st);
   e->launches += launch_reduced_system(lin, radius, st, radius_dev);
@@ -226,10 +230,33 @@
   } else {
     e->launches += launch_jacobi_scale(lin, st);
   }
+  bool spec_size_ok = e->img.size() <= 20000;
+  if (const char* sp = std::getenv("CTVIO_SPECULATION")) {
+    if (std::strcmp(sp, "always") == 0) spec_size_ok = true;
+    if (std::strcmp(sp, "never") == 0) spec_size_ok = false;
+  }
+  const bool pipelined = spec_size_ok && !sharded && !is_constrained && !e->deterministic;
+  if (pipelined) {
+    rc = alloc_state(e, e->xs);
+    if (rc) return rc;
+  }
   gradient_norm(e, cur, cur, true, !sharded);
   if (sharded) {
     rc = allreduce_scalars(e);
     if (rc) return rc;
+  }
+  int cur_ne = cur;
+  bool spec_ready = false;
+  bool spec_in_flight = false;
+  int spec_out = -1;
+  unsigned spec_chol_seq0 = e->chol_seq;
+  if (pipelined && max_iterations > 0) {
+    spec_out = 0;
+    while (spec_out == cur) ++spec_out;
+    cudaMemsetAsync(e->ne_slab[cur_ne ^ 1].p, 0, e->ne_slab_len * sizeof(double), st);
+    rc = lm_step(e, cur_ne, initial_radius, apply_launch(e, cur, spec_out, 1.0), true);
+    if (rc) return rc;
+    spec_ready = true;
   }
   rc = read_scalars(e, !sharded);
   if (rc) return rc;
@@ -244,21 +271,6 @@
   int iter = 0;
   int term = CTVIO_TERM_NO_CONVERGENCE;
 
-  bool spec_size_ok = e->img.size() <= 20000;
-  if (const char* sp = std::getenv("CTVIO_SPECULATION")) {
-    if (std::strcmp(sp, "always") == 0) spec_size_ok = true;
-    if (std::strcmp(sp, "never") == 0) spec_size_ok = false;
-  }
-  const bool pipelined = spec_size_ok && !sharded && !is_constrained && !e->deterministic;
-  if (pipelined) {
-    rc = alloc_state(e, e->xs);
-    if (rc) return rc;
-  }
-  int cur_ne = cur;
-  bool spec_ready = false;
-  bool spec_in_flight = false;
-  int spec_out = -1;
-  unsigned spec_chol_seq0 = e->chol_seq;
   while (true) {
     if (iter >= max_iterations) { term = CTVIO_TERM_NO_CONVERGENCE; break; }
     if (last_ok && gmax <= gradient_tolerance) { term = CTVIO_TERM_GRADIENT; break; }
@@ -266,9 +278,9 @@
     ++iter;
     const int cand_ne = cur_ne ^ 1;
     int cand;
-    if (spec_ready) {
+    const bool speculated = spec_ready;
+    if (speculated) {
       cand = spec_out;
-      prezero_slab(e, cand_ne);
     } else {
       cand = 0;
       while (cand == cur) ++cand;
@@ -277,7 +289,7 @@
       if (rc) return rc;
     }
     sum.num_linear_solves++;
-    evaluate(e, cand, cand_ne, true, false);
+    evaluate(e, cand, cand_ne, true, false, speculated);
     sum.num_jacobian_evals++;
     if (pipelined) {
       const LmDecideArgs da{e->d_dec.p, x_cost, radius, min_relative_decrease, max_radius,
```

New measurement: 36.88 million (median of 6 runs). +3.6%, better.
